# liangfu/dspnet

Hardware: AMD Instinct MI355X
Metric: training images/sec at 512x512 multitask (higher is better)
Workload: dtype f32; 1 GPU; resnet-50 multitask (det+depth+seg) 512x512, 8 det classes, 19 seg classes, N=6132 anchors, forward+backward+SGD; batch_per_gpu=32, global_batch=32, parallelism=dp1, f16x2_fallback_calls=0

## Files before the change

### dspnet_amd/csrc/bn_final_job.h

```cpp
#pragma once
#include <hip/hip_runtime.h>

namespace dspn {

constexpr int kBnJobChannels = 16;

struct BnFinalJob {
  const float *tile_sums;
  int tiles, C, blocks;
  double inv_rows;
  const float *mean, *rstd, *gamma;
  float *coef, *dgamma, *dbeta;
  const float *dy_absmax, *x_minmax;
  unsigned *dx_bound, *dx_bound_min;
};

void bn_job_defer(hipStream_t s, const BnFinalJob &job);
bool bn_job_take(hipStream_t s, BnFinalJob *job);

__device__ __forceinline__ void bn_final_channel(const int c, const int C, const double S, const double SS, const double inv_rows,
                                                 const float *__restrict__ mean, const float *__restrict__ rstd, const float *__restrict__ gamma,
                                                 float *__restrict__ coef, float *__restrict__ dgamma, float *__restrict__ dbeta,
                                                 const float *__restrict__ x_minmax, unsigned *__restrict__ dx_bound,
                                                 unsigned *__restrict__ dx_bound_min, const float D) {
  if (dbeta) dbeta[c] = (float)S;
  if (dgamma) dgamma[c] = (float)SS;
  const double rs = rstd[c], mu = mean[c];
  const double a = (gamma ? (double)gamma[c] : 1.0) * rs;
  const double c1 = -a * rs * (SS * inv_rows);
  coef[c] = (float)a;
  coef[C + c] = (float)c1;
  const double c0 = -a * (S * inv_rows) - c1 * mu;
  coef[2 * C + c] = (float)c0;
  if (dx_bound) {
    const double lo = x_minmax[c], hi = x_minmax[C + c];
    double b = fabs(a) * (double)D + fmax(fabs(c1 * lo + c0), fabs(c1 * hi + c0));
    b *= 1.0 + 1e-6;
    float bf = (float)b;
    if (!(bf == bf)) bf = INFINITY;
    if (bf > 0.f) atomicMax(dx_bound + (c & 63), __float_as_uint(bf));
    if (dx_bound_min && bf > 0.f && bf < INFINITY) atomicMin(dx_bound_min, __float_as_uint(bf));
  }
}

__device__ __forceinline__ void bn_final_job_run(const BnFinalJob &j, const int b, void *smem) {
  double *s_S = static_cast<double *>(smem), *s_SS = s_S + 16 * kBnJobChannels;
  float *s_D = reinterpret_cast<float *>(s_SS + 16 * kBnJobChannels);
  const int tid = threadIdx.x;
  if (j.dx_bound && tid < 64) {
    float m = j.dy_absmax[tid];
#pragma unroll
    for (int o = 32; o >= 1; o >>= 1) m = fmaxf(m, __shfl_xor(m, o, 64));
    if (tid == 0) *s_D = m;
  }
  const int cl = tid & (kBnJobChannels - 1), v = tid >> 4;
  const int c = b * kBnJobChannels + cl;
  const int C = j.C;
  if (tid < 256) {
    double S = 0, SS = 0;
    if (c < C) {
      const float *__restrict__ ts = j.tile_sums;
#pragma unroll 8
      for (int k = v; k < j.tiles; k += 16) {
        S += ts[(long long)k * 2 * C + c];
        SS += ts[(long long)k * 2 * C + C + c];
      }
    }
    s_S[v * kBnJobChannels + cl] = S; s_SS[v * kBnJobChannels + cl] = SS;
  }
  __syncthreads();
  if (tid < kBnJobChannels && c < C) {
    double S = s_S[cl], SS = s_SS[cl];
    for (int k = 1; k < 16; ++k) { S += s_S[k * kBnJobChannels + cl]; SS += s_SS[k * kBnJobChannels + cl]; }
    bn_final_channel(c, C, S, SS, j.inv_rows, j.mean, j.rstd, j.gamma, j.coef, j.dgamma, j.dbeta, j.x_minmax, j.dx_bound,
                     j.dx_bound_min, j.dx_bound ? *s_D : 0.f);
// ... 5 lines not shown
```

### dspnet_amd/csrc/conv.hip

```cpp
#include "dspn_common.h"
#include "bn_final_job.h"
#include "dspn_store.h"
#include "dspn_pieces.h"
#include "conv_geom.h"
#include <cstdlib>
#include "../../include/dspn_nn.h"

using dspn::st_t;
using dspn::kHalf;
using dspn::u32x4_t;

namespace {

using dspn::conv::f32x16;
using dspn::conv::bf16x8;
using dspn::pieces::bf16x4;
typedef __attribute__((address_space(3))) bf16x4 lds_bf16x4;

constexpr int kLdsRowH = kHalf ? 72 : 40;
__device__ __forceinline__ bf16x4 to_bf16x4(const float4 v) {
  bf16x4 r = {(__bf16)v.x, (__bf16)v.y, (__bf16)v.z, (__bf16)v.w};
  return r;
}

// ... 1630 lines not shown
    splits = (int)std::min<long long>((384 + nblk - 1) / nblk, nk / 8);
    splits = std::max(1, std::min(splits, 32));
    while (splits > 1 && sizeof(float) * (size_t)splits * M * g.Cout > ws.bytes) --splits;
    per = (nk + splits - 1) / splits;
    splits = (nk + per - 1) / per;
  }
  static const int eight_mode = (int)dspn::env_int("DSPN_NT_8WAVE", -1);
  const bool one_tap = g.TR * g.TS == 1;
  const bool eight = eight_mode == 0 ? false : eight_mode == 1 ? true : (kHalf || g.bf16 >= 2) ? true
                     : ((!g.stats && !g.bn_sums) || (eight_mode == 2 && one_tap && g.bn_sums) || (eight_mode == 3 && one_tap));
  bool wide_ok = splits == 1 && (cfg == 0 || (cfg == 2 && g.Cout > 32 && g.Cout <= 64)) && (g.flags & 16) && g.Cout % 4 == 0 &&
                 g.TR * g.TS > 0;
  if (kHalf) wide_ok = wide_ok && !g.in_scale && g.Cin % 64 == 0 && dspn::wide_tiles_mode() >= 2;
  else wide_ok = wide_ok && pre && g.bf16 == 3;
  const dspn::conv::WideRoute route = wide_ok ? dspn::conv::wide_route(g, M, nk) : dspn::conv::WideRoute{};
  if (g.sadd) {
    constexpr const char *who = DSPN_FN_NAME(dspn_conv2d_dgrad_bn_sadd);
    if (kHalf) return dspn::fail(DSPN_ERR_ARG_, "%s: the strided addend takes float tensors only", who);
    if (g.bf16 != 3) return dspn::fail(DSPN_ERR_ARG_, "%s: the strided addend needs DSPN_MATH_F32_F16X2", who);
    if (splits > 1) return dspn::fail(DSPN_ERR_ARG_, "%s: the strided addend cannot be combined with split-K (%d splits)", who, splits);
    if (!g.bn_sums) return dspn::fail(DSPN_ERR_ARG_, "%s: the strided addend needs the BatchNorm-backward sums (bn_sums)", who);
    if (!g.dense || g.ldc != g.Cout || (g.flags & (1 | 2 | 4 | 8)) || residual)
      return dspn::fail(DSPN_ERR_ARG_, "%s: the strided addend needs a dense dx written by this call alone (no accumulate)", who);
    if (g.sadd_h != (g.Hg + 1) / 2 || g.sadd_w != (g.Wg + 1) / 2 || g.Wg < 8 || g.Wg % 4 != 0)
      return dspn::fail(DSPN_ERR_ARG_, "%s: the strided addend is (N, ceil(H / 2), ceil(W / 2), Cin) with W >= 8 and W %% 4 == 0, got %d x %d for %d x %d", who,
                        g.sadd_h, g.sadd_w, g.Hg, g.Wg);
    if (!((route.tile == dspn::conv::WideTile::P128x128 || route.tile == dspn::conv::WideTile::P128x256) &&
          route.loop == dspn::conv::WideLoop::Spanning))
      return dspn::fail(DSPN_ERR_ARG_, "%s: no kernel takes the strided addend on this route (it needs dy as piece planes, N H W %% 128 == 0 "
                        "and the plane-fed 128-row tiles on the tile-spanning loop)", who);
    g.sadd_bytes = (unsigned)((long long)sizeof(st_t) * g.N * g.sadd_h * g.sadd_w * g.Cout);
    if (g.probe) return 0;
  }
  if (route) return dspn::conv::launch_wide(route, in, w, bias, out, g, s, residual);
  const int rc = cfg == 0 && eight ? launch_nt<4, 2, 1, 2>(in, w, bias, out, g, s, splits, per, ws.ptr, residual)
                 : cfg == 0        ? launch_nt<2, 2, 2, 2>(in, w, bias, out, g, s, splits, per, ws.ptr, residual)
                 : cfg == 1        ? launch_nt<2, 2, 2, 1>(in, w, bias, out, g, s, splits, per, ws.ptr, residual)
                 : cfg == 2        ? launch_nt<2, 2, 1, 1>(in, w, bias, out, g, s, splits, per, ws.ptr, residual)
                                   : launch_nt<4, 1, 2, 1>(in, w, bias, out, g, s, splits, per, ws.ptr, residual);
  return rc ? rc : output_absmax_pass(out, g, s);
}

struct WgradPlan { int bm; int bn; int splits; int pps; };
constexpr int kPlanPK = 64;
static_assert(kPlanPK % kPK == 0, "split sizes must be whole k-steps");
long long wgrad_x_footprint(long long P, int Cin, int taps, int stride) { return taps > 1 ? 4ll * P * Cin * std::min(stride, 2) * std::min(stride, 2) : 0; }
WgradPlan wgrad_plan(long long P, int Cout, int J, long long x_bytes = 0, long long max_splits = 1 << 30) {
  WgradPlan p;
  p.bm = Cout <= 32 ? 32 : (Cout <= 64 ? 64 : 128);
  if (p.bm == 128 && (Cout + 63) / 64 * 64 < (Cout + 127) / 128 * 128) p.bm = 64;
  p.bn = (J <= 64 && p.bm == 128) ? 64 : 128;
  if (const char *e = getenv("DSPN_WG_TILE")) {
    const int t = atoi(e);
    p.bm = t == 0 ? 32 : (t == 1 ? 64 : 128);
    p.bn = t == 2 ? 64 : 128;
  }
  const long long tiles = (long long)((Cout + p.bm - 1) / p.bm) * ((J + p.bn - 1) / p.bn);
  const long long lds = 4ll * std::max(2 * kPK * (p.bm + p.bn), p.bm * (p.bn + 4));
  const long long slots = 256 * std::min<long long>(8, (160ll << 10) / lds);
  long long s_min = 1;
  if (x_bytes > 0) s_min = (x_bytes + (32ll << 20) - 1) / (32ll << 20);
  const long long s_max = std::max<long long>(1, std::min<long long>(std::min<long long>(P / 128, 1024), max_splits));
  s_min = std::min(s_min, s_max);
  const double flop_per_pix = 2.0 * p.bm * p.bn, slot_rate = 120e12 / (double)slots, ovh_pix = 160;
  double best = 1e30;
  long long splits = s_min;
// ... 268 lines not shown
  return dspn::check_launch("absmax_batch");
}

int dspn_conv2d_weight_planes_batch_f32(const void *table, int n, long long total_tiles, void *stream) {
  DSPN_REQUIRE(table && n > 0 && total_tiles > 0 && total_tiles < (1ll << 31), "weight_planes_batch: bad argument");
  static_assert(sizeof(WpDesc) == 64, "table row layout: 3 pointers, 4 ints, 1 int64, 1 pointer, 2 ints");
  hipLaunchKernelGGL(weight_planes_batch_kernel, dim3((unsigned)total_tiles), dim3(256), 0, (hipStream_t)stream,
                     static_cast<const WpDesc *>(table), n);
  return dspn::check_launch("weight_planes_batch");
}
#else
int dspn_conv2d_weight_prepare_bf16(const float *w, st_t *wh, st_t *wt, int Cout, int taps, int Cin,
                                    int Cout_pad, void *stream) {
  DSPN_REQUIRE(w && wt && Cout > 0 && taps > 0 && Cin > 0 && Cout_pad >= Cout && Cout_pad % kEPC == 0,
               "weight_prepare: bad argument");
  const long long total = (long long)Cin * taps * Cout_pad;
  const int blocks = (int)std::min<long long>((total + 255) / 256, 4096);
  hipLaunchKernelGGL(weight_transpose_kernel, dim3(blocks), dim3(256), 0, (hipStream_t)stream, w,
                     wt, wh, Cout, taps, Cin, Cout_pad);
  return dspn::check_launch("weight_prepare");
}

int dspn_conv2d_weight_prepare_batch_bf16(const void *table, int n, long long total_tiles, void *stream) {
  DSPN_REQUIRE(table && n > 0 && total_tiles > 0 && total_tiles < (1ll << 31), "weight_prepare_batch: bad argument");
  static_assert(sizeof(WtDesc) == 48, "table row layout: 2 pointers, 4 ints, 1 int64, 1 pointer");
  hipLaunchKernelGGL(weight_transpose_batch_kernel, dim3((unsigned)total_tiles), dim3(256), 0, (hipStream_t)stream,
                     static_cast<const WtDesc *>(table), n);
  return dspn::check_launch("weight_prepare_batch");
}
#endif

struct BnBwd { const st_t *x; const float *scale, *shift, *mean, *rstd; int relu; float *sums; float *dy_absmax; };
struct StridedAddend { const st_t *p; int h, w, probe; };

static int dgrad_tiles(int N, int H, int W, int Cin, int stride, int *per_class ) {
  int total = 0;
  for (int ph = 0; ph < (stride == 1 ? 1 : 2); ++ph)
    for (int pw = 0; pw < (stride == 1 ? 1 : 2); ++pw) {
      const long long hg = stride == 1 ? H : (H - ph + 1) / 2, wg = stride == 1 ? W : (W - pw + 1) / 2;
      const long long M = (long long)N * hg * wg;
      const int t = M > 0 ? (int)((M + kNtBm[nt_config(M, Cin)] - 1) / kNtBm[nt_config(M, Cin)]) : 0;
      if (per_class) per_class[ph * 2 + pw] = t;
      total += t;
    }
  return total;
}

static int conv2d_dgrad_one(int math, OpScales scales, const st_t *dy, const st_t *wt, const void *wt_planes, st_t *dx, int N, int H, int W,
                          int Cin, int ldy, int R, int S, int stride, int pad_h, int pad_w, int dil, int Ho,
                          int Wo, int dx_ldc, int accumulate, BnBwd bn, void *workspace, size_t workspace_bytes,
                          void *stream, StridedAddend sa = StridedAddend{nullptr, 0, 0, 0}) {
  DSPN_REQUIRE(dy && (wt || wt_planes) && dx, "conv2d_dgrad: null pointer");
  DSPN_REQUIRE(ldy % kEPC == 0, "conv2d_dgrad: dy channel stride must be a multiple of %d", kEPC);
  DSPN_REQUIRE(stride == 1 || (stride == 2 && dil == 1), "conv2d_dgrad: stride 1, or stride 2 with dilation 1");
  DSPN_REQUIRE(N > 0 && H > 0 && W > 0 && Cin > 0 && R > 0 && S > 0, "conv2d_dgrad: bad geometry");
  ConvGeom g;
  memset(&g, 0, sizeof(g));
  g.N = N; g.Hin = Ho; g.Win = Wo; g.Cin = ldy; g.Cout = Cin;
  g.WTAPS = R * S; g.WS = S;
  g.ldc = dx_ldc > 0 ? dx_ldc : Cin;
  g.obs = (long long)H * W * g.ldc;
  g.OW = W;
  g.flags = accumulate ? 4 : 0;
  g.bf16 = kHalf ? 1 : math;
  g.w_planes = wt_planes;
  g.a_absmax = scales.a; g.b_absmax = scales.b;
  g.bn_x = bn.x; g.bn_scale = bn.scale; g.bn_shift = bn.shift; g.bn_mean = bn.mean; g.bn_rstd = bn.rstd;
  g.bn_relu = bn.relu; g.bn_sums = bn.sums; g.bn_tile_base = 0;
  g.bn_dy_absmax = (bn.sums && !kHalf && math == DSPN_MATH_F32_F16X2) ? reinterpret_cast<unsigned *>(bn.dy_absmax) : nullptr;
  g.a_planes = scales.a_planes;
  g.sadd = sa.p; g.sadd_h = sa.h; g.sadd_w = sa.w; g.probe = sa.probe;
  int class_tiles[4] = {0, 0, 0, 0};
  if (bn.sums) dgrad_tiles(N, H, W, Cin, stride, class_tiles);
  hipStream_t s = (hipStream_t)stream;
  const SplitWs sws{static_cast<float *>(workspace), workspace ? workspace_bytes : 0};
  if (stride == 1) {
    g.Hg = H; g.Wg = W; g.ish = 1; g.isw = 1; g.ioh = pad_h; g.iow = pad_w; g.idh = -dil; g.idw = -dil;
    g.TR = R; g.TS = S; g.wr0 = 0; g.wrs = 1; g.ws0 = 0; g.wss = 1;
    g.osh = 1; g.osw = 1; g.dense = 1;
    return dispatch_nt(dy, wt, nullptr, dx, g, s, sws);
  }
  for (int ph = 0; ph < 2; ++ph)
    for (int pw = 0; pw < 2; ++pw) {
      ConvGeom c = g;
      c.Hg = (H - ph + 1) / 2; c.Wg = (W - pw + 1) / 2;
      for (int q = 0; q < ph * 2 + pw; ++q) c.bn_tile_base += class_tiles[q];
      if (c.Hg <= 0 || c.Wg <= 0) continue;
      const int r0 = (ph + pad_h) & 1, s0 = (pw + pad_w) & 1;
      c.TR = r0 < R ? (R - r0 + 1) / 2 : 0;
      c.TS = s0 < S ? (S - s0 + 1) / 2 : 0;
      if (c.TR == 0 || c.TS == 0) {
        c.TR = 0; c.TS = 1;
        if (accumulate && !bn.sums) continue;
      }
      c.ish = 1; c.isw = 1; c.ioh = (ph + pad_h - r0) / 2; c.iow = (pw + pad_w - s0) / 2;
      c.idh = -1; c.idw = -1;
      c.wr0 = r0; c.wrs = 2; c.ws0 = s0; c.wss = 2;
      c.osh = 2; c.osw = 2; c.ooh = ph; c.oow = pw; c.dense = 0;
      const int rc = dispatch_nt(dy, wt, nullptr, dx, c, s, sws);
      if (rc) return rc;
    }
  return 0;
}

static int dgrad_bn_tiles(int N, int H, int W, int Cin, int stride) {
  if (N <= 0 || H <= 0 || W <= 0 || Cin <= 0 || Cin % 4 != 0 || (stride != 1 && stride != 2)) return 0;
  return dgrad_tiles(N, H, W, Cin, stride, nullptr);
}
#ifndef DSPN_HALF
int dspn_conv2d_dgrad_bn_tiles(int N, int H, int W, int Cin, int stride) { return dgrad_bn_tiles(N, H, W, Cin, stride); }
#endif

}
static int conv2d_dgrad_bn_impl(const st_t *dy, const st_t *wt, const void *wt_planes, st_t *dx, int N, int H, int W,
                             int Cin, int ldy, int R, int S, int stride, int pad_h, int pad_w, int dil, int Ho,
                             int Wo, int dx_ldc, int accumulate,
                             const st_t *bn_x, const float *bn_scale, const float *bn_shift, const float *bn_mean,
                             const float *bn_rstd, int bn_relu, float *bn_sums, size_t bn_sums_bytes, float *bn_dy_absmax,
                             int math, const float *dy_absmax, const float *w_absmax, void *workspace, size_t workspace_bytes,
                             void *stream, StridedAddend sa) {
  DSPN_REQUIRE(N > 0 && Ho > 0 && Wo > 0 && ldy > 0, "conv2d_dgrad: bad geometry");
  if (sa.p) {
    constexpr const char *who = DSPN_FN_NAME(dspn_conv2d_dgrad_bn_sadd);
    DSPN_REQUIRE(stride == 1 && !accumulate, "%s: the strided addend goes with a stride-1 data gradient that is the only writer of dx (no accumulate)", who);
    DSPN_REQUIRE((dx_ldc <= 0 || dx_ldc == Cin), "%s: the strided addend needs a dense dx (dx_ldc %d, Cin %d)", who, dx_ldc, Cin);
    DSPN_REQUIRE(batch_chunk(N, (long long)sizeof(st_t) * Ho * Wo * ldy) == N, "%s: dy of 2 GiB or more", who);
  }
  const int flags = split_math(&math, DSPN_MATH_DY_PLANES), dy_planes = (flags & DSPN_MATH_DY_PLANES) ? 1 : 0;
  DSPN_REQUIRE(!dy_planes || (!dspn::kHalf && math == DSPN_MATH_F32_F16X2 && ldy % 32 == 0 && dy_absmax),
               "conv2d_dgrad: DSPN_MATH_DY_PLANES needs DSPN_MATH_F32_F16X2, ldy %% 32 == 0 and the block the planes were cut by (dy_absmax)");
  if (const int rc = check_math_mode("conv2d_dgrad", math)) return rc;
  if (const int rc = check_math_blocks("conv2d_dgrad", math, flags, dy_absmax, w_absmax)) return rc;
  const int ldc = dx_ldc > 0 ? dx_ldc : Cin;
  const int nb = batch_chunk(N, (long long)sizeof(st_t) * Ho * Wo * ldy);
  if (bn_sums) {
    DSPN_REQUIRE(bn_x && bn_mean && bn_rstd && (!bn_relu || (bn_scale && bn_shift)), "conv2d_dgrad: BatchNorm operands missing");
    DSPN_REQUIRE(ldc == Cin && nb == N, "conv2d_dgrad: BatchNorm sums need a dense dx and dy below 2 GiB");
    const int tiles = dgrad_bn_tiles(N, H, W, Cin, stride);
    DSPN_REQUIRE(tiles > 0 && bn_sums_bytes >= sizeof(float) * 2 * (size_t)tiles * Cin,
                 "conv2d_dgrad: bn_sums needs dspn_conv2d_dgrad_bn_tiles() x 2 x Cin floats");
  }
  for (int n0 = 0; n0 < N; n0 += nb) {
    const int n = std::min(nb, N - n0);
    const int rc = conv2d_dgrad_one(math, OpScales{dy_absmax, w_absmax, dy_planes}, dy + (long long)n0 * Ho * Wo * ldy, wt, wt_planes, dx + (long long)n0 * H * W * ldc, n, H,
                                    W, Cin, ldy, R, S, stride, pad_h, pad_w, dil, Ho, Wo, dx_ldc, accumulate,
                                    BnBwd{bn_x, bn_scale, bn_shift, bn_mean, bn_rstd, bn_relu, bn_sums, bn_dy_absmax}, workspace,
                                    workspace_bytes, stream, sa);
    if (rc) return rc;
  }
  return 0;
}
extern "C" {
int DSPN_FN(dspn_conv2d_dgrad_bn)(const st_t *dy, const st_t *wt, const void *wt_planes, st_t *dx, int N, int H, int W,
                             int Cin, int ldy, int R, int S, int stride, int pad_h, int pad_w, int dil, int Ho,
                             int Wo, int dx_ldc, int accumulate,
                             const st_t *bn_x, const float *bn_scale, const float *bn_shift, const float *bn_mean,
                             const float *bn_rstd, int bn_relu, float *bn_sums, size_t bn_sums_bytes, float *bn_dy_absmax,
                             int math, const float *dy_absmax, const float *w_absmax, void *workspace, size_t workspace_bytes,
                             void *stream) {
  return conv2d_dgrad_bn_impl(dy, wt, wt_planes, dx, N, H, W, Cin, ldy, R, S, stride, pad_h, pad_w, dil, Ho, Wo, dx_ldc, accumulate, bn_x,
                              bn_scale, bn_shift, bn_mean, bn_rstd, bn_relu, bn_sums, bn_sums_bytes, bn_dy_absmax, math, dy_absmax,
                              w_absmax, workspace, workspace_bytes, stream, StridedAddend{nullptr, 0, 0, 0});
}
int DSPN_FN(dspn_conv2d_dgrad_bn_sadd)(const st_t *dy, const st_t *wt, const void *wt_planes, st_t *dx, int N, int H, int W,
                             int Cin, int ldy, int R, int S, int stride, int pad_h, int pad_w, int dil, int Ho,
                             int Wo, int dx_ldc, int accumulate,
                             const st_t *bn_x, const float *bn_scale, const float *bn_shift, const float *bn_mean,
                             const float *bn_rstd, int bn_relu, float *bn_sums, size_t bn_sums_bytes, float *bn_dy_absmax,
                             int math, const float *dy_absmax, const float *w_absmax, void *workspace, size_t workspace_bytes,
                             const st_t *strided_addend, int addend_h, int addend_w, void *stream) {
  DSPN_REQUIRE(strided_addend && addend_h > 0 && addend_w > 0, "%s: no strided addend (dspn_conv2d_dgrad_bn is the call without one)",
               DSPN_FN_NAME(dspn_conv2d_dgrad_bn_sadd));
  return conv2d_dgrad_bn_impl(dy, wt, wt_planes, dx, N, H, W, Cin, ldy, R, S, stride, pad_h, pad_w, dil, Ho, Wo, dx_ldc, accumulate, bn_x,
                              bn_scale, bn_shift, bn_mean, bn_rstd, bn_relu, bn_sums, bn_sums_bytes, bn_dy_absmax, math, dy_absmax,
                              w_absmax, workspace, workspace_bytes, stream, StridedAddend{strided_addend, addend_h, addend_w, 0});
}
#ifndef DSPN_HALF
int dspn_conv2d_dgrad_bn_sadd_route_f32(int N, int H, int W, int Cin, int ldy, int dy_planes) {
  float *const q = reinterpret_cast<float *>(uintptr_t(256));
  const int tiles = dgrad_bn_tiles(N, H, W, Cin, 1);
  if (tiles <= 0 || N <= 0 || ldy <= 0) return 0;
  return conv2d_dgrad_bn_impl(q, nullptr, q, q, N, H, W, Cin, ldy, 1, 1, 1, 0, 0, 1, H, W, Cin, 0, q, q, q, q, q, 1, q,
                              sizeof(float) * 2 * (size_t)tiles * Cin, q, DSPN_MATH_F32_F16X2 | (dy_planes ? DSPN_MATH_DY_PLANES : 0), q, q,
                              nullptr, 0, nullptr, StridedAddend{q, (H + 1) / 2, (W + 1) / 2, 1}) == 0 ? 1 : 0;
}
#endif

#ifndef DSPN_HALF
int dspn_conv2d_dgrad_f32(const float *dy, const float *wt, float *dx, int N, int H, int W,
                          int Cin, int ldy, int R, int S, int stride, int pad_h, int pad_w, int dil, int Ho,
                          int Wo, int dx_ldc, int accumulate, void *workspace, size_t workspace_bytes,
                          void *stream) {
  return dspn_conv2d_dgrad_bn_f32(dy, wt, nullptr, dx, N, H, W, Cin, ldy, R, S, stride, pad_h, pad_w, dil, Ho, Wo, dx_ldc,
                                  accumulate, nullptr, nullptr, nullptr, nullptr, nullptr, 0, nullptr, 0, nullptr, DSPN_MATH_FP32,
                                  nullptr, nullptr, workspace, workspace_bytes, stream);
}

size_t dspn_conv2d_input_sum_grad_workspace_bytes(int Ho, int Wo, int ldy, int R, int S) {
  return sizeof(float) * ((size_t)Ho * Wo * ldy + (size_t)R * S * 32 * ldy);
}
#endif

int DSPN_FN(dspn_conv2d_input_sum_grad)(const st_t *dy, const float *w, float *out, int N, int H, int W,
                                   int Cin, int Cout, int ldy, int R, int S, int stride, int pad_h, int pad_w, int dil,
                                   int Ho, int Wo, void *workspace, size_t workspace_bytes, void *stream) {
  DSPN_REQUIRE(dy && w && out && workspace, "conv2d_input_sum_grad: null pointer");
  DSPN_REQUIRE(ldy % 4 == 0 && Cin >= 1 && Cin <= 8, "conv2d_input_sum_grad: Cin <= 8, ldy % 4 == 0");
  if (workspace_bytes < sizeof(float) * ((size_t)Ho * Wo * ldy + (size_t)R * S * 32 * ldy))
    return dspn::fail(DSPN_ERR_WORKSPACE_, "conv2d_input_sum_grad: workspace too small");
  hipStream_t s = (hipStream_t)stream;
  float *p2 = static_cast<float *>(workspace);
  float *partial = p2 + (size_t)Ho * Wo * ldy;
  const long long per4 = (long long)Ho * Wo * ldy / 4;
  hipLaunchKernelGGL(batch_sum_kernel, dim3((int)std::min<long long>((per4 + 255) / 256, 8192)), dim3(256), 0, s,
                     dspn::CA4Ptr(dy), reinterpret_cast<float4 *>(p2), N, per4);
  SumGradGeom g{H, W, Ho, Wo, ldy, R, S, stride, stride, pad_h, pad_w, dil, dil, 32};
  hipLaunchKernelGGL(tap_sum_kernel, dim3(R * S, 32), dim3(256), 0, s, p2, partial, g);
// ... 146 lines not shown
```

### dspnet_amd/csrc/conv_geom.h

```cpp
#pragma once
#include <hip/hip_runtime.h>

namespace dspn {
namespace conv {

typedef float f32x16 __attribute__((ext_vector_type(16)));
typedef __bf16 bf16x8 __attribute__((ext_vector_type(8)));

template <typename st_t>
struct ConvGeomT {
  int N, Hin, Win, Cin;
  int Hg, Wg;
  int ish, isw, ioh, iow, idh, idw;
  int TR, TS;
  int WTAPS, WS, wr0, wrs, ws0, wss;
  int Cout;
  long long obs;
  int OW, osh, osw, ooh, oow, ldc;
  int flags;
  int dense;
  int dbg;
  int bf16;
  unsigned in_bytes, w_bytes;
  const float *in_scale, *in_shift;
  float *stats;
  float *minmax;
  const st_t *bn_x;
  const float *bn_scale, *bn_shift, *bn_mean, *bn_rstd;
  float *bn_sums;
  int bn_relu, bn_tile_base;
  unsigned *bn_dy_absmax;
  const float *a_absmax, *b_absmax;
  int a_planes;
  const void *w_planes;
  const st_t *sadd;
  int sadd_h, sadd_w;
  unsigned sadd_bytes;
  int probe;
};

__device__ __forceinline__ int xcd_remap(int bid, int nblk) {
  const int q = nblk >> 3, r = nblk & 7, x = bid & 7;
  const int start = x < r ? x * (q + 1) : r * (q + 1) + (x - r) * q;
  return start + (bid >> 3);
}


enum class WideTile { None, P256x128, P128x256, P128x128, P256x64, F128x256, F128x128, F256x64 };
enum class WideLoop { Plain, Spanning, Direct };
struct WideRoute {
  WideTile tile = WideTile::None; WideLoop loop = WideLoop::Plain;
  explicit operator bool() const { return tile != WideTile::None; }
};
WideRoute wide_route(const ConvGeomT<float> &g, long long M, int nk);
WideRoute wide_route(const ConvGeomT<__bf16> &g, long long M, int nk);
int launch_wide(WideRoute r, const float *in, const float *w_planes, const float *bias, float *out, const ConvGeomT<float> &g,
                hipStream_t s, const float *residual);
int launch_wide(WideRoute r, const __bf16 *in, const __bf16 *w, const float *bias, __bf16 *out, const ConvGeomT<__bf16> &g,
                hipStream_t s, const __bf16 *residual);

int launch_stem(const float *x, const float *w, float *y, int N, int H, int W, int Cin, int Cout, int Ho, int Wo,
                const float *x_absmax, const float *w_absmax, float *stats, float *minmax, hipStream_t s);

}
}
```

### dspnet_amd/csrc/conv_wide.h

```cpp

#ifdef DSPN_STAMPS
__device__ unsigned long long g_wide_stamps[1024 * 16];
struct WideStamps {
  unsigned long long last, sum[16];
  __device__ __forceinline__ void begin() { for (int i = 0; i < 16; ++i) sum[i] = 0; last = __builtin_readcyclecounter(); }
  __device__ __forceinline__ void mark(int i) { const unsigned long long t = __builtin_readcyclecounter(); sum[i] += t - last; last = t; }
  __device__ __forceinline__ void flush() {
    if (threadIdx.x == 0 && blockIdx.x < 1024) for (int i = 0; i < 16; ++i) g_wide_stamps[blockIdx.x * 16 + i] = sum[i];
  }
};
#define DSPN_STAMP_DECL WideStamps stamps_; stamps_.begin()
#define DSPN_STAMP(i) stamps_.mark(i)
#define DSPN_STAMP_FLUSH stamps_.flush()
#define DSPN_STAMP_ARG , stamps_
#define DSPN_STAMP_PARAM , WideStamps &stamps_
#else
#define DSPN_STAMP_DECL
#define DSPN_STAMP(i)
#define DSPN_STAMP_FLUSH
#define DSPN_STAMP_ARG
#define DSPN_STAMP_PARAM
#endif

struct NoStage {};
// ... 170 lines not shown
  if constexpr (EPI == 2) {
    __builtin_amdgcn_s_barrier();
    float *red = reinterpret_cast<float *>(wsm);
    if (cvalid) {
#pragma unroll
      for (int h = 0; h < HALVES; ++h)
#pragma unroll
        for (int e = 0; e < 4; ++e) {
          red[((h * RPP + er0) * BN + c4 * 4 + e) * 2] = gs[h][e];
          red[((h * RPP + er0) * BN + c4 * 4 + e) * 2 + 1] = gss[h][e];
        }
    }
    asm volatile("s_waitcnt lgkmcnt(0)" ::: "memory");
    __builtin_amdgcn_s_barrier();
    for (int hc = tid; hc < HALVES * BN; hc += NTHR) {
      const int h = hc / BN, col = hc - h * BN;
      if (n0 + col >= g.Cout || m0 + h * SR >= M) continue;
      const float *rh = red + (size_t)h * RPP * BN * 2;
      float a = 0.f, b = 0.f;
      for (int er = 0; er < RPP; ++er) { a += rh[(er * BN + col) * 2]; b += rh[(er * BN + col) * 2 + 1]; }
      const long long mt_ = g.bn_tile_base + m0 / SR + h;
      g.bn_sums[(mt_ * 2 + 0) * g.Cout + n0 + col] = a;
      g.bn_sums[(mt_ * 2 + 1) * g.Cout + n0 + col] = b;
    }
    gmx_all = fmaxf(gmx_all, gmx);
  }
  if constexpr (EPI == 0) gmx_all = fmaxf(gmx_all, gmx);
  asm volatile("s_waitcnt lgkmcnt(0)" ::: "memory");
  __builtin_amdgcn_s_barrier();
  DSPN_STAMP(6);
}

#ifndef DSPN_HALF
template <int WAVES_M, int WAVES_N, int EPI, int RB = 16, int SR = 128, bool CLOSE = false, bool SADD = false>
__device__ __forceinline__ void direct_epilogue(const ConvGeom &g, char *exch, f32x16 (&acc)[2][2], const float inv_a, const float inv_b, const int m0,
                                                const int n0, const int M, const int tid, const int wave,
                                                const float *__restrict__ bias, float *__restrict__ out,
                                                const float *__restrict__ residual, float &gmx_all) {
  constexpr int TM = 2, TN = 2, BN = WAVES_N * 64, NTHR = WAVES_M * WAVES_N * 64, PARTS = WAVES_M * 2;
  constexpr int WRT = SR / 64, TILES = WAVES_M / WRT, PPT = WRT * 2;
  static_assert(SR == 64 || SR == 128, "statistics tiles of 64 or 128 rows");
  static_assert(WAVES_M % WRT == 0, "whole statistics tiles per output tile");
  const int lane = tid & 63, half = lane >> 5, lc = lane & 31;
  const int wr = wave / WAVES_N, wm = wr * 64, wn = (wave % WAVES_N) * 64;
  const bool has_bias = g.flags & 1, relu = g.flags & 2, accum = g.flags & 4, has_res = g.flags & 8;
  const float *addsrc = has_res ? residual : (accum ? out : nullptr);
  const unsigned obytes = (unsigned)M * (unsigned)g.ldc * 4u;
  const __amdgpu_buffer_rsrc_t rs_o = __builtin_amdgcn_make_buffer_rsrc(out, 0, obytes, 0x00020000);
  const __amdgpu_buffer_rsrc_t rs_a = __builtin_amdgcn_make_buffer_rsrc(const_cast<float *>(addsrc ? addsrc : out), 0, addsrc ? obytes : 0u, 0x00020000);
  const __amdgpu_buffer_rsrc_t rs_x = __builtin_amdgcn_make_buffer_rsrc(const_cast<float *>(EPI == 2 ? g.bn_x : out), 0, EPI == 2 ? obytes : 0u, 0x00020000);
  constexpr unsigned kOOB = 0x80000000u;
  constexpr float kInf = __builtin_huge_valf();
  int col[TN];
  unsigned cbyte[TN];
  bool cv[TN];
  float bv[TN], bsc[TN], bsh[TN], bmu[TN], brs[TN];
#pragma unroll
  for (int j = 0; j < TN; ++j) {
    col[j] = n0 + wn + j * 32 + lc;
    cv[j] = col[j] < g.Cout;
    cbyte[j] = cv[j] ? (unsigned)col[j] * 4u : kOOB;
    bv[j] = (has_bias && cv[j]) ? bias[col[j]] : 0.f;
    bsc[j] = bsh[j] = bmu[j] = brs[j] = 0.f;
    if (EPI == 2 && cv[j]) {
      bmu[j] = g.bn_mean[col[j]]; brs[j] = g.bn_rstd[col[j]];
      if (g.bn_relu) { bsc[j] = g.bn_scale[col[j]]; bsh[j] = g.bn_shift[col[j]]; }
    }
  }
  const int row0 = m0 + wm + 4 * half;
  const unsigned pitch = (unsigned)g.ldc * 4u;
  float sK[TN], s1[TN], s2[TN], vmn[TN], vmx[TN], gs[TN], gss[TN];
  int scnt = 0;
  float gmx = 0.f;
#pragma unroll
  for (int j = 0; j < TN; ++j) { sK[j] = 0.f; s1[j] = 0.f; s2[j] = 0.f; vmn[j] = kInf; vmx[j] = -kInf; gs[j] = 0.f; gss[j] = 0.f; }
  const bool both = has_res && accum;
  constexpr int NB = TM * 16 / RB;
  const bool need_rows = addsrc != nullptr || EPI == 2;
  if constexpr (EPI == 2) {
    float rq[2][RB][TN], xq[2][RB][TN], oq[2][RB][TN];
    int sa_n = 0, sa_h = 0, sa_w = 0;
    __amdgpu_buffer_rsrc_t rs_s = rs_a;
    if constexpr (SADD) {
      static_assert(!SADD || RB == 4, "one group of four rows per batch");
      rs_s = __builtin_amdgcn_make_buffer_rsrc(const_cast<float *>(g.sadd), 0, g.sadd_bytes, 0x00020000);
      const int hw = g.Hg * g.Wg;
      sa_n = row0 / hw;
      const int rem = row0 - sa_n * hw;
      sa_h = rem / g.Wg; sa_w = rem - sa_h * g.Wg;
    }
    auto request = [&](const int bb, const int s_) __attribute__((always_inline)) {
      const int i = bb / (16 / RB), r0 = (bb % (16 / RB)) * RB;
      unsigned sa_off[TN];
#pragma unroll
      for (int j = 0; j < TN; ++j) sa_off[j] = kOOB;
      if constexpr (SADD) {
        const unsigned sa_rb = (unsigned)((sa_n * g.sadd_h + (sa_h >> 1)) * g.sadd_w + (sa_w >> 1)) * pitch;
#pragma unroll
        for (int j = 0; j < TN; ++j) sa_off[j] = ((sa_h & 1) || !cv[j]) ? kOOB : sa_rb + cbyte[j];
        sa_w += 8;
        const bool wrap = sa_w >= g.Wg;
        sa_w -= wrap ? g.Wg : 0;
        sa_h += wrap ? 1 : 0;
        const bool wrap2 = sa_h >= g.Hg;
        sa_h = wrap2 ? 0 : sa_h;
        sa_n += wrap2 ? 1 : 0;
      }
#pragma unroll
      for (int rr = 0; rr < RB; ++rr) {
        const int r = r0 + rr;
        const unsigned rb = (unsigned)(row0 + 32 * i + (r & 3) + 8 * (r >> 2)) * pitch;
#pragma unroll
        for (int j = 0; j < TN; ++j) {
          const unsigned off = rb + cbyte[j];
          if constexpr (SADD)
            rq[s_][rr][j] = (rr & 1) ? 0.f : __builtin_bit_cast(float, __builtin_amdgcn_raw_buffer_load_b32(rs_s, (int)(sa_off[j] + (unsigned)(rr >> 1) * pitch), 0, 0));
          else
          rq[s_][rr][j] = addsrc ? __builtin_bit_cast(float, __builtin_amdgcn_raw_buffer_load_b32(rs_a, (int)off, 0, 0)) : 0.f;
          xq[s_][rr][j] = __builtin_bit_cast(float, __builtin_amdgcn_raw_buffer_load_b32(rs_x, (int)off, 0, 0));
          oq[s_][rr][j] = both ? __builtin_bit_cast(float, __builtin_amdgcn_raw_buffer_load_b32(rs_o, (int)off, 0, 0)) : 0.f;
        }
      }
    };
    request(0, 0);
#pragma unroll
    for (int bb = 0; bb < NB; ++bb) {
      const int i = bb / (16 / RB), r0 = (bb % (16 / RB)) * RB, s_ = bb & 1;
      if (bb + 1 < NB) request(bb + 1, s_ ^ 1);
#pragma unroll
      for (int rr = 0; rr < RB; ++rr) {
        const int r = r0 + rr;
        const unsigned rb = (unsigned)(row0 + 32 * i + (r & 3) + 8 * (r >> 2)) * pitch;
#pragma unroll
        for (int j = 0; j < TN; ++j) {
          float v = acc[i][j][r] * inv_a * inv_b + bv[j];
          v += rq[s_][rr][j];
          if (both) v += oq[s_][rr][j];
          if (relu) v = v > 0.f ? v : 0.f;
          __builtin_amdgcn_raw_buffer_store_b32(__builtin_bit_cast(unsigned, v), rs_o, (int)(rb + cbyte[j]), 0, 0);
          const float xv = xq[s_][rr][j];
          const float gd = (!g.bn_relu || fmaf(xv, bsc[j], bsh[j]) > 0.f) ? v : 0.f;
          gs[j] += gd;
          gss[j] += gd * ((xv - bmu[j]) * brs[j]);
          gmx = fmaxf(gmx, fabsf(v));
        }
      }
    }
#pragma unroll
    for (int j = 0; j < TN; ++j) { gs[j] = cv[j] ? gs[j] : 0.f; gss[j] = cv[j] ? gss[j] : 0.f; }
  } else {
    typedef float f32x2 __attribute__((ext_vector_type(2)));
    f32x2 s1p[TN], s2p[TN];
#pragma unroll
    for (int j = 0; j < TN; ++j) { s1p[j] = f32x2{0.f, 0.f}; s2p[j] = f32x2{0.f, 0.f}; }
    f32x2 rq[2][RB / 2][TN], oq[2][RB / 2][TN];
    auto request = [&](const int bb, const int s_) __attribute__((always_inline)) {
      const int i = bb / (16 / RB), r0 = (bb % (16 / RB)) * RB;
#pragma unroll
      for (int rr = 0; rr < RB; rr += 2) {
        const int r = r0 + rr;
        const unsigned rb = (unsigned)(row0 + 32 * i + (r & 3) + 8 * (r >> 2)) * pitch;
#pragma unroll
        for (int j = 0; j < TN; ++j) {
          const unsigned off = rb + cbyte[j];
          rq[s_][rr / 2][j] = f32x2{0.f, 0.f}; oq[s_][rr / 2][j] = f32x2{0.f, 0.f};
          if (addsrc) rq[s_][rr / 2][j] = f32x2{__builtin_bit_cast(float, __builtin_amdgcn_raw_buffer_load_b32(rs_a, (int)off, 0, 0)),
                                               __builtin_bit_cast(float, __builtin_amdgcn_raw_buffer_load_b32(rs_a, (int)(off + pitch), 0, 0))};
          if (both) oq[s_][rr / 2][j] = f32x2{__builtin_bit_cast(float, __builtin_amdgcn_raw_buffer_load_b32(rs_o, (int)off, 0, 0)),
                                             __builtin_bit_cast(float, __builtin_amdgcn_raw_buffer_load_b32(rs_o, (int)(off + pitch), 0, 0))};
        }
      }
    };
    if (need_rows) request(0, 0);
#pragma unroll
    for (int bb = 0; bb < NB; ++bb) {
      const int i = bb / (16 / RB), r0 = (bb % (16 / RB)) * RB, s_ = bb & 1;
      if (need_rows && bb + 1 < NB) request(bb + 1, s_ ^ 1);
#pragma unroll
      for (int rr = 0; rr < RB; rr += 2) {
        const int r = r0 + rr;
        const unsigned rb = (unsigned)(row0 + 32 * i + (r & 3) + 8 * (r >> 2)) * pitch;
#pragma unroll
        for (int j = 0; j < TN; ++j) {
          f32x2 t = f32x2{acc[i][j][r], acc[i][j][r + 1]} * inv_a * inv_b + bv[j];
          if (need_rows) t += rq[s_][rr / 2][j];
          else t += f32x2{0.f, 0.f};
          float v0 = t[0], v1 = t[1];
          if (both) { v0 += oq[s_][rr / 2][j][0]; v1 += oq[s_][rr / 2][j][1]; }
          if (relu) { v0 = v0 > 0.f ? v0 : 0.f; v1 = v1 > 0.f ? v1 : 0.f; }
          __builtin_amdgcn_raw_buffer_store_b32(__builtin_bit_cast(unsigned, v0), rs_o, (int)(rb + cbyte[j]), 0, 0);
          __builtin_amdgcn_raw_buffer_store_b32(__builtin_bit_cast(unsigned, v1), rs_o, (int)(rb + pitch + cbyte[j]), 0, 0);
          const f32x2 v = f32x2{v0, v1};
          if constexpr (EPI == 0) {
            if (g.bn_dy_absmax) gmx = fmaxf(fmaxf(gmx, fabsf(v0)), fabsf(v1));
          }
          if constexpr (EPI == 1) {
            if (bb == 0 && rr == 0) sK[j] = v0;
            const f32x2 d = v - sK[j];
            s1p[j] += d; s2p[j] += d * d;
            vmn[j] = fminf(fminf(vmn[j], v0), v1); vmx[j] = fmaxf(fmaxf(vmx[j], v0), v1);
          }
        }
      }
    }
    scnt = 32;
#pragma unroll
    for (int j = 0; j < TN; ++j) { s1[j] = s1p[j].x + s1p[j].y; s2[j] = s2p[j].x + s2p[j].y; }
  }
  if constexpr (EPI == 0) gmx_all = fmaxf(gmx_all, gmx);
  if constexpr (EPI == 2) gmx_all = fmaxf(gmx_all, gmx);
  if constexpr (EPI != 0) {
    float *red = reinterpret_cast<float *>(exch);
    float *red2 = red + PARTS * BN * 4;
    const bool mmx = EPI == 1 && g.minmax != nullptr;
    const int p = wr * 2 + half;
#pragma unroll
    for (int j = 0; j < TN; ++j) {
      float *q = red + (p * BN + wn + j * 32 + lc) * 4;
      if constexpr (EPI == 1) {
        const float inv_n = scnt > 0 ? 1.f / (float)scnt : 0.f;
        q[0] = (float)scnt; q[1] = sK[j] + s1[j] * inv_n; q[2] = s2[j] - s1[j] * s1[j] * inv_n;
        if (mmx) { float *q2 = red2 + (p * BN + wn + j * 32 + lc) * 2; q2[0] = vmn[j]; q2[1] = vmx[j]; }
      } else {
        q[0] = gs[j]; q[1] = gss[j];
      }
    }
    asm volatile("s_waitcnt lgkmcnt(0)" ::: "memory");
    __builtin_amdgcn_s_barrier();
    for (int hc = tid; hc < TILES * BN; hc += NTHR) {
      const int h = hc / BN, c = hc - h * BN;
      if (n0 + c >= g.Cout || m0 + h * SR >= M) continue;
      const long long mt_ = m0 / SR + h;
      if constexpr (EPI == 1) {
        float n = 0.f, mean = 0.f, m2 = 0.f, mn = kInf, mx = -kInf;
#pragma unroll
        for (int pq = 0; pq < PPT; ++pq) {
          const int pp = h * PPT + pq;
          const float *q = red + (pp * BN + c) * 4;
          const float nb = q[0];
          if (nb > 0.f) {
            const float d = q[1] - mean, nn = n + nb;
            mean += d * (nb / nn);
            m2 += q[2] + d * d * (n * nb / nn);
            n = nn;
// ... 11 lines not shown
#pragma unroll
        for (int pq = 0; pq < PPT; ++pq) { a += red[((h * PPT + pq) * BN + c) * 4]; b += red[((h * PPT + pq) * BN + c) * 4 + 1]; }
        const long long t_ = g.bn_tile_base + mt_;
        g.bn_sums[(t_ * 2 + 0) * g.Cout + n0 + c] = a;
        g.bn_sums[(t_ * 2 + 1) * g.Cout + n0 + c] = b;
      }
    }
    if constexpr (CLOSE) {
      asm volatile("s_waitcnt lgkmcnt(0)" ::: "memory");
      __builtin_amdgcn_s_barrier();
    }
  }
}
#endif

template <int NWV>
__device__ __forceinline__ void wide_publish_absmax(const ConvGeom &g, char *wsm, float gmx_all, const int tid) {
  const int lane = tid & 63, wave = tid >> 6;
    if (g.bn_dy_absmax) {
#pragma unroll
      for (int o = 32; o >= 1; o >>= 1) gmx_all = fmaxf(gmx_all, __shfl_xor(gmx_all, o, 64));
      float *sm = reinterpret_cast<float *>(wsm);
      if (lane == 0) sm[wave] = gmx_all;
      asm volatile("s_waitcnt lgkmcnt(0)" ::: "memory");
      __builtin_amdgcn_s_barrier();
      if (tid == 0) {
        float m = sm[0];
        for (int q = 1; q < NWV; ++q) m = fmaxf(m, sm[q]);
        if (m > 0.f) atomicMax(g.bn_dy_absmax + (blockIdx.x & 63u), __float_as_uint(m));
      }
    }
}

template <int WAVES_M, int WAVES_N, int STAGES, int EPI, int SR = 128, bool XT = false, bool SADD = false>
__global__ __launch_bounds__(WAVES_M * WAVES_N * 64, 2) void conv_ntw_kernel(
    const st_t *__restrict__ in, const st_t *__restrict__ wgt, const float *__restrict__ bias,
    st_t *__restrict__ out, const ConvGeom g, const int m_tiles, const int n_tiles,
    const st_t *__restrict__ residual) {
  constexpr int TM = 2, TN = 2;
  constexpr int KB = 128 / (int)sizeof(st_t);
  constexpr int NKK = kHalf ? 4 : 2, NPROD = kHalf ? 1 : 3;
  constexpr int BM = WAVES_M * TM * 32, BN = WAVES_N * TN * 32;
  constexpr int NWV = WAVES_M * WAVES_N, NTHR = NWV * 64;
  constexpr int A_NI = BM / (8 * NWV), B_NI = BN / (8 * NWV), NI = A_NI + B_NI;
  static_assert(BM % (8 * NWV) == 0 && BN % (8 * NWV) == 0, "whole pieces per wave");
  constexpr int STG = (BM + BN) * 128;
  constexpr int D = STAGES - 1;
  static_assert(STAGES >= 2 && STAGES <= 4, "ring depth");
  static_assert(BM % SR == 0, "BatchNorm tables are per SR rows");
  static_assert(!XT || !kHalf, "the tile-spanning loop: float build");
  static_assert(!SADD || (XT && EPI == 2 && SR == 128), "the strided addend: tile-spanning loop, BatchNorm-backward sums, 128-row tables");
  extern __shared__ __attribute__((aligned(1024))) char wsm[];

#ifdef DSPN_ABLATE
  const int dbg = g.dbg;
#else
  constexpr int dbg = 0;
#endif
  const int tid = threadIdx.x, lane = tid & 63;
  const int wave = __builtin_amdgcn_readfirstlane(tid >> 6);
  const int ntiles = m_tiles * n_tiles;
  const int M = g.N * g.Hg * g.Wg;
  const int CB = g.Cin / KB;
  const int ntaps = g.TR * g.TS;
  const int nk = ntaps * CB;
  const float sc_a = kHalf ? 1.f : operand_scale(g.a_absmax), sc_b = kHalf ? 1.f : operand_scale(g.b_absmax);
  const float inv_a = 1.f / sc_a, inv_b = 1.f / sc_b;
  const __amdgpu_buffer_rsrc_t rsrc_a = __builtin_amdgcn_make_buffer_rsrc(const_cast<st_t *>(in), 0, g.in_bytes, 0x00020000);
  const __amdgpu_buffer_rsrc_t rsrc_b = __builtin_amdgcn_make_buffer_rsrc(const_cast<st_t *>(wgt), 0, g.w_bytes, 0x00020000);
  constexpr unsigned kOOB = 0x80000000u;

  int a_row[A_NI], b_row[B_NI], a_cb[A_NI], b_cb[B_NI];
#pragma unroll
  for (int i = 0; i < A_NI; ++i) {
    const int line = 4 * (wave * A_NI + i) + (lane >> 4), sl = (lane & 15) ^ (line & 7);
    a_row[i] = 2 * line + (sl >> 3); a_cb[i] = (sl & 7) * 16;
  }
#pragma unroll
  for (int i = 0; i < B_NI; ++i) {
    const int line = 4 * (wave * B_NI + i) + (lane >> 4), sl = (lane & 15) ^ (line & 7);
    b_row[i] = 2 * line + (sl >> 3); b_cb[i] = (sl & 7) * 16;
  }
  int a_ih0[A_NI], a_iw0[A_NI], a_boff[A_NI], b_boff[B_NI];
  int ld_m0 = 0, ld_n0 = 0;
// ... 109 lines not shown
        acc[i][j] = __builtin_amdgcn_mfma_f32_32x32x16_bf16(fa[ia][i], fb[ib][j], acc[i][j], 0, 0, 0);
      else
        acc[i][j] = __builtin_amdgcn_mfma_f32_32x32x16_f16(__builtin_bit_cast(f16x8, fa[ia][i]),
                                                           __builtin_bit_cast(f16x8, fb[ib][j]), acc[i][j], 0, 0, 0);
#pragma unroll
      for (int q = 0; q < NI; ++q)
        if (((q + 1) * NMMA) / NI - 1 == m) {
          issue_piece(q);
          __builtin_amdgcn_sched_barrier(0);
        }
    }
  };

  float gmx_all = 0.f;

  if constexpr (XT) {
    constexpr bool EXCH_IN_RING = NWV == 8 || BM == 256;
    int t = blockIdx.x;
    if (t < ntiles) {
      setup_tile(t);
#pragma unroll
      for (int j = 0; j < D; ++j) issue(j, true);
    }
    int slot = 0, islot = D % STAGES;
    bool more = false;
    DSPN_STAMP_DECL;
    for (; t < ntiles; t += gridDim.x) {
      const int m0 = ld_m0, n0 = ld_n0;
      const int tn = t + (int)gridDim.x;
      const bool first = t == (int)blockIdx.x;
      zero_acc();
      int last_slot = 0;
      for (int kt = 0; kt < nk; ++kt) {
        if (!first && kt < D) asm volatile("s_waitcnt vmcnt(63)" ::: "memory");
        else asm volatile("s_waitcnt vmcnt(%0)" ::"n"((D - 1) * NI) : "memory");
        __builtin_amdgcn_s_barrier();
        if (kt + D < nk) {
          issue_begin(islot, true);
        } else {
          if (kt + D == nk) { more = tn < ntiles; if (more) setup_tile(tn); }
          issue_begin(islot, more);
        }
        mma_step(slot);
        last_slot = slot;
        slot = slot + 1 == STAGES ? 0 : slot + 1;
        islot = islot + 1 == STAGES ? 0 : islot + 1;
      }
      DSPN_STAMP(2);
      char *exch = wsm + STAGES * STG;
      if constexpr (EXCH_IN_RING) {
        exch = wsm + last_slot * STG;
        if constexpr (EPI != 0) { asm volatile("s_waitcnt lgkmcnt(0)" ::: "memory"); __builtin_amdgcn_s_barrier(); }
      }
      if constexpr (!kHalf) direct_epilogue<WAVES_M, WAVES_N, EPI, (EPI == 2 ? 4 : 8), SR, false, SADD>(g, exch, acc, inv_a, inv_b, m0, n0, M, tid, wave, bias, out, residual, gmx_all);
      DSPN_STAMP(5);
    }
    DSPN_STAMP_FLUSH;
    asm volatile("s_waitcnt vmcnt(0)" ::: "memory");
    if constexpr (EPI != 1) {
      asm volatile("s_waitcnt lgkmcnt(0)" ::: "memory");
      __builtin_amdgcn_s_barrier();
      wide_publish_absmax<NWV>(g, wsm, gmx_all, tid);
    }
    return;
  }

  DSPN_STAMP_DECL;
  for (int t = blockIdx.x; t < ntiles; t += gridDim.x) {
    setup_tile(t);
    const int m0 = ld_m0, n0 = ld_n0;
#pragma unroll
    for (int j = 0; j < D; ++j) issue(j, j < nk);
    zero_acc();
    DSPN_STAMP(1);
    int slot = 0, islot = D % STAGES;
    for (int kt = 0; kt < nk; ++kt) {
      asm volatile("s_waitcnt vmcnt(%0)" ::"n"((D - 1) * NI) : "memory");
      if (!(dbg & 8)) __builtin_amdgcn_s_barrier();
      issue_begin(islot, kt + D < nk);
      mma_step(slot);
      slot = slot + 1 == STAGES ? 0 : slot + 1;
      islot = islot + 1 == STAGES ? 0 : islot + 1;
    }
    asm volatile("s_waitcnt vmcnt(0)" ::: "memory");
    asm volatile("s_waitcnt lgkmcnt(0)" ::: "memory");
    __builtin_amdgcn_s_barrier();
    DSPN_STAMP(2);
    if (dbg & 16) { if (acc[0][0][0] == 1.2345e33f) out[0] = (st_t)acc[TM - 1][TN - 1][5]; continue; }

    {
      constexpr int SLD = BN + 4;
      float *st = reinterpret_cast<float *>(wsm);
// ... 362 lines not shown
  const int mt = (int)((M + BM - 1) / BM), nt = (g.Cout + BN - 1) / BN;
  const size_t lds = XT == 1 ? (size_t)2 * (BM + BN) * 128 + sizeof(float) * 4 * BN * 6
                     : XT == 2 ? (size_t)2 * (BM + BN) * 128
                               : std::max<size_t>((size_t)2 * (BM + BN) * 128, sizeof(float) * BM * (BN + 4));
  static_assert(XT != 2 || (size_t)(BM + BN) * 128 >= sizeof(float) * 2 * WAVES_M * BN * 6, "the exchange fits a ring slot");
  constexpr auto kern = conv_ntv_kernel<WAVES_M, WAVES_N, INTF, EPI, SR, XT>;
  const int grid_x = dspn::persistent_grid<kern>(WAVES_M * WAVES_N * 64, lds, (long long)mt * nt, "conv_ntv",
                                                 "conv_ntv<%d,%d,intf=%d,epi=%d,xt=%d>", WAVES_M, WAVES_N, (int)INTF, EPI, (int)XT);
  if (grid_x < 0) return grid_x;
  {
    dspn::ProfScope prof(0, s);
    hipLaunchKernelGGL(kern, dim3(grid_x), dim3(WAVES_M * WAVES_N * 64), lds, s, in, w, bias, out, g, mt, nt, residual);
  }
  return dspn::check_launch("conv_ntv");
}
template <int WAVES_M, int WAVES_N, int SR, int XT>
int launch_ntv_on(const float *in, const float *w, const float *bias, float *out, const ConvGeom &g, hipStream_t s, const float *residual) {
#define DSPN_NTV_(T) \
  (g.bn_sums ? launch_ntv_impl<WAVES_M, WAVES_N, T, 2, SR, XT>(in, w, bias, out, g, s, residual) \
   : g.stats ? launch_ntv_impl<WAVES_M, WAVES_N, T, 1, SR, XT>(in, w, bias, out, g, s, residual) \
             : launch_ntv_impl<WAVES_M, WAVES_N, T, 0, SR, XT>(in, w, bias, out, g, s, residual))
  return g.in_scale ? DSPN_NTV_(true) : DSPN_NTV_(false);
#undef DSPN_NTV_
}
template <int WAVES_M, int WAVES_N, int SR = 128, bool SPANS = false>
int launch_ntv(WideLoop loop, const float *in, const float *w, const float *bias, float *out, const ConvGeom &g, hipStream_t s,
               const float *residual) {
  if constexpr (SPANS) if (loop == WideLoop::Spanning) return launch_ntv_on<WAVES_M, WAVES_N, SR, 1>(in, w, bias, out, g, s, residual);
  return loop == WideLoop::Direct ? launch_ntv_on<WAVES_M, WAVES_N, SR, 2>(in, w, bias, out, g, s, residual)
                                  : launch_ntv_on<WAVES_M, WAVES_N, SR, 0>(in, w, bias, out, g, s, residual);
}
#endif

template <int WAVES_M, int WAVES_N, int STAGES, int EPI, int SR, bool XT, bool SADD = false>
int launch_ntw_impl(const st_t *in, const st_t *w, const float *bias, st_t *out, const ConvGeom &g, hipStream_t s,
                    const st_t *residual) {
  constexpr int BM = WAVES_M * 64, BN = WAVES_N * 64;
  const long long M = (long long)g.N * g.Hg * g.Wg;
  const int mt = (int)((M + BM - 1) / BM), nt = (g.Cout + BN - 1) / BN;
  const size_t lds = XT ? (size_t)STAGES * (BM + BN) * 128 + ((WAVES_M * WAVES_N == 8 || BM == 256) ? 0 : sizeof(float) * 4 * BN * 6)
                        : std::max<size_t>((size_t)STAGES * (BM + BN) * 128, sizeof(float) * BM * (BN + 4));
  constexpr auto kern = conv_ntw_kernel<WAVES_M, WAVES_N, STAGES, EPI, SR, XT, SADD>;
  const int grid_x = dspn::persistent_grid<kern>(WAVES_M * WAVES_N * 64, lds, (long long)mt * nt, "conv_ntw",
                                                 SADD ? "conv_ntw<%d,%d,stages=%d,epi=%d,xt=%d,sadd>" : "conv_ntw<%d,%d,stages=%d,epi=%d,xt=%d>",
                                                 WAVES_M, WAVES_N, STAGES, EPI, (int)XT);
  if (grid_x < 0) return grid_x;
  {
    dspn::ProfScope prof(0, s);
    hipLaunchKernelGGL(kern, dim3(grid_x), dim3(WAVES_M * WAVES_N * 64), lds, s, in, w, bias, out, g, mt, nt, residual);
  }
  return dspn::check_launch("conv_ntw");
}
template <int WAVES_M, int WAVES_N, int STAGES, int SR, bool XT>
int launch_ntw_on(const st_t *in, const st_t *w, const float *bias, st_t *out, const ConvGeom &g, hipStream_t s, const st_t *residual) {
  if constexpr (XT && SR == 128 && WAVES_M == 2 && !kHalf) {
    if (g.bn_sums && g.sadd) return launch_ntw_impl<WAVES_M, WAVES_N, STAGES, 2, SR, XT, true>(in, w, bias, out, g, s, residual);
  }
  if (g.sadd) return dspn::fail(DSPN_ERR_ARG_, "conv: this kernel does not take a strided addend");
  if (g.bn_sums) return launch_ntw_impl<WAVES_M, WAVES_N, STAGES, 2, SR, XT>(in, w, bias, out, g, s, residual);
  if (g.stats) return launch_ntw_impl<WAVES_M, WAVES_N, STAGES, 1, SR, XT>(in, w, bias, out, g, s, residual);
  return launch_ntw_impl<WAVES_M, WAVES_N, STAGES, 0, SR, XT>(in, w, bias, out, g, s, residual);
}
template <int WAVES_M, int WAVES_N, int STAGES, int SR = 128, bool SPANS = false>
int launch_ntw(WideLoop loop, const st_t *in, const st_t *w, const float *bias, st_t *out, const ConvGeom &g, hipStream_t s,
               const st_t *residual) {
  if constexpr (SPANS) if (loop == WideLoop::Spanning) return launch_ntw_on<WAVES_M, WAVES_N, STAGES, SR, true>(in, w, bias, out, g, s, residual);
  return launch_ntw_on<WAVES_M, WAVES_N, STAGES, SR, false>(in, w, bias, out, g, s, residual);
}
```

### dspnet_amd/csrc/conv_wide.hip

```cpp
#include "dspn_common.h"
#include "dspn_store.h"
#include "dspn_pieces.h"
#include "conv_geom.h"
#include "../../include/dspn_nn.h"
#include <algorithm>
#include <type_traits>

namespace {
using namespace dspn::pieces;
using dspn::st_t;
using dspn::kHalf;
using dspn::u32x4_t;
using dspn::conv::f32x16;
using dspn::conv::bf16x8;
using dspn::conv::xcd_remap;
using dspn::conv::WideLoop;
using ConvGeom = dspn::conv::ConvGeomT<st_t>;
#include "conv_wide.h"
#ifndef DSPN_HALF
#include "conv_stem.h"
#endif
}

#ifndef DSPN_HALF
namespace {
struct AbsminRowsDesc { const float *w; unsigned *out; int rows, row_len; long long begin; };
__global__ __launch_bounds__(256) void absmin_rows_batch_kernel(const AbsminRowsDesc *__restrict__ d, int n) {
  __shared__ float sm[4];
  const long long row = blockIdx.x;
  int lo = 0, hi = n - 1;
  while (lo < hi) {
    const int mid = (lo + hi + 1) >> 1;
    if (d[mid].begin <= row) lo = mid; else hi = mid - 1;
  }
  const AbsminRowsDesc e = d[lo];
  const float *p = e.w + (row - e.begin) * (long long)e.row_len;
// ... 35 lines not shown
  return dspn::check_launch("absmin_rows_batch");
}
int dspn_tile_minmax_f32(const float *x, long long rows, int C, int tile_rows, float *minmax, void *stream) {
  DSPN_REQUIRE(x && minmax && rows > 0 && C > 0 && C % 4 == 0 && tile_rows > 0, "tile_minmax: bad argument (C must be a multiple of 4)");
  const long long tiles = (rows + tile_rows - 1) / tile_rows;
  DSPN_REQUIRE(tiles < (1ll << 31), "tile_minmax: too many tiles");
  hipLaunchKernelGGL(tile_minmax_kernel, dim3((unsigned)tiles, (C / 4 + 255) / 256), dim3(256), 0, (hipStream_t)stream,
                     reinterpret_cast<const float4 *>(x), rows, C / 4, tile_rows, reinterpret_cast<float4 *>(minmax));
  return dspn::check_launch("tile_minmax");
}
}

#endif

namespace dspn {
namespace conv {
#ifndef DSPN_HALF
int launch_stem(const float *x, const float *w, float *y, int N, int H, int W, int Cin, int Cout, int Ho, int Wo,
                const float *x_absmax, const float *w_absmax, float *stats, float *minmax, hipStream_t s) {
  return launch_conv_stem(x, w, y, N, H, W, Cin, Cout, Ho, Wo, x_absmax, w_absmax, stats, minmax, s);
}
#endif
static WideTile wide_tile_choice(long long M, int Cout, int nk, int fused_epilogue) {
  constexpr WideTile forced[5] = {WideTile::None, WideTile::None, WideTile::P256x128, WideTile::P128x256, WideTile::P128x128};
  const int mode = dspn::wide_tiles_mode();
  if (mode == 1) return WideTile::None;
  if (mode >= 2) return Cout <= 64 ? WideTile::P256x64 : forced[mode];
  if (Cout <= 64) return nk >= 4 ? WideTile::P256x64 : WideTile::None;
  if (nk < 4 && !(fused_epilogue && nk >= 2)) return WideTile::None;
  if (Cout % 256 == 0 && nk >= 8 && ((M + 127) / 128) * (Cout / 256) >= 256) return WideTile::P128x256;
  return WideTile::P128x128;
}
WideRoute wide_route(const ConvGeomT<st_t> &g, long long M, int nk) {
  WideRoute r{wide_tile_choice(M, g.Cout, nk, (g.stats || g.bn_sums) ? 1 : 0)};
#ifndef DSPN_HALF
  if (!r) return r;
  if (!g.a_planes)
    r.tile = r.tile == WideTile::P128x256 ? WideTile::F128x256 : r.tile == WideTile::P256x64 ? WideTile::F256x64 : WideTile::F128x128;
  const int xt = dspn::tile_spanning();
  const int bm = (r.tile == WideTile::P256x64 || r.tile == WideTile::F256x64) ? 256 : 128;
  const bool output_ok = g.dense && (g.flags & 16) && M % bm == 0 && M * g.ldc * (long long)sizeof(st_t) < (1ll << 31);
  if (xt == 0 || !output_ok) return r;
  if (r.tile == WideTile::P128x128) {
    if (nk >= 2) r.loop = WideLoop::Spanning;
  } else if (r.tile == WideTile::P128x256) {
    static const bool wide8 = dspn::env_int("DSPN_XT8", 1) != 0;
    if (nk >= 3 && wide8) r.loop = WideLoop::Spanning;
  } else if (bm == 256) {
    static const bool c64 = dspn::env_int("DSPN_XT64", 1) != 0;
    if (nk >= 2 && c64) r.loop = r.tile == WideTile::P256x64 ? WideLoop::Spanning : WideLoop::Direct;
  } else if (r.tile == WideTile::F128x128 && xt >= 2 && nk >= 2 && nk <= 8 && nk % 2 == 0 &&
             ((M + 127) / 128) * ((g.Cout + 127) / 128) >= 2048) {
    r.loop = WideLoop::Spanning;
  } else if (r.tile == WideTile::F128x128) {
    static const bool direct = dspn::env_int("DSPN_NTV_DIRECT", 1) != 0;
    if (nk >= 2 && direct) r.loop = WideLoop::Direct;
  } else if (r.tile == WideTile::F128x256) {
    static const bool direct8 = dspn::env_int("DSPN_NTV_DIRECT8", 1) != 0;
    if (nk >= 2 && direct8) r.loop = WideLoop::Direct;
  }
#endif
  return r;
}
int launch_wide(WideRoute r, const st_t *in, const st_t *w_planes, const float *bias, st_t *out, const ConvGeomT<st_t> &g,
                hipStream_t s, const st_t *residual) {
  switch (r.tile) {
    case WideTile::P256x128: return launch_ntw<4, 2, 3>(r.loop, in, w_planes, bias, out, g, s, residual);
// ... 14 lines not shown
```

### dspnet_amd/csrc/nn.hip

```cpp
#include "dspn_common.h"
#include "bn_final_job.h"
#include "dspn_store.h"
#include "dspn_pieces.h"
#include "../../include/dspn_nn.h"

using dspn::st_t;
using dspn::A1Ptr;
using dspn::A4Ptr;
using dspn::CA1Ptr;
using dspn::CA4Ptr;

#pragma clang fp contract(fast)

namespace {

constexpr int kT = 256;
inline int slab_rows_for(long long rows) {
  const long long want = (rows + 1023) / 1024;
  return (int)std::min<long long>(512, std::max<long long>(32, (want + 7) / 8 * 8));
}

inline int grid_for(long long n, int per_block = kT, int cap = 8192) {
  long long b = (n + per_block - 1) / per_block;
  return (int)std::max<long long>(1, std::min<long long>(b, cap));
// ... 1774 lines not shown
  j.dx_bound = reinterpret_cast<unsigned *>(dx_bound); j.dx_bound_min = reinterpret_cast<unsigned *>(dx_bound_min);
  return j;
}
static void bn_final_launch(hipStream_t s, const dspn::BnFinalJob &j) {
  hipLaunchKernelGGL(bn_bwd_final_kernel, dim3((j.C + 63) / 64), dim3(1024), 0, s, j.tile_sums, j.tiles, j.C, j.inv_rows, j.mean,
                     j.rstd, j.gamma, j.coef, j.dgamma, j.dbeta, j.dy_absmax, j.x_minmax, j.dx_bound, j.dx_bound_min);
}

static int bn_bwd_apply_launch(hipStream_t s, const st_t *x, const float *scale, const float *shift, const st_t *dy,
                               const float *coef, st_t *dx, long long rows, int C, int relu, int accumulate, float *dx_absmax,
                               const char *what) {
  const int C4 = C / 4;
  const long long n4 = rows * C4;
  int fixed = 0, u4 = 0;
#ifdef DSPN_HALF
  if (C % 8 == 0 && ((reinterpret_cast<uintptr_t>(x) | reinterpret_cast<uintptr_t>(dy) | reinterpret_cast<uintptr_t>(dx)) & 15) == 0) {
    const int grid8 = grid_fixed_channel(n4 / 2, C / 8, &fixed, &u4);
    hipLaunchKernelGGL(u4 ? bn_bwd_apply8_kernel<4> : bn_bwd_apply8_kernel<1>, dim3(grid8), dim3(kT), 0, s,
                       reinterpret_cast<const dspn::u32x4_t *>(x), reinterpret_cast<const float4 *>(scale),
                       reinterpret_cast<const float4 *>(shift), reinterpret_cast<const dspn::u32x4_t *>(dy),
                       reinterpret_cast<const float4 *>(coef), reinterpret_cast<dspn::u32x4_t *>(dx), n4 / 2, C / 8, relu,
                       accumulate, fixed);
    return dspn::check_launch(what);
  }
#endif
  const int grid4 = grid_fixed_channel(n4, C4, &fixed, &u4);
  hipLaunchKernelGGL(u4 ? bn_bwd_apply_kernel<4> : bn_bwd_apply_kernel<1>, dim3(grid4), dim3(kT), 0, s, CA4Ptr(x),
                     reinterpret_cast<const float4 *>(scale), reinterpret_cast<const float4 *>(shift), CA4Ptr(dy),
                     reinterpret_cast<const float4 *>(coef), A4Ptr(dx), n4, C4, relu, accumulate,
                     dspn::kHalf ? nullptr : reinterpret_cast<unsigned *>(dx_absmax), fixed);
  return dspn::check_launch(what);
}

extern "C" {

#ifndef DSPN_HALF
size_t dspn_bn_workspace_bytes(long long rows, int C) { return bn_workspace_bytes(rows, C); }
#endif

static int bn_moving_arg(const dspn_bn_moving *mv, long long rows, int C, const char *what, BnMovingK *out) {
  *out = kNoMoving;
  if (!mv) return 0;
  DSPN_REQUIRE(mv->moving_mean && mv->moving_var, "%s: moving_mean and moving_var must not be NULL", what);
  DSPN_REQUIRE(mv->momentum >= 0.f && mv->momentum <= 1.f, "%s: momentum must be in [0, 1]", what);
  DSPN_REQUIRE(mv->mode == DSPN_BN_TRACK || mv->mode == DSPN_BN_GLOBAL, "%s: mode must be DSPN_BN_TRACK or DSPN_BN_GLOBAL", what);
  DSPN_REQUIRE(mv->channels >= 0 && mv->channels <= C, "%s: channels must be in [0, C]", what);
  const double n = (double)rows;
  *out = BnMovingK{mv->moving_mean, mv->moving_var, (double)mv->momentum, 1.0 - (double)mv->momentum,
                   rows > 1 ? n / (n - 1.0) : 1.0, mv->mode, mv->channels ? mv->channels : C};
  return 0;
}

static int bn_stats_run(const st_t *x, long long rows, int C, float eps, const float *gamma, const float *beta, float *mean,
                        float *rstd, float *scale, float *shift, void *workspace, size_t workspace_bytes, const BnMovingK &mv,
                        void *stream) {
  DSPN_REQUIRE(x && beta && mean && rstd && scale && shift && workspace, "bn_stats: null pointer");
  DSPN_REQUIRE(rows > 0 && C > 0 && C % 4 == 0, "bn_stats: C must be a positive multiple of 4");
  if (workspace_bytes < bn_workspace_bytes(rows, C))
    return dspn::fail(DSPN_ERR_WORKSPACE_, "bn_stats: workspace too small");
  const int C4 = C / 4, CL = std::min(C4, 64);
  int ns = 0;
  float *partial = static_cast<float *>(workspace);
  if (mv.mode != DSPN_BN_GLOBAL) {
    ns = bn_slabs(rows);
    hipLaunchKernelGGL(bn_stats_partial_kernel, dim3(ns, (C4 + CL - 1) / CL), dim3(kT),
                       sizeof(float4) * 2 * kT, S_(stream), CA4Ptr(x), rows,
// ... 137 lines not shown
                     reinterpret_cast<const float4 *>(scale), reinterpret_cast<const float4 *>(shift),
                     reinterpret_cast<const float4 *>(coef), reinterpret_cast<float4 *>(dx), n4, C4, relu,
                     reinterpret_cast<unsigned *>(dx_absmax), pool);
  return dspn::check_launch("bn_backward_maxpool");
}
#endif

#ifndef DSPN_HALF
int dspn_bn_apply_planes_f32(const float *x, const float *scale, const float *shift, void *y_planes, long long rows, int C,
                             int relu, const float *y_absmax, void *stream) {
  DSPN_REQUIRE(x && scale && shift && y_planes && y_absmax, "bn_apply_planes: null pointer (y_absmax is the block the planes are cut by)");
  DSPN_REQUIRE(rows > 0 && C > 0 && C % 32 == 0, "bn_apply_planes: C must be a positive multiple of 32");
  DSPN_REQUIRE(static_cast<const void *>(x) != y_planes, "bn_apply_planes: in place is not supported");
  const long long n4 = rows * (C / 4);
  int fixed4 = 0, u4 = 0;
  const int grid4 = grid_fixed_channel(n4, C / 4, &fixed4, &u4);
  hipLaunchKernelGGL(u4 ? bn_apply_planes_kernel<4> : bn_apply_planes_kernel<1>, dim3(grid4), dim3(kT), 0, S_(stream),
                     reinterpret_cast<const float4 *>(x), reinterpret_cast<const float4 *>(scale),
                     reinterpret_cast<const float4 *>(shift), static_cast<uint4 *>(y_planes), n4, C / 4, relu, y_absmax, fixed4);
  return dspn::check_launch("bn_apply_planes");
}
#endif

int DSPN_FN(dspn_bn_backward_from_sums)(const st_t *x, const float *scale, const float *shift, const st_t *dy,
                                   const float *mean, const float *rstd, const float *gamma, const float *tile_sums,
                                   int tiles, st_t *dx, float *dgamma, float *dbeta, long long rows, int C, int relu,
                                   int accumulate, float *dx_absmax, float *dx_absmin, const float *dy_absmax, const float *x_chan_minmax,
                                   int flags, void *workspace, size_t workspace_bytes, void *stream) {
  const int planes = flags & DSPN_BN_SUMS_PLANES, half = flags & (DSPN_BN_SUMS_FINALIZE_ONLY | DSPN_BN_SUMS_APPLY_ONLY),
            parked = flags & DSPN_BN_SUMS_PARKED;
  DSPN_REQUIRE((flags & ~(DSPN_BN_SUMS_PLANES | DSPN_BN_SUMS_FINALIZE_ONLY | DSPN_BN_SUMS_APPLY_ONLY | DSPN_BN_SUMS_PARKED)) == 0 &&
                   half != (DSPN_BN_SUMS_FINALIZE_ONLY | DSPN_BN_SUMS_APPLY_ONLY) && (!parked || half == DSPN_BN_SUMS_FINALIZE_ONLY),
               "bn_backward_from_sums: flag word = dx_planes | 2 (finalize only, | 8: parked for the next weight gradient) | 4 (apply only)");
  DSPN_REQUIRE(x && dy && mean && rstd && workspace && tile_sums && tiles > 0, "bn_backward_from_sums: null pointer");
  DSPN_REQUIRE(dx || flags == DSPN_BN_SUMS_FINALIZE_ONLY, "bn_backward_from_sums: dx == NULL needs the finalize-only flag word 2");
  DSPN_REQUIRE(!planes || (!dspn::kHalf && !accumulate && C % 32 == 0 && dx_absmax && dy_absmax && x_chan_minmax &&
                           static_cast<const void *>(dx) != static_cast<const void *>(dy) && static_cast<const void *>(dx) != static_cast<const void *>(x)),
               "bn_backward_from_sums: dx as piece planes needs float tensors, C %% 32 == 0, no accumulation, dx apart from x and dy, "
               "and dx_absmax / dy_absmax / x_chan_minmax (the bound of dx is formed from the last two)");
  DSPN_REQUIRE(!relu || (scale && shift), "bn_backward_from_sums: relu needs the forward scale/shift");
  DSPN_REQUIRE(rows > 0 && C > 0 && C % 4 == 0, "bn_backward_from_sums: C must be a positive multiple of 4");
  const size_t coef_bytes = sizeof(float) * 3 * (size_t)C;
  if (workspace_bytes < coef_bytes)
    return dspn::fail(DSPN_ERR_WORKSPACE_, "bn_backward_from_sums: workspace too small (3*C floats)");
  float *coef = static_cast<float *>(workspace);
  if (half == DSPN_BN_SUMS_APPLY_ONLY) {
    for (dspn::BnFinalJob job; dspn::bn_job_take(S_(stream), &job);)
      hipLaunchKernelGGL(bn_final_job_kernel, dim3(job.blocks), dim3(256), 0, S_(stream), job);
  } else {
    BnTiles t{tile_sums, tiles, 1, tiles, nullptr};
    bn_group_tiles<1>(S_(stream), t, C, coef + 3 * (size_t)C, workspace_bytes - coef_bytes);
    const dspn::BnFinalJob job = bn_final_job(t.table, t.tiles, C, rows, mean, rstd, gamma, coef, dgamma, dbeta,
                                              planes ? dy_absmax : nullptr, planes ? x_chan_minmax : nullptr,
                                              planes ? dx_absmax : nullptr, planes ? dx_absmin : nullptr);
    if (parked) {
      dspn::bn_job_defer(S_(stream), job);
      return dspn::check_launch("bn_backward_from_sums (parked)");
    }
    bn_final_launch(S_(stream), job);
  }
  if (half == DSPN_BN_SUMS_FINALIZE_ONLY) return dspn::check_launch("bn_backward_from_sums (finalize)");
#ifndef DSPN_HALF
  if (planes) {
    const int C4 = C / 4;
    const long long n4 = rows * C4;
    int fixed4 = 0, u4 = 0;
    const int grid4 = grid_fixed_channel(n4, C4, &fixed4, &u4);
    hipLaunchKernelGGL(u4 ? bn_bwd_apply_planes_kernel<4> : bn_bwd_apply_planes_kernel<1>, dim3(grid4), dim3(kT), 0, S_(stream),
                       CA4Ptr(x), reinterpret_cast<const float4 *>(scale), reinterpret_cast<const float4 *>(shift), CA4Ptr(dy),
                       reinterpret_cast<const float4 *>(coef), reinterpret_cast<uint4 *>(dx), n4, C4, relu, dx_absmax, fixed4);
    return dspn::check_launch("bn_backward_from_sums");
  }
#endif
  return bn_bwd_apply_launch(S_(stream), x, scale, shift, dy, coef, dx, rows, C, relu, accumulate, dx_absmax, "bn_backward_from_sums");
}

int DSPN_FN(dspn_add)(const st_t *a, const st_t *b, st_t *out, long long n, void *stream) {
  DSPN_REQUIRE(a && b && out && n >= 0, "add: bad argument");
  const long long n4 = n / 4;
  if (n4 > 0)
    hipLaunchKernelGGL(add_kernel, dim3(grid_for(n4)), dim3(kT), 0, S_(stream),
// ... 446 lines not shown
```

### dspnet_amd/engine.py

```python
import math
import os
import re

import numpy as np
import torch

from . import functional as fn, graph_plan


FUSE_BATCHNORM = True
COMMUTE_RESIZE_CONV = True
MATERIALISE_MULTITAP_INPUT_BF16 = os.environ.get("DSPN_MAT3X3", "1") != "0"


_SHARED_STREAMS = {}


def shared_stream(device, kind, priority=0):
    key = (str(device), kind)
    ent = _SHARED_STREAMS.get(key)
    if ent is None:
        ent = _SHARED_STREAMS[key] = (torch.cuda.Stream(device=device, priority=priority), priority)
    assert ent[1] == priority, "shared stream %r of %s was created with priority %d, asked for %d" % (kind, device, ent[1], priority)
    return ent[0]
# ... 130 lines not shown
        wrapped.__wrapped__ = init
        cls.__init__ = wrapped

    def forward(self):
        raise NotImplementedError

    def backward(self):
        pass


class Graph:
    def __init__(self, device):
        self.device = device
        self.nodes = []
        self.params = {}
        self.param_order = []
        self.bn_names = []
        self.bn_nodes = {}
        self.bn_momentum, self.bn_global = 0.9, False
        self.bn_track = False
        self.tensors = {}
        self.all_tensors = []
        self.pre_forward = []
        self.wgrad_side_allowed = True
        self.wg = WgradSide(device)
        self._bn_chain = None
        self.side_segment = None
        self.side_pending = False
        self.side_bwd = None
        self.side_fwd_events, self.side_fwd_waits = {}, {}
        self.side_plan = None
        self.slab_tables = {}
        self.sc_compact_buf = None
        self.wt_table = None
        self.wt_batched = False
        self.arena = self.grad_arena = self.mom_arena = None
        self.half_operands = False
        self.math = fn.get_conv_math()
        self.wp_table = None
        self._nscal = 0
        self.scalars = None
        self.am_table = None
        self._am_x = {}
        self._am_wanted = set()
        self._am_done = set()
        self._am_bwd_slots, self._am_bwd_ran = set(), False
        self._am_table_slots = set()
        self.scalars_min = None
        self.guard = dict(enabled=os.environ.get("DSPN_RANGE_GUARD", "1") != "0", have_stats=False, risk=frozenset(),
                          calls=0, calls_total=0, at_risk_slots=0)
        self.wmin_table = None
        self.fixed_names, self.freeze_re, self.freezing = frozenset(), None, False
        self.wt_frozen = self.wp_frozen = self.am_frozen = self.wmin_frozen = None
        self.frozen_stale = False
        self._nscal_step = 0

    def set_freeze(self, fixed_param_names=None, freeze_pattern=None):
        assert not self.nodes, "set_freeze() before the graph is built"
        self.fixed_names = frozenset(fixed_param_names or ())
        self.freeze_re = re.compile(freeze_pattern) if freeze_pattern else None
        self.freezing = bool(self.fixed_names) or self.freeze_re is not None

    def is_fixed(self, name):
        return name in self.fixed_names or (self.freeze_re is not None and self.freeze_re.match(name) is not None)

    @property
# ... 406 lines not shown

    def begin_backward(self):
        for t in self.all_tensors:
            t._gw = False
            t.grad = None
            t.grad_planes = False
            t.sc_compact = None
        if self.side_bwd is not None:
            assert not self.side_bwd["dirty"], "the previous backward pass left side-stream work unjoined"
            self.side_bwd["forked"] = False
        self.guard["have_stats"] = True
        if self.scalars is not None:
            if self._am_bwd_ran:
                for slot in self._am_bwd_slots & self._am_done:
                    self.scalar(slot).zero_()
                self._am_done -= self._am_bwd_slots
            self._am_bwd_ran = True
        if self.half_operands:
            return
        self.wt_batched = self.wt_table is not None
        if self.wt_batched:
            fn.weight_transpose_batch(*self.wt_table)

    def abandon_backward(self):
        self.wg.reset()
        self.side_pending = False
        if self.side_bwd is not None:
            self.side_bwd["dirty"] = self.side_bwd["forked"] = False
        streams = set()
        for n in self.nodes:
            if isinstance(n, BatchNorm):
                if n._pending is not None:
                    streams.add(n._pending[2])
                n._pending, n.bwd_sums_ready = None, False
        for s in streams:
            fn.bn_discard_parked(s)

    def backward(self):
        self.begin_backward()
        for idx in range(len(self.nodes) - 1, -1, -1):
            self.backward_node(idx)
        self.join_side_backward()
        self.flush_slabs()

    def num_params(self):
        return sum(p.size for p in self.param_order)

    def set_params(self, arg_params, allow_missing=False, allow_extra=True):
        missing = [p.name for p in self.param_order if p.name not in arg_params]
        if missing and not allow_missing:
            raise KeyError("set_params: no value for " + ", ".join(missing[:8]) + (" ..." if len(missing) > 8 else ""))
        extra = [k for k in arg_params if k not in self.params]
        if extra and not allow_extra:
            raise KeyError("set_params: graph has no parameter " + ", ".join(extra[:8]))
        for p in self.param_order:
            if p.name not in arg_params:
                continue
            v = np.asarray(arg_params[p.name], np.float32)
            logical = tuple(p.logical or p.shape)
            if tuple(v.shape) != logical:
                raise ValueError("set_params: %s has shape %s, the graph expects %s" % (p.name, tuple(v.shape), logical))
            dev = np.zeros(p.shape, np.float32)
            if p.kind == "raw":
                dev[:] = v.reshape(p.shape)
            elif p.kind in ("conv", "deconv"):
                t = v.transpose(0, 2, 3, 1)
                dev[:t.shape[0], :, :, :t.shape[3]] = t
# ... 118 lines not shown
            if p is not None:
                p.logical = (x.channels or C,)
        g.bn_names.append((name, x.channels or C, bool(fix_gamma)))
        g.bn_nodes[name] = self
        self.channels = x.channels or C
        self.momentum, self.use_global_stats = float(g.bn_momentum), bool(g.bn_global)
        self.moving_mean = torch.zeros(C, dtype=torch.float32, device=g.device)
        self.moving_var = torch.ones(C, dtype=torch.float32, device=g.device)
        self.mean = fn.zeros(C, device=g.device)
        self.rstd = fn.zeros(C, device=g.device)
        self.scale = fn.zeros(C, device=g.device)
        self.shift = fn.zeros(C, device=g.device)
        self.defer_apply = defer_apply
        self.tile_stats = (x.producer.enable_out_stats()
                           if FUSE_BATCHNORM and x.producer is not None else None)
        self.out = g.tensor(x.shape, name + ("_relu" if relu else "_out"), requires_grad=not beta_grad_from_consumer,
                            virtual=bool(defer_apply))
        if defer_apply:
            self.out.affine_src = (x, self.scale, self.shift, relu)
        self.out.bn_node = self
        self.am_out = g.new_scalar() if (g.math == "f16x2" and self.out.dtype == torch.float32) else None
        self.out.am_slot = self.am_out
        self.conv_consumers = []
        self.mat_consumers = []
        self.bwd_sums = None
        self.bwd_sums_ready = False
        self.bwd_ws = None
        self.dx_planes, self.x_ext, self.am_dyin = False, None, None
        self.planes, self.planes_ready = None, False
        self.pool_grad = None
        self._g = g
        self.completes_x_grad = False
        self._pending = None

    def _moving(self):
        if self.use_global_stats:
            mode = fn.BN_GLOBAL
        elif self._g.bn_track:
            mode = fn.BN_TRACK
        else:
            return None
        return fn.bn_moving(self.moving_mean, self.moving_var, self.momentum, mode, self.channels)

    def forward(self):
        moving = self._moving()
        if self.tile_stats is not None:
            buf, tiles, tile_rows = self.tile_stats
            rows = int(np.prod(self.x.shape[:-1]))
            g, mm, am = self._g, getattr(self.x.producer, "out_minmax", None), None
            slot = g._am_x.get((id(self.x), id(self.scale))) if (mm is not None and g.scalars is not None) else None
            if slot is not None:
                am = g.scalar(slot)
                g._am_done.add(slot)
            fn.bn_stats_from_tiles(buf, tiles, tile_rows, rows, self.x.shape[-1], self.eps,
                                   None if self.gamma is None else self.gamma.data, self.beta.data,
                                   self.mean, self.rstd, self.scale, self.shift,
                                   tile_minmax=mm if am is not None else None, relu=self.relu, out_absmax=am,
                                   out_absmin=None if am is None else g.scalars_min[slot:slot + 1],
                                   out_chan_minmax=self.x_ext if am is not None else None, moving=moving)
            self.planes_ready = self.planes is not None and am is not None
            if self.planes_ready:
                fn.bn_apply_planes(self.x.data, self.scale, self.shift, am, relu=self.relu, out=self.planes)
        else:
            fn.bn_stats(self.x.data, self.eps, None if self.gamma is None else self.gamma.data, self.beta.data,
                        self.mean, self.rstd, self.scale, self.shift, moving=moving)
        if not self.defer_apply:
            am = self._g.scalar(self.am_out)
            fn.bn_apply(self.x.data, self.scale, self.shift, relu=self.relu, out=self.out.data, out_absmax=am)
            if am is not None:
                self._g._am_done.add(self.am_out)

    def _x_ext_valid(self):
        g = self._g
        slot = g._am_x.get((id(self.x), id(self.scale)))
        return slot is not None and slot in g._am_done

    def finalize_beside(self):
        g = self._g
        if (not FINALIZE_BESIDE or g.device.type != "cuda" or not self.bwd_sums_ready or self.pool_grad is not None
                or not self.out._gw or self._pending is not None or not self.x.requires_grad):
            return False
        self.backward(beside=True)
        return self._pending is not None

    def _from_sums(self, beside, args, kw):
        kw["workspace"] = self.bwd_ws
        if not beside:
            fn.bn_backward_from_sums(*args, **kw)
            return
        fn.bn_backward_from_sums(*args, phase=1, park=True, **kw)
        self._pending = (args, kw, fn.stream())

    def backward(self, beside=False):
        if self._pending is not None:
            args, kw, _ = self._pending
            self._pending = None
            fn.bn_backward_from_sums(*args, phase=2, **kw)
            return
        if not self.out._gw:
            return
        am = None
        dgam = None if self.gamma is None else (fn.NO_OUTPUT if self.gamma.fixed else self.gamma.grad)
        dbet = fn.NO_OUTPUT if self.beta.fixed else self.beta.grad
        if self.x.requires_grad:
            dx, acc = self.x.grad_target()
            prod, g = self.x.producer, self._g
            if (isinstance(prod, Conv) and prod.am_dy is not None and g.scalars is not None and dx.dtype == torch.float32
                    and self.completes_x_grad):
                am = g.scalar(prod.am_dy)
                g._am_done.add(prod.am_dy)
        else:
            dx, acc = fn.NO_OUTPUT, False
        if self.pool_grad is not None:
            argmax, dyp, k, s, p = self.pool_grad
            self.pool_grad = None
            if not acc:
                fn.bn_backward_maxpool(self.x.data, self.scale, self.shift, dyp, argmax, k, s, p, self.mean, self.rstd,
                                       None if self.gamma is None else self.gamma.data, relu=self.relu, dx=dx,
                                       dgamma=dgam, dbeta=dbet, dx_absmax=am)
                return
            fn.maxpool_backward_argmax(argmax, dyp, self.out.shape, k, s, p, dx=self.out.own_grad())
            self.out.grad = self.out.own_grad()
        if (self.bwd_sums_ready and self.dx_planes and am is not None and not acc and self._x_ext_valid()
                and not getattr(prod, "guard_fb", False)):
            self.bwd_sums_ready = False
            self._from_sums(beside, (self.x.data, self.scale, self.shift, self.out.grad, self.mean, self.rstd,
                                     None if self.gamma is None else self.gamma.data, self.bwd_sums[0], self.bwd_sums[1]),
                            dict(relu=self.relu, dx=dx, dgamma=dgam, dbeta=dbet, accumulate=False, dx_absmax=am,
                                 dy_absmax=self._g.scalar(self.am_dyin), x_chan_minmax=self.x_ext, dx_planes=True,
                                 dx_absmin=g.scalars_min[prod.am_dy:prod.am_dy + 1] if g.guard["enabled"] else None))
            self.x.grad_planes = True
            return
        if self.bwd_sums_ready:
            self.bwd_sums_ready = False
            self._from_sums(beside, (self.x.data, self.scale, self.shift, self.out.grad, self.mean, self.rstd,
                                     None if self.gamma is None else self.gamma.data, self.bwd_sums[0], self.bwd_sums[1]),
                            dict(relu=self.relu, dx=dx, dgamma=dgam, dbeta=dbet, accumulate=acc, dx_absmax=am))
            return
        assert not beside, "finalize_beside() without the data gradient's sums"
        fn.bn_backward(self.x.data, self.scale, self.shift, self.out.grad, self.mean, self.rstd,
                       None if self.gamma is None else self.gamma.data, relu=self.relu, dx=dx, dgamma=dgam, dbeta=dbet,
                       accumulate=acc, dx_absmax=am)


WGRAD_SIDE = int(os.environ.get("DSPN_WGRAD_SIDE", "1"))
WGRAD_SIDE_MIN_US = float(os.environ.get("DSPN_WGRAD_SIDE_MIN_US", "30"))

FINALIZE_BESIDE = os.environ.get("DSPN_FINALIZE_BESIDE", "1") != "0"

FUSE_CONV_MAGNITUDES = os.environ.get("DSPN_CONV_MAGNITUDES", "1") != "0"

SC_COMPACT = os.environ.get("DSPN_SC_COMPACT", "1") != "0"


def xa_unavailable(conv):
    return conv.out.data is None or conv.out.data.shape[-1] % 4 != 0


class Conv(Node):

    def __init__(self, g, x, name, num_filter, kernel, stride=1, pad=0, dilate=1, no_bias=True, relu=False,
                 init="xavier", cin_logical=None, cout_phys=None, input_sum_grad=None, residual=None, out_name=None,
                 tap_expand=False):
        N, H, W, Cin = x.shape
        kh, kw = fn._hw(kernel)
        ph, pw = fn._hw(pad)
        self.x, self.stride, self.pad, self.dil, self.relu = x, stride, (ph, pw), dilate, relu
        self.x_raw, self.in_affine = x, None
        if x.affine_src is not None:
            raw, sc, sh, arelu = x.affine_src
            self.x_raw, self.in_affine = raw, (sc, sh, arelu)
            assert not tap_expand
            x.bn_node.conv_consumers.append(self)
        elif x.bn_node is not None and not tap_expand:
            x.bn_node.mat_consumers.append(self)
        self.cout = num_filter
        self.input_sum_grad = input_sum_grad
        cin_meta = cin_logical if cin_logical is not None else (x.channels or Cin)
        cin_logical = Cin if cin_logical is None else cin_logical
        self.w = g.param(name + "_weight", (num_filter, kh, kw, Cin), conv_weight_init(init, cin_logical))
        self.b = None if no_bias else g.param(name + "_bias", (num_filter,), init_zeros)
        self.w.logical, self.w.kind = (num_filter, cin_meta, kh, kw), "conv"
        if self.b is not None:
            self.b.logical = (num_filter,)
        Ho, Wo = fn.conv_out_size(H, kh, stride, ph, dilate), fn.conv_out_size(W, kw, stride, pw, dilate)
        ldc = fn.padc(num_filter) if cout_phys is None else cout_phys
        self.out = g.tensor((N, Ho, Wo, ldc), out_name or (name + "_out"))
        self.out.channels = num_filter
        self.out.producer = self
        self.slabs, self.slabs_fresh = None, False
        self.out_stats = None
        self.out_minmax = None
        self._g = g
        self.residual = residual
        assert residual is None or residual.shape == self.out.shape
        half = self.out.dtype == torch.bfloat16
        self.wt_shape = (Cin, kh, kw, ldc)
        planes_t = g.device.type == "cuda" and x.requires_grad and fn.needs_planes(self.out.dtype, ldc, g.math)
        self.wt = None if (not x.requires_grad or planes_t) else fn.zeros(Cin, kh, kw, ldc, device=g.device, dtype=self.out.dtype)
        self.wh = fn.zeros(num_filter, kh, kw, Cin, device=g.device, dtype=torch.bfloat16) if half else None
        self.math = g.math
        self.am_x = self.am_dy = self.am_w = None
        if g.math == "f16x2" and self.out.dtype == torch.float32:
            key = (id(self.x_raw), None if self.in_affine is None else id(self.in_affine[0]))
            if key not in g._am_x:
                g._am_x[key] = g.new_scalar()
            self.am_x, self.am_dy, self.am_w = g._am_x[key], g.new_scalar(backward=True), g.new_scalar()
        self.am_out = g.new_scalar() if (self.am_x is not None and not tap_expand) else None
        if self.am_out is not None:
            self.out.am_slot = self.am_out
        if self.am_x is not None and self.in_affine is None:
            g.want_magnitude(self.x_raw)
        self.x_planes_bn = None
        self.bn_bwd_node = None
        self._wg_worth = None
        self.guard_fb = False
        self.sc_pair = None
        self.wp = self.wtp = None
        if g.device.type == "cuda":
            npc = fn.plane_pieces(g.math)
            if fn.needs_planes(self.out.dtype, Cin, g.math):
                self.wp = fn.zeros(num_filter, kh * kw, Cin // 32, npc, 32, device=g.device, dtype=torch.bfloat16)
            if x.requires_grad and fn.needs_planes(self.out.dtype, ldc, g.math):
                self.wtp = fn.zeros(Cin, kh * kw, ldc // 32, npc, 32, device=g.device, dtype=torch.bfloat16)
        self.tap_expand = bool(tap_expand) and kh * kw > 1
        if self.tap_expand:
            assert stride == 1 and dilate == 1 and not relu and residual is None
            assert (Ho, Wo) == (H, W), "tap expansion needs a 'same' convolution"
            self.z = fn.act_zeros(N, H, W, fn.padc(num_filter * kh * kw), device=g.device)
        self.flops_fwd = 2.0 * cin_logical * num_filter * kh * kw * Ho * Wo * N
        self.flops_bwd = self.flops_fwd * (2 if x.requires_grad else 1)

    def alloc_slabs(self):
        if self.w.fixed:
            return
        cout, kh, kw, cin = self.w.shape
        wshape = (cout * kh * kw, 1, 1, cin) if self.tap_expand else self.w.shape
        xs = self.x.shape
        splits = fn.conv2d_wgrad_splits(xs, self.z.shape if self.tap_expand else self.out.shape, wshape,
                                        1 if self.tap_expand else self.stride)
        if splits > 0 and self.w.data.numel() % 4 == 0:
            self.slabs = fn.zeros(splits, self.w.data.numel(), device=self._g.device)

    def wop(self):
        return self.w.data if self.wh is None else self.wh

    def enable_out_stats(self):
        if self.tap_expand or self.out.shape[3] != self.cout or self.cout % 4 != 0:
            return None
# ... 165 lines not shown
            self._g.guard["calls"] += 1
            self._g.guard["calls_total"] += 1
        elif self.slabs is not None:
            xp = self._x_planes()
            fn.conv2d_wgrad_slabs(self.x_raw.data if xp is None else xp, dy, self.w.shape, self.slabs, self.stride, self.pad,
                                  self.dil, in_affine=self.in_affine if xp is None else None, math=self.math, x_absmax=xa,
                                  dy_absmax=dya, dy_planes=planes, x_planes=xp is not None)
        else:
            xp = self._x_planes()
            fn.conv2d_wgrad(self.x_raw.data if xp is None else xp, dy, self.w.shape, self.stride, self.pad, self.dil,
                            out=self.w.grad, in_affine=self.in_affine if xp is None else None, math=self.math, x_absmax=xa,
                            dy_absmax=dya, dy_planes=planes, x_planes=xp is not None)
        self.slabs_fresh = self.slabs is not None

    def _data_gradient(self, dy, planes, dya, wa):
        g = self._g
        if self.wtp is not None and (g.wp_frozen if self.w.fixed else g.wp_table) is None:
            fn.weight_planes(self.w.data, transposed=True, cols=self.wtp.shape[2] * 32, out=self.wtp, math=self.math,
                             w_absmax=wa)
        elif self.wtp is None and not (g.wt_frozen is not None if self.w.fixed else g.wt_batched):
            fn.weight_transpose(self.w.data, out=self.wt, copy=self.wh)
        if self.sc_pair is not None and self.stride == 2 and self._compact_shortcut(dy, planes, dya, wa):
            return
        dx, acc = self.x.grad_target()
        sa = self.x.sc_compact
        assert sa is None or (not acc and not self.guard_fb and self.bn_bwd_node is not None)
        bn = self.bn_bwd_node
        bn_bwd, bn_dya = None, None
        if bn is not None:
            bn_bwd = (bn.x.data, bn.scale, bn.shift, bn.mean, bn.rstd, bn.relu, bn.bwd_sums[0])
            bn.bwd_sums_ready = True
            if bn.dx_planes:
                bn_dya = self._g.scalar(bn.am_dyin)
        if self.guard_fb:
            w3 = self._w3(True)
            fn.conv2d_dgrad(dy, self.wt if w3 is None else None, self.x.shape, self.stride, self.pad, self.dil, out=dx,
                            accumulate=acc, bn_bwd=bn_bwd, wt_planes=w3, math="bf16x3", wt_shape=self.wt_shape)
            if bn_dya is not None:
                fn.absmax(dx, out=bn_dya)
            self._g.guard["calls"] += 1
            self._g.guard["calls_total"] += 1
            return
        fn.conv2d_dgrad(dy, self.wt, self.x.shape, self.stride, self.pad, self.dil, out=dx, accumulate=acc,
                        bn_bwd=bn_bwd, wt_planes=self.wtp, math=self.math, dy_absmax=dya, w_absmax=wa,
                        bn_dy_absmax=bn_dya, dy_planes=planes, wt_shape=self.wt_shape, strided_addend=sa)

    def _compact_shortcut(self, dy, planes, dya, wa):
        conv1, x, g = self.sc_pair, self.x, self._g
        if (not SC_COMPACT or self.guard_fb or conv1.guard_fb or planes or x._gw or not conv1.out._gw or g.sc_compact_buf is None
                or not fn.conv2d_dgrad_addend_route(x.shape, conv1.out.shape[3], conv1.out.grad_planes)):
            return False
        N, H, W, C = x.shape
        Ho, Wo = dy.shape[1], dy.shape[2]
        dxc = g.sc_compact_buf[:N * Ho * Wo * C].view(N, Ho, Wo, C)
        fn.conv2d_dgrad(dy, self.wt, dxc.shape, 1, 0, 1, out=dxc, wt_planes=self.wtp, math=self.math, dy_absmax=dya, w_absmax=wa,
                        wt_shape=self.wt_shape)
        x.sc_compact = dxc
        return True


class BilinearConcatConv(Node):

    def __init__(self, g, inputs, name, num_filter, kernel, pad, target_hw, theta, init="maxdim"):
        N = inputs[0].shape[0]
        kh, kw = fn._hw(kernel)
        self.pad = fn._hw(pad)
        assert (kh - 1) // 2 == self.pad[0] and (kw - 1) // 2 == self.pad[1], "needs a 'same' convolution"
        Ht, Wt = target_hw
        self.inputs = inputs
        self.theta = theta
        self.offsets = np.cumsum([0] + [t.shape[3] for t in inputs]).tolist()
        Cin = self.offsets[-1]
        self.cout, self.kh, self.kw = num_filter, kh, kw
        self.w = g.param(name + "_weight", (num_filter, kh, kw, Cin), conv_weight_init(init, Cin))
        self.w.logical, self.w.kind = (num_filter, Cin, kh, kw), "conv"
        T = num_filter * kh * kw
        Tp = fn.padc(T)
        self.T = T
# ... 289 lines not shown
```

### dspnet_amd/functional.py

```python
import ctypes
import os

import numpy as np
import torch

from . import _lib
from ._lib import check

_c = ctypes
_vp = _c.c_void_p
_i = _c.c_int
_ll = _c.c_longlong
_f = _c.c_float
_sz = _c.c_size_t

_lib.register({
    "dspn_conv2d_split_workspace_bytes": (_sz, [_ll, _i]),
    "dspn_conv2d_forward_f32": (_i, [_vp, _vp, _vp, _vp, _vp, _i, _i, _i, _i, _i, _i, _i, _i, _i, _i, _i, _i, _i,
                                     _ll, _i, _i, _i, _vp, _sz, _vp]),
    "dspn_conv2d_forward_bn_f32": (_i, [_vp, _vp, _vp, _i, _vp, _vp, _vp, _vp, _vp, _i, _i, _i, _i, _i, _i, _i, _i, _i, _i, _i, _i,
                                        _i, _ll, _i, _i, _i, _vp, _sz, _vp, _i, _vp, _vp, _vp, _sz, _vp]),
    "dspn_absmax_f32": (_i, [_vp, _ll, _i, _vp, _vp, _i, _vp, _vp]),
    "dspn_absmax_batch_f32": (_i, [_vp, _i, _ll, _vp]),
    "dspn_conv2d_weight_planes_f32": (_i, [_vp, _vp, _vp, _i, _i, _i, _i, _i, _vp, _vp]),
    "dspn_conv2d_weight_planes_tiles": (_ll, [_i, _i, _i, _i, _i]),
    "dspn_conv2d_weight_planes_batch_f32": (_i, [_vp, _i, _ll, _vp]),
    "dspn_conv2d_stats_layout": (_i, [_ll, _i, _c.POINTER(_c.c_int)]),
    "dspn_bn_stats_from_tiles_f32": (_i, [_vp, _i, _i, _ll, _i, _f, _vp, _vp, _vp, _vp, _vp, _vp, _vp, _i, _vp, _vp, _vp, _vp, _sz, _vp]),
    "dspn_bn_tiles_workspace_bytes": (_sz, [_i, _i]),
    "dspn_conv2d_wgrad_bn_f32": (_i, [_vp, _vp, _vp, _i, _vp, _vp, _i, _i, _i, _i, _i, _i, _i, _i, _i, _i, _i, _i, _i, _i,
                                      _i, _i, _vp, _vp, _vp, _sz, _vp]),
    "dspn_conv2d_wgrad_splits": (_i, [_i, _i, _i, _i, _i, _i, _i, _i]),
    "dspn_conv2d_wgrad_slabs_f32": (_i, [_vp, _vp, _vp, _i, _vp, _vp, _sz, _i, _i, _i, _i, _i, _i, _i, _i, _i, _i, _i, _i,
                                         _i, _i, _i, _vp, _vp, _vp]),
    "dspn_conv2d_slab_reduce_batch_f32": (_i, [_vp, _i, _ll, _vp]),
    "dspn_conv2d_weight_transpose_batch_f32": (_i, [_vp, _i, _ll, _vp]),
    "dspn_conv2d_weight_transpose_tiles": (_ll, [_i, _i, _i, _i]),
    "dspn_conv2d_weight_transpose_f32": (_i, [_vp, _vp, _i, _i, _i, _i, _vp]),
    "dspn_conv2d_dgrad_f32": (_i, [_vp, _vp, _vp, _i, _i, _i, _i, _i, _i, _i, _i, _i, _i, _i, _i, _i, _i, _i, _vp,
                                   _sz, _vp]),
    "dspn_conv2d_dgrad_bn_tiles": (_i, [_i, _i, _i, _i, _i]),
    "dspn_conv2d_dgrad_bn_f32": (_i, [_vp, _vp, _vp, _vp, _i, _i, _i, _i, _i, _i, _i, _i, _i, _i, _i, _i, _i, _i, _i,
                                      _vp, _vp, _vp, _vp, _vp, _i, _vp, _sz, _vp, _i, _vp, _vp, _vp, _sz, _vp]),
    "dspn_conv2d_dgrad_bn_sadd_f32": (_i, [_vp, _vp, _vp, _vp, _i, _i, _i, _i, _i, _i, _i, _i, _i, _i, _i, _i, _i, _i, _i,
                                           _vp, _vp, _vp, _vp, _vp, _i, _vp, _sz, _vp, _i, _vp, _vp, _vp, _sz, _vp, _i, _i, _vp]),
    "dspn_conv2d_dgrad_bn_sadd_route_f32": (_i, [_i, _i, _i, _i, _i, _i]),
    "dspn_bn_backward_from_sums_f32": (_i, [_vp, _vp, _vp, _vp, _vp, _vp, _vp, _vp, _i, _vp, _vp, _vp, _ll, _i, _i, _i,
                                            _vp, _vp, _vp, _vp, _i, _vp, _sz, _vp]),
    "dspn_bn_discard_parked": (_i, [_vp]),
    "dspn_absmin_rows_batch_f32": (_i, [_vp, _i, _ll, _vp]),
    "dspn_tile_minmax_f32": (_i, [_vp, _ll, _i, _i, _vp, _vp]),
    "dspn_conv2d_input_sum_grad_workspace_bytes": (_sz, [_i, _i, _i, _i, _i]),
    "dspn_conv2d_input_sum_grad_f32": (_i, [_vp, _vp, _vp, _i, _i, _i, _i, _i, _i, _i, _i, _i, _i, _i, _i, _i, _i,
                                            _vp, _sz, _vp]),
    "dspn_conv2d_wgrad_workspace_bytes": (_sz, [_i, _i, _i, _i, _i, _i, _i]),
    "dspn_conv2d_wgrad_f32": (_i, [_vp, _vp, _vp, _i, _i, _i, _i, _i, _i, _i, _i, _i, _i, _i, _i, _i, _i, _i,
                                   _vp, _sz, _vp]),
    "dspn_bn_workspace_bytes": (_sz, [_ll, _i]),
    "dspn_bn_stats_f32": (_i, [_vp, _ll, _i, _f, _vp, _vp, _vp, _vp, _vp, _vp, _vp, _sz, _vp]),
    "dspn_bn_apply_f32": (_i, [_vp, _vp, _vp, _vp, _ll, _i, _i, _vp, _vp]),
    "dspn_bn_apply_planes_f32": (_i, [_vp, _vp, _vp, _vp, _ll, _i, _i, _vp, _vp]),
    "dspn_absmax_affine_bound_f32": (_i, [_vp, _vp, _i, _vp, _vp, _vp]),
    "dspn_bn_backward_f32": (_i, [_vp, _vp, _vp, _vp, _vp, _vp, _vp, _vp, _vp, _vp, _ll, _i, _i, _i, _vp, _vp, _sz,
                                  _vp]),
    "dspn_add_f32": (_i, [_vp, _vp, _vp, _ll, _vp]),
    "dspn_relu_backward_f32": (_i, [_vp, _vp, _vp, _ll, _i, _vp]),
    "dspn_fill_f32": (_i, [_vp, _f, _ll, _vp]),
    "dspn_relu_backward_colsum_f32": (_i, [_vp, _vp, _vp, _ll, _i, _i, _vp, _vp, _vp, _sz, _vp]),
    "dspn_colsum_workspace_bytes": (_sz, [_ll, _i]),
    "dspn_colsum_f32": (_i, [_vp, _ll, _i, _i, _vp, _vp, _sz, _vp]),
    "dspn_nchw_to_nhwc_f32": (_i, [_vp, _vp, _i, _i, _i, _i, _i, _vp]),
    "dspn_nhwc_to_nchw_f32": (_i, [_vp, _vp, _i, _i, _i, _i, _i, _vp]),
    "dspn_copy_block_f32": (_i, [_vp, _vp, _i, _ll, _i, _ll, _i, _i, _ll, _i, _i, _i, _vp]),
    "dspn_copy_block_batch_f32": (_i, [_vp, _i, _ll, _vp]),
    "dspn_transpose_bnc_f32": (_i, [_vp, _vp, _i, _i, _i, _vp]),
    "dspn_avgpool2d_forward_f32": (_i, [_vp, _vp, _i, _i, _i, _i, _i, _i, _i, _i, _i, _vp]),
    "dspn_avgpool2d_backward_f32": (_i, [_vp, _vp, _i, _i, _i, _i, _i, _i, _i, _i, _i, _i, _vp]),
    "dspn_bilinear_backward_workspace_bytes": (_sz, [_i, _i, _i, _i]),
    "dspn_bilinear_backward_ws_f32": (_i, [_vp, _vp, _i, _i, _i, _i, _i, _i, _i, _i, _vp, _sz, _vp]),
# ... 6 lines not shown
    "dspn_maxpool_forward_f32": (_i, [_vp, _vp, _vp, _i, _i, _i, _i, _i, _i, _i, _i, _i, _vp]),
    "dspn_maxpool_forward_bn_f32": (_i, [_vp, _vp, _vp, _i, _vp, _vp, _i, _i, _i, _i, _i, _i, _i, _i, _i, _vp, _vp]),
    "dspn_maxpool_backward_argmax_f32": (_i, [_vp, _vp, _vp, _i, _i, _i, _i, _i, _i, _i, _i, _i, _vp]),
    "dspn_bn_backward_maxpool_f32": (_i, [_vp, _vp, _vp, _vp, _vp, _i, _i, _i, _i, _i, _i, _i, _i, _i, _vp, _vp, _vp, _vp, _vp,
                                          _vp, _i, _vp, _vp, _sz, _vp]),
    "dspn_maxpool_backward_f32": (_i, [_vp, _vp, _vp, _vp, _i, _i, _i, _i, _i, _i, _i, _i, _i, _vp]),
    "dspn_avgpool_forward_f32": (_i, [_vp, _vp, _i, _i, _i, _i, _i, _i, _i, _vp]),
    "dspn_avgpool_backward_f32": (_i, [_vp, _vp, _i, _i, _i, _i, _i, _i, _i, _i, _vp]),
    "dspn_bilinear_forward_f32": (_i, [_vp, _vp, _i, _i, _i, _i, _i, _i, _i, _i, _vp]),
    "dspn_bilinear_forward_acc_f32": (_i, [_vp, _vp, _i, _i, _i, _i, _i, _i, _i, _i, _vp]),
    "dspn_bilinear_backward_f32": (_i, [_vp, _vp, _i, _i, _i, _i, _i, _i, _i, _i, _vp]),
    "dspn_affine_sampler_forward_f32": (_i, [_vp, _vp, _vp, _vp, _vp, _i, _vp, _vp, _i, _i, _i, _i, _vp]),
    "dspn_affine_sampler_backward_data_f32": (_i, [_vp, _vp, _vp, _i, _i, _i, _i, _i, _i, _i, _i, _i, _vp]),
    "dspn_affine_sampler_theta_workspace_bytes": (_sz, [_i, _i, _i]),
    "dspn_affine_sampler_backward_theta_f32": (_i, [_vp, _vp, _vp, _vp, _vp, _i, _vp, _vp, _i, _i, _i, _i, _vp, _i,
                                                    _vp, _sz, _vp]),
    "dspn_affine_sampler_backward_data_theta_f32": (_i, [_vp, _vp, _vp, _vp, _i, _i, _i, _i, _i, _i, _i, _i, _i, _vp, _sz, _vp,
                                                         _vp, _sz, _vp]),
    "dspn_affine_sampler_theta_rows": (_ll, [_i, _i, _i, _i]),
    "dspn_affine_sampler_backward_workspace_bytes": (_sz, [_i, _i, _i, _i, _i]),
    "dspn_affine_sampler_theta_reduce_workspace_bytes": (_sz, [_ll]),
    "dspn_affine_sampler_theta_reduce": (_i, [_vp, _ll, _vp, _i, _vp, _sz, _vp]),
    "dspn_softmax_output_f32": (_i, [_vp, _vp, _vp, _vp, _ll, _i, _i, _f, _f, _vp, _vp]),
    "dspn_count_f32": (_i, [_vp, _ll, _i, _f, _vp, _vp]),
    "dspn_smooth_l1_forward_f32": (_i, [_vp, _vp, _vp, _vp, _ll, _vp]),
    "dspn_smooth_l1_backward_f32": (_i, [_vp, _vp, _vp, _vp, _ll, _f, _vp, _vp]),
    "dspn_cross_entropy_sum_f32": (_i, [_vp, _vp, _ll, _i, _i, _f, _f, _vp, _vp]),
    "dspn_sum_f32": (_i, [_vp, _ll, _vp, _vp]),
    "dspn_sgd_momentum_f32": (_i, [_vp, _vp, _vp, _ll, _f, _f, _f, _f, _vp]),
    "dspn_sgd_momentum_segments_f32": (_i, [_vp, _vp, _vp, _vp, _i, _ll, _f, _f, _f, _f, _vp]),
})


for _name in ("dspn_conv2d_forward_bn", "dspn_conv2d_dgrad_bn", "dspn_conv2d_dgrad_bn_sadd", "dspn_conv2d_wgrad_bn", "dspn_conv2d_wgrad_slabs",
              "dspn_conv2d_input_sum_grad", "dspn_bn_stats", "dspn_bn_apply", "dspn_bn_backward",
              "dspn_bn_backward_from_sums", "dspn_add", "dspn_relu_backward", "dspn_relu_backward_colsum", "dspn_colsum",
              "dspn_nchw_to_nhwc", "dspn_copy_block", "dspn_tap_sum", "dspn_tap_spread", "dspn_maxpool_forward", "dspn_maxpool_forward_bn",
              "dspn_maxpool_backward_argmax", "dspn_maxpool_backward", "dspn_avgpool_forward", "dspn_avgpool_backward",
              "dspn_avgpool2d_forward", "dspn_avgpool2d_backward", "dspn_softmax_output", "dspn_affine_sampler_forward",
              "dspn_affine_sampler_backward_data", "dspn_affine_sampler_backward_theta",
              "dspn_affine_sampler_backward_data_theta"):
    _lib.register({_name + "_bf16": _lib.SIGNATURES[_name + "_f32"]})
_lib.register({
    "dspn_conv2d_weight_prepare_bf16": (_i, [_vp, _vp, _vp, _i, _i, _i, _i, _vp]),
    "dspn_conv2d_weight_prepare_batch_bf16": (_i, [_vp, _i, _ll, _vp]),
    "dspn_copy_block_bf16_f32": _lib.SIGNATURES["dspn_copy_block_f32"],
    "dspn_copy_block_f32_bf16": _lib.SIGNATURES["dspn_copy_block_f32"],
})
_lib.register({
    "dspn_box_rank_select_f32": (_i, [_vp, _i, _i, _i, _vp, _i, _vp, _vp, _vp, _vp]),
    "dspn_box_rank_select_u16": (_i, [_vp, _i, _i, _i, _vp, _i, _vp, _vp, _vp, _vp]),
    "dspn_distance_boxes_workspace_bytes": (_sz, [_i]),
    "dspn_distance_boxes_f32": (_i, [_vp, _i, _i, _i, _i, _f, _i, _i, _vp, _vp, _vp, _vp, _sz, _vp]),
})
_lib.register({
    "dspn_tensor_stats_chunk_elems": (_i, []),
    "dspn_tensor_stats_workspace_bytes": (_sz, [_i, _ll]),
    "dspn_tensor_stats": (_i, [_vp, _i, _ll, _vp, _vp, _sz, _vp]),
})
_lib.register({
    "dspn_render_chunk_rows": (_i, []),
    "dspn_render_classmap_f32": (_i, [_vp, _i, _i, _i, _i, _i, _vp, _vp, _vp, _i, _i, _vp, _i, _i, _i, _i, _vp]),
    "dspn_render_labels_f32": (_i, [_vp, _i, _i, _i, _vp, _vp, _vp, _i, _i, _vp, _i, _i, _i, _i, _vp]),
    "dspn_render_data_f32": (_i, [_vp, _i, _i, _i, _c.POINTER(_c.c_int), _c.POINTER(_c.c_double), _vp, _i, _i, _i, _i, _vp]),
    "dspn_render_check_draw_rows": (_i, [_vp, _i, _vp, _i]),
    "dspn_render_draw_list_u8": (_i, [_vp, _i, _i, _i, _i, _i, _i, _i, _vp, _i, _vp, _vp, _vp]),
})
# ... 315 lines not shown
    Cout, R, S, Cin = w.shape
    dtype = out.dtype if out is not None else (dtype or torch.float32)
    Kp = padc(Cout, dtype) if out is None else out.shape[3]
    if out is None:
        out = empty(Cin, R, S, Kp, device=w.device, dtype=dtype)
    if dtype == torch.bfloat16:
        check(L().dspn_conv2d_weight_prepare_bf16(ptr(w), ptr(copy), ptr(out), Cout, R * S, Cin, Kp, stream()),
              "weight_prepare")
    else:
        check(L().dspn_conv2d_weight_transpose_f32(ptr(w), ptr(out), Cout, R * S, Cin, Kp, stream()),
              "weight_transpose")
    return out


def weight_cast(w):
    return w.to(torch.bfloat16)


def conv_dgrad_bn_tiles(x_shape, stride):
    N, H, W, C = x_shape
    return L().dspn_conv2d_dgrad_bn_tiles(N, H, W, C, stride)


MATH_DY_PLANES = 0x200
MATH_X_PLANES = 0x400
BN_SUMS_PLANES, BN_SUMS_FINALIZE_ONLY, BN_SUMS_APPLY_ONLY, BN_SUMS_PARKED = 1, 2, 4, 8


def conv2d_dgrad_addend_route(x_shape, ldy, dy_planes):
    N, H, W, C = x_shape
    return bool(L().dspn_conv2d_dgrad_bn_sadd_route_f32(N, H, W, C, ldy, int(bool(dy_planes))))


def conv2d_dgrad(dy, wt, x_shape, stride=1, pad=0, dil=1, out=None, accumulate=False, bn_bwd=None, wt_planes=None,
                 math=None, dy_absmax=None, w_absmax=None, bn_dy_absmax=None, dy_planes=False, wt_shape=None,
                 strided_addend=None):
    N, H, W, Cx = x_shape
    Cin, R, S, ldy = wt.shape if wt is not None else wt_shape
    assert dy.shape[3] == ldy, (dy.shape, (Cin, R, S, ldy))
    assert wt is not None or wt_planes is not None
    math = _math_code(math)
    if math == 3 and dy.dtype == torch.float32:
        assert wt_planes is None or w_absmax is not None, "f16x2 planes come with the magnitude block they were cut by"
        assert not dy_planes or dy_absmax is not None, "piece-plane gradients come with the magnitude block they were cut by"
        dy_absmax = absmax(dy) if dy_absmax is None else dy_absmax
        w_absmax = absmax(wt) if w_absmax is None else w_absmax
    else:
        dy_absmax = w_absmax = None
    if needs_planes(dy.dtype, ldy, math):
        if wt_planes is None:
            wt_planes = weight_planes(wt, math=math, w_absmax=w_absmax)
    else:
        wt_planes = None
    Ho, Wo = dy.shape[1], dy.shape[2]
    if out is None:
        out = (zeros if Cx != Cin else empty)(N, H, W, Cx, device=dy.device, dtype=dy.dtype)
    assert (wt is None or wt.dtype == dy.dtype) and dy.dtype == out.dtype, (dy.dtype, out.dtype)
    ws = workspace(L().dspn_conv2d_split_workspace_bytes(N * H * W, Cin), dy.device, "split")
    ph, pw = _hw(pad)
    bx, bsc, bsh, bmu, brs, brelu, bsums = bn_bwd if bn_bwd is not None else (None, None, None, None, None, False, None)
    args = (ptr(dy), ptr(wt), ptr(wt_planes), ptr(out), N, H, W, Cin, ldy, R, S, stride, ph, pw,
            dil, Ho, Wo, out.shape[3], int(accumulate), ptr(bx), ptr(bsc), ptr(bsh), ptr(bmu),
            ptr(brs), int(brelu), ptr(bsums), 0 if bsums is None else bsums.numel() * 4,
            ptr(bn_dy_absmax), math | (MATH_DY_PLANES if dy_planes else 0), ptr(dy_absmax),
            ptr(w_absmax), ptr(ws), ws.numel())
    if strided_addend is not None:
        sa = strided_addend
        assert sa.dtype == out.dtype and sa.is_contiguous() and sa.shape == (N, (H + 1) // 2, (W + 1) // 2, Cin), (sa.shape, x_shape)
        check(_f("dspn_conv2d_dgrad_bn_sadd", dy)(*args, ptr(sa), sa.shape[1], sa.shape[2], stream()), "conv2d_dgrad")
    else:
        check(_f("dspn_conv2d_dgrad_bn", dy)(*args, stream()), "conv2d_dgrad")
    return out


def _wgrad_absmax(x, dy, in_affine, math, x_absmax, dy_absmax):
    if math == 3 and x.dtype == torch.float32:
        return (absmax(x, in_affine) if x_absmax is None else x_absmax, absmax(dy) if dy_absmax is None else dy_absmax)
    return None, None


def conv2d_wgrad(x, dy, w_shape, stride=1, pad=0, dil=1, out=None, accumulate=False, in_affine=None, math=None,
                 x_absmax=None, dy_absmax=None, dy_planes=False, x_planes=False):
    N, H, W, Cin = x.shape
    Cout, R, S, Cw = w_shape
    assert Cw == Cin
    Ho, Wo, ldy = dy.shape[1], dy.shape[2], dy.shape[3]
    if out is None:
        out = empty(Cout, R, S, Cin, device=x.device)
    nbytes = L().dspn_conv2d_wgrad_workspace_bytes(N, Ho, Wo, Cin, Cout, R, S)
    ws = workspace(nbytes, x.device, "wgrad")
    ph, pw = _hw(pad)
    sc, sh, arelu = in_affine if in_affine is not None else (None, None, False)
    assert x.dtype == dy.dtype and out.dtype == torch.float32
    math = _math_code(math)
    assert not x_planes or (x_absmax is not None and in_affine is None)
    x_absmax, dy_absmax = _wgrad_absmax(x, dy, in_affine, math, x_absmax, dy_absmax)
    check(_f("dspn_conv2d_wgrad_bn", x)(ptr(x), ptr(sc), ptr(sh), int(arelu), ptr(dy), ptr(out), N, H, W, Cin, Cout, ldy,
                                       R, S, stride, ph, pw, dil, Ho, Wo, int(accumulate),
                                       math | (MATH_DY_PLANES if dy_planes else 0) | (MATH_X_PLANES if x_planes else 0),
                                       ptr(x_absmax), ptr(dy_absmax), ptr(ws), ws.numel(), stream()), "conv2d_wgrad")
    return out

# ... 137 lines not shown
    check(_f("dspn_bn_backward", x)(ptr(x), ptr(scale), ptr(shift), ptr(dy), ptr(mean), ptr(rstd), ptr(gamma), ptr(dx),
                                   ptr(dgamma), ptr(dbeta), rows, C, int(relu), int(accumulate), ptr(dx_absmax), ptr(ws),
                                   ws.numel(), stream()), "bn_backward")
    return dx, dgamma, dbeta


def bn_backward_maxpool(x, scale, shift, dy_pool, argmax, k, stride, pad, mean, rstd, gamma, relu=False, dx=None, dgamma=None,
                        dbeta=None, dx_absmax=None):
    N, H, W, C = x.shape
    assert x.dtype == dy_pool.dtype == torch.float32 and argmax.dtype == torch.uint8 and argmax.shape == dy_pool.shape
    dx, dgamma, dbeta = _bn_outputs(x, gamma, dx, dgamma, dbeta)
    ws = workspace(L().dspn_bn_workspace_bytes(N * H * W, C), x.device, "bn")
    check(L().dspn_bn_backward_maxpool_f32(ptr(x), ptr(scale), ptr(shift), ptr(dy_pool), ptr(argmax), N, H, W, C, k, stride, pad,
                                           dy_pool.shape[1], dy_pool.shape[2], ptr(mean), ptr(rstd), ptr(gamma), ptr(dx),
                                           ptr(dgamma), ptr(dbeta), int(relu), ptr(dx_absmax), ptr(ws), ws.numel(), stream()),
          "bn_backward_maxpool")
    return dx, dgamma, dbeta


def bn_backward_from_sums(x, scale, shift, dy, mean, rstd, gamma, sums, tiles, relu=False, dx=None, dgamma=None,
                          dbeta=None, accumulate=False, dx_absmax=None, dy_absmax=None, x_chan_minmax=None, dx_planes=False,
                          dx_absmin=None, phase=0, park=False, workspace=None):
    assert phase in (0, 1, 2) and (not park or phase == 1)
    C = x.shape[-1]
    rows = _rows(x)
    dx, dgamma, dbeta = _bn_outputs(x, gamma, dx, dgamma, dbeta)
    if dx is None:
        assert phase == 0 and not park and not dx_planes, "dx=NO_OUTPUT is a whole call"
        phase = 1
    flags = ((BN_SUMS_PLANES if dx_planes else 0) | {0: 0, 1: BN_SUMS_FINALIZE_ONLY, 2: BN_SUMS_APPLY_ONLY}[phase] |
             (BN_SUMS_PARKED if park else 0))
    if workspace is None:
        workspace = _scratch(12 * C + L().dspn_bn_tiles_workspace_bytes(tiles, C), x.device, "bn_from_sums")
    assert dy.dtype == x.dtype
    check(_f("dspn_bn_backward_from_sums", x)(ptr(x), ptr(scale), ptr(shift), ptr(dy), ptr(mean), ptr(rstd), ptr(gamma),
                                             ptr(sums), tiles, ptr(dx), ptr(dgamma), ptr(dbeta), rows, C, int(relu),
                                             int(accumulate), ptr(dx_absmax), ptr(dx_absmin), ptr(dy_absmax), ptr(x_chan_minmax),
                                             flags, ptr(workspace), workspace.numel(), stream()),
          "bn_backward_from_sums")
    return dx, dgamma, dbeta


def bn_from_sums_workspace(tiles, C, device):
    return torch.empty(12 * C + L().dspn_bn_tiles_workspace_bytes(tiles, C), dtype=torch.uint8, device=device)


def bn_discard_parked(stream_handle):
    return L().dspn_bn_discard_parked(stream_handle)


def add(a, b, out=None):
    out = torch.empty_like(a) if out is None else out
    assert a.dtype == b.dtype == out.dtype
    check(_f("dspn_add", a)(ptr(a), ptr(b), ptr(out), a.numel(), stream()), "add")
    return out


def relu_backward(y, dy, dx=None, accumulate=False):
    dx = torch.empty_like(y) if dx is None else dx
    assert y.dtype == dy.dtype == dx.dtype
    check(_f("dspn_relu_backward", y)(ptr(y), ptr(dy), ptr(dx), y.numel(), int(accumulate), stream()),
          "relu_backward")
    return dx


def relu_backward_colsum(y, dy, C, dx=None, out=None, dx_absmax=None):
    dx = dy if dx is None else dx
# ... 557 lines not shown
```

### dspnet_amd/graph_plan.py

```python
import os

import torch

from . import engine as E, functional as fn


class WiringIndex:

    def __init__(self, nodes):
        self.readers, self.writer = {}, {}
        for i, n in enumerate(nodes):
            for t in n.wiring.outputs:
                self.writer[id(t)] = i
            for k, t in n.wiring.reads:
                self.readers.setdefault(id(t), []).append((i, k))

    def reader_nodes(self, t, skip=()):
        return {i for i, k in self.readers.get(id(t), ()) if k not in skip}

    def first_reader(self, t):
        return min(self.reader_nodes(t), default=None)

    def repoint(self, i, node, attr, old, new):
        node.wiring.reads[node.wiring.reads.index((attr, old))] = (attr, new)
        self.readers[id(old)].remove((i, attr))
        self.readers[id(new)] = sorted(self.readers[id(new)] + [(i, attr)])


def plan(g):
    index = WiringIndex(g.nodes)
    resolve_auto_deferred(g, index)
    side_sync(g, index)
    if os.environ.get("DSPN_X_PLANES", "1") != "0":
        input_planes(g)
    bn_backward_fusion(g, index)
    gradient_magnitudes(g, index)
    if os.environ.get("DSPN_DY_PLANES", "1") != "0":
        gradient_planes(g, index)
    shortcut_compaction(g, index)


def resolve_auto_deferred(g, index):
    def applies_in_loader(m, k, t):
        return (isinstance(m, E.Conv) and k == "x" and not m.tap_expand and not
                (E.MATERIALISE_MULTITAP_INPUT_BF16 and t.dtype == torch.bfloat16 and m.w.shape[1] * m.w.shape[2] > 1))

    for n in g.nodes:
        if not isinstance(n, E.BatchNorm) or n.defer_apply != "auto":
            continue
        rs = [(g.nodes[i], k) for i, k in index.readers.get(id(n.out), ()) if k != "x_raw"]
        if rs and all(applies_in_loader(m, k, n.out) for m, k in rs):
            n.defer_apply = True
            continue
        n.defer_apply = False
        n.out.affine_src = None
        n.out.data = fn.zeros(*n.out.shape, device=g.device, dtype=n.out.dtype)
        for c in n.conv_consumers:
            index.repoint(g.nodes.index(c), c, "x_raw", c.x_raw, c.x)
            c.x_raw, c.in_affine = c.x, None
        n.mat_consumers = list(n.conv_consumers)
        n.conv_consumers = []


def bn_backward_fusion(g, index):
    for n in g.nodes:
        if not isinstance(n, E.BatchNorm) or not n.out.requires_grad:
            continue
        cons = n.conv_consumers if n.defer_apply else n.mat_consumers
        if not cons or (not n.defer_apply and index.reader_nodes(n.out) != {g.nodes.index(c) for c in cons}):
            continue
        last = min(cons, key=g.nodes.index)
        if last.stride not in (1, 2) or (last.stride == 2 and last.dil != 1) or last.x.shape[3] % 4 != 0:
# ... 28 lines not shown
        if not (prod is not None and prod.out is x and index.reader_nodes(x, skip=("x_raw",)) == {idx} and x.requires_grad
                and x.dtype == torch.float32 and n.completes_x_grad and n.tile_stats is not None):
            continue
        if (prod.tap_expand or prod.relu or prod.b is not None or prod.residual is not None or prod.input_sum_grad is not None
                or prod.am_dy is None or x.shape[3] != prod.cout or prod.cout % 32 != 0 or prod.out_minmax is None
                or gatherer[id(n)].math != "f16x2"):
            continue
        n.dx_planes = True
        n.x_ext = fn.zeros(2, x.shape[3], device=g.device)
        n.am_dyin = g.new_scalar(backward=True)


def shortcut_compaction(g, index):
    if g.math != "f16x2" or g.device.type != "cuda":
        return
    largest = 0
    for n in g.nodes:
        if not isinstance(n, E.BatchNorm) or not n.out.requires_grad or n.out.dtype != torch.float32:
            continue
        readers = sorted(index.reader_nodes(n.out))
        if len(readers) != 2 or not all(isinstance(g.nodes[i], E.Conv) and g.nodes[i].x is n.out for i in readers):
            continue
        conv1, sc = g.nodes[readers[0]], g.nodes[readers[1]]
        one_by_one = lambda c: c.w.shape[1:3] == (1, 1) and c.pad == (0, 0) and c.dil == 1 and not c.tap_expand
        if not (one_by_one(conv1) and conv1.stride == 1 and conv1.bn_bwd_node is n and conv1.math == "f16x2"
                and one_by_one(sc) and sc.stride == 2 and sc.math == "f16x2" and sc.input_sum_grad is None
                and conv1.input_sum_grad is None and n.out.shape[3] == conv1.w.shape[3]):
            continue
        conv1.sc_pair, sc.sc_pair = sc, conv1
        N, H, W, C = n.out.shape
        largest = max(largest, N * ((H + 1) // 2) * ((W + 1) // 2) * C)
    if largest:
        g.sc_compact_buf = fn.zeros(largest, device=g.device)


def input_planes(g):
    if g.math != "f16x2" or g.device.type != "cuda":
        return
    for n in g.nodes:
        if not isinstance(n, E.BatchNorm) or n.defer_apply is not True or n.tile_stats is None:
            continue
        x = n.x
        if (x.dtype != torch.float32 or x.shape[3] % 32 != 0 or x.data is None
                or x.producer is None or x.producer.out_minmax is None):
            continue
        cons = [c for c in n.conv_consumers if c.math == "f16x2" and c.wp is not None and c.x_raw is x]
        reads = sum(c.w.shape[1] * c.w.shape[2] * ((c.cout + 127) // 128) for c in cons)
        if reads < E.X_PLANES_MIN_READS:
            continue
        n.planes = fn.zeros(*x.shape, device=g.device)
        for c in cons:
            c.x_planes_bn = n


def side_sync(g, index):
    plan = g.side_plan
    g.side_fwd_events, g.side_fwd_waits = {}, {}
    if plan is None:
        return
    first, last = plan["first"], plan["last"]
    cuda = g.side_segment is not None
    refs = [g._node_tensors(n) for n in g.nodes]
    holders = {}
    for i, ts in enumerate(refs):
        for t in ts:
            holders.setdefault(id(t), []).append(i)
# ... 40 lines not shown
```

### include/dspn_nn.h

```cpp
#ifndef DSPN_NN_H_
#define DSPN_NN_H_

#include <stddef.h>

#ifdef __cplusplus
extern "C" {
#endif


size_t dspn_conv2d_split_workspace_bytes(long long out_pixels, int Cout);
#define DSPN_MATH_FP32 0
#define DSPN_MATH_BF16 1
#define DSPN_MATH_F32_BF16X3 2
#define DSPN_MATH_F32_F16X2 3
#define DSPN_MATH_UNSCALED_OK 0x100
#define DSPN_MATH_DY_PLANES 0x200
#define DSPN_MATH_X_PLANES 0x400

int dspn_conv2d_forward_f32(const float *x, const float *w, const float *bias, const float *residual, float *y,
                            int N, int H, int W, int Cin, int Cout, int R, int S,
                            int stride, int pad_h, int pad_w, int dil, int Ho, int Wo,
                            long long y_batch_stride, int y_ldc, int relu, int accumulate,
                            void *workspace, size_t workspace_bytes, void *stream);

// ... 6 lines not shown
                               const float *x_absmax, const float *w_absmax,
                               void *workspace, size_t workspace_bytes, void *stream);
int dspn_conv2d_stats_layout(long long out_pixels, int Cout, int *tile_rows);

int dspn_conv2d_weight_planes_f32(const float *w, void *planes, void *planes_t, int Cout, int taps, int Cin, int cols_t,
                                  int pieces, const float *w_absmax, void *stream);
long long dspn_conv2d_weight_planes_tiles(int Cout, int taps, int Cin, int cols_t, int with_transposed);
int dspn_conv2d_weight_planes_batch_f32(const void *table, int n, long long total_tiles, void *stream);

int dspn_conv2d_weight_transpose_f32(const float *w, float *wt, int Cout, int taps, int Cin,
                                     int Cout_pad, void *stream);
long long dspn_conv2d_weight_transpose_tiles(int Cout, int taps, int Cin, int Cout_pad);
int dspn_conv2d_weight_transpose_batch_f32(const void *table, int n, long long total_tiles, void *stream);

int dspn_conv2d_dgrad_f32(const float *dy, const float *wt, float *dx,
                          int N, int H, int W, int Cin, int ldy, int R, int S,
                          int stride, int pad_h, int pad_w, int dil, int Ho, int Wo, int dx_ldc,
                          int accumulate, void *workspace, size_t workspace_bytes, void *stream);
int dspn_conv2d_dgrad_bn_tiles(int N, int H, int W, int Cin, int stride);
int dspn_conv2d_dgrad_bn_f32(const float *dy, const float *wt, const void *wt_planes, float *dx, int N, int H, int W, int Cin, int ldy,
                             int R, int S, int stride, int pad_h, int pad_w, int dil, int Ho, int Wo, int dx_ldc,
                             int accumulate, const float *bn_x, const float *bn_scale, const float *bn_shift,
                             const float *bn_mean, const float *bn_rstd, int bn_relu, float *bn_sums,
                             size_t bn_sums_bytes, float *bn_dy_absmax, int math, const float *dy_absmax, const float *w_absmax,
                             void *workspace, size_t workspace_bytes, void *stream);
int dspn_conv2d_dgrad_bn_sadd_f32(const float *dy, const float *wt, const void *wt_planes, float *dx, int N, int H, int W, int Cin, int ldy,
                                  int R, int S, int stride, int pad_h, int pad_w, int dil, int Ho, int Wo, int dx_ldc,
                                  int accumulate, const float *bn_x, const float *bn_scale, const float *bn_shift,
                                  const float *bn_mean, const float *bn_rstd, int bn_relu, float *bn_sums,
                                  size_t bn_sums_bytes, float *bn_dy_absmax, int math, const float *dy_absmax, const float *w_absmax,
                                  void *workspace, size_t workspace_bytes, const float *strided_addend, int addend_h, int addend_w,
                                  void *stream);
int dspn_conv2d_dgrad_bn_sadd_route_f32(int N, int H, int W, int Cin, int ldy, int dy_planes);

size_t dspn_conv2d_input_sum_grad_workspace_bytes(int Ho, int Wo, int ldy, int R, int S);
int dspn_conv2d_input_sum_grad_f32(const float *dy, const float *w, float *out, int N, int H, int W,
                                   int Cin, int Cout, int ldy, int R, int S, int stride, int pad_h, int pad_w, int dil,
                                   int Ho, int Wo, void *workspace, size_t workspace_bytes, void *stream);

size_t dspn_conv2d_wgrad_workspace_bytes(int N, int Ho, int Wo, int Cin, int Cout, int R, int S);

int dspn_conv2d_wgrad_f32(const float *x, const float *dy, float *dw,
                          int N, int H, int W, int Cin, int Cout, int ldy, int R, int S,
                          int stride, int pad_h, int pad_w, int dil, int Ho, int Wo, int accumulate,
                          void *workspace, size_t workspace_bytes, void *stream);
int dspn_conv2d_wgrad_bn_f32(const float *x, const float *in_scale, const float *in_shift, int in_relu,
                             const float *dy, float *dw, int N, int H, int W, int Cin, int Cout, int ldy,
                             int R, int S, int stride, int pad_h, int pad_w, int dil, int Ho, int Wo,
                             int accumulate, int math, const float *x_absmax, const float *dy_absmax,
                             void *workspace, size_t workspace_bytes, void *stream);

int dspn_conv2d_wgrad_splits(int N, int Ho, int Wo, int Cin, int Cout, int R, int S, int stride);
int dspn_conv2d_wgrad_slabs_f32(const float *x, const float *in_scale, const float *in_shift, int in_relu,
                                const float *dy, float *slabs, size_t slabs_bytes, int N, int H, int W, int Cin,
                                int Cout, int ldy, int R, int S, int stride, int pad_h, int pad_w, int dil, int Ho,
                                int Wo, int math, const float *x_absmax, const float *dy_absmax, void *stream);
int dspn_conv2d_slab_reduce_batch_f32(const void *table, int n, long long total4, void *stream);

#define DSPN_ABSMAX_SLOTS 64
int dspn_absmax_f32(const float *x, long long rows, int C, const float *scale, const float *shift, int relu,
                    float *out_dev, void *stream);
int dspn_absmin_rows_batch_f32(const void *table, int n, long long total_rows, void *stream);
int dspn_tile_minmax_f32(const float *x, long long rows, int C, int tile_rows, float *minmax, void *stream);
int dspn_absmax_batch_f32(const void *table, int n, long long total_chunks, void *stream);
int dspn_absmax_affine_bound_f32(const float *scale, const float *shift, int C, const float *x_absmax_dev, float *out_dev,
                                 void *stream);

#ifdef DSPN_BF16_ELEMENT
typedef DSPN_BF16_ELEMENT dspn_bf16;
#else
typedef unsigned short dspn_bf16;
#endif
int dspn_conv2d_forward_bn_bf16(const dspn_bf16 *x, const float *in_scale, const float *in_shift, int in_relu,
                                const dspn_bf16 *w, const void *w_planes_unused, const float *bias, const dspn_bf16 *residual, dspn_bf16 *y,
                                int N, int H, int W, int Cin, int Cout, int R, int S,
                                int stride, int pad_h, int pad_w, int dil, int Ho, int Wo,
                                long long y_batch_stride, int y_ldc, int relu, int accumulate,
                                float *out_stats, size_t out_stats_bytes, float *out_minmax_unused, int math,
                                const float *absmax_unused_a, const float *absmax_unused_b,
                                void *workspace, size_t workspace_bytes, void *stream);
int dspn_conv2d_dgrad_bn_bf16(const dspn_bf16 *dy, const dspn_bf16 *wt, const void *wt_planes_unused, dspn_bf16 *dx, int N, int H, int W, int Cin,
                              int ldy, int R, int S, int stride, int pad_h, int pad_w, int dil, int Ho, int Wo,
                              int dx_ldc, int accumulate, const dspn_bf16 *bn_x, const float *bn_scale,
                              const float *bn_shift, const float *bn_mean, const float *bn_rstd, int bn_relu,
                              float *bn_sums, size_t bn_sums_bytes, float *bn_dy_absmax_unused, int math,
                              const float *absmax_unused_a, const float *absmax_unused_b, void *workspace,
                              size_t workspace_bytes, void *stream);
int dspn_conv2d_dgrad_bn_sadd_bf16(const dspn_bf16 *dy, const dspn_bf16 *wt, const void *wt_planes_unused, dspn_bf16 *dx, int N, int H, int W,
                                   int Cin, int ldy, int R, int S, int stride, int pad_h, int pad_w, int dil, int Ho, int Wo,
                                   int dx_ldc, int accumulate, const dspn_bf16 *bn_x, const float *bn_scale,
                                   const float *bn_shift, const float *bn_mean, const float *bn_rstd, int bn_relu,
                                   float *bn_sums, size_t bn_sums_bytes, float *bn_dy_absmax_unused, int math,
                                   const float *absmax_unused_a, const float *absmax_unused_b, void *workspace,
                                   size_t workspace_bytes, const dspn_bf16 *strided_addend, int addend_h, int addend_w,
                                   void *stream);
int dspn_conv2d_wgrad_bn_bf16(const dspn_bf16 *x, const float *in_scale, const float *in_shift, int in_relu,
                              const dspn_bf16 *dy, float *dw, int N, int H, int W, int Cin, int Cout, int ldy,
                              int R, int S, int stride, int pad_h, int pad_w, int dil, int Ho, int Wo,
                              int accumulate, int math, const float *absmax_unused_a, const float *absmax_unused_b,
                              void *workspace, size_t workspace_bytes, void *stream);
int dspn_conv2d_wgrad_slabs_bf16(const dspn_bf16 *x, const float *in_scale, const float *in_shift, int in_relu,
                                 const dspn_bf16 *dy, float *slabs, size_t slabs_bytes, int N, int H, int W, int Cin,
                                 int Cout, int ldy, int R, int S, int stride, int pad_h, int pad_w, int dil, int Ho,
                                 int Wo, int math, const float *absmax_unused_a, const float *absmax_unused_b, void *stream);
int dspn_conv2d_input_sum_grad_bf16(const dspn_bf16 *dy, const float *w, float *out, int N, int H, int W,
                                    int Cin, int Cout, int ldy, int R, int S, int stride, int pad_h, int pad_w, int dil,
                                    int Ho, int Wo, void *workspace, size_t workspace_bytes, void *stream);
int dspn_conv2d_weight_prepare_bf16(const float *w, dspn_bf16 *wh, dspn_bf16 *wt, int Cout, int taps, int Cin,
                                    int Cout_pad, void *stream);
int dspn_conv2d_weight_prepare_batch_bf16(const void *table, int n, long long total_tiles, void *stream);


size_t dspn_bn_workspace_bytes(long long rows, int C);

int dspn_bn_stats_f32(const float *x, long long rows, int C, float eps, const float *gamma,
                      const float *beta, float *mean, float *rstd, float *scale, float *shift,
                      void *workspace, size_t workspace_bytes, void *stream);

int dspn_bn_stats_from_tiles_f32(const float *tile_stats, int tiles, int tile_rows, long long rows, int C, float eps,
                                 const float *gamma, const float *beta, float *mean, float *rstd, float *scale,
                                 float *shift, const float *tile_minmax, int relu, float *out_absmax, float *out_absmin,
                                 float *out_chan_minmax, void *workspace, size_t workspace_bytes, void *stream);
size_t dspn_bn_tiles_workspace_bytes(int tiles, int C);

#define DSPN_BN_TRACK 1
#define DSPN_BN_GLOBAL 2
typedef struct dspn_bn_moving {
  float *moving_mean;
// ... 227 lines not shown
```

Baseline: 974.6 images/s.

## Recompute 1x1 dgrad to fuse BatchNorm-backward apply into its epilogue

```diff
diff --git a/dspnet_amd/csrc/bn_final_job.h b/dspnet_amd/csrc/bn_final_job.h
--- a/dspnet_amd/csrc/bn_final_job.h
+++ b/dspnet_amd/csrc/bn_final_job.h
@@ -17,6 +17,7 @@
 
 void bn_job_defer(hipStream_t s, const BnFinalJob &job);
 bool bn_job_take(hipStream_t s, BnFinalJob *job);
+void bn_jobs_run(hipStream_t s);
 
 __device__ __forceinline__ void bn_final_channel(const int c, const int C, const double S, const double SS, const double inv_rows,
                                                  const float *__restrict__ mean, const float *__restrict__ rstd, const float *__restrict__ gamma,
@@ -41,6 +42,11 @@
     if (bf > 0.f) atomicMax(dx_bound + (c & 63), __float_as_uint(bf));
     if (dx_bound_min && bf > 0.f && bf < INFINITY) atomicMin(dx_bound_min, __float_as_uint(bf));
   }
+}
+
+__device__ __forceinline__ float bn_apply_element(const float a, const float g, const float c1, const float x, const float c0) {
+  const float ag = a * g;
+  return fmaf(c1, x, ag) + c0;
 }
 
 __device__ __forceinline__ void bn_final_job_run(const BnFinalJob &j, const int b, void *smem) {
diff --git a/dspnet_amd/csrc/conv.hip b/dspnet_amd/csrc/conv.hip
--- a/dspnet_amd/csrc/conv.hip
+++ b/dspnet_amd/csrc/conv.hip
@@ -1686,6 +1686,26 @@
     g.sadd_bytes = (unsigned)((long long)sizeof(st_t) * g.N * g.sadd_h * g.sadd_w * g.Cout);
     if (g.probe) return 0;
   }
+  if (g.bn_recompute) {
+    const char *who = g.bn_recompute == 1 ? DSPN_FN_NAME(dspn_conv2d_dgrad_bn_sums) : DSPN_FN_NAME(dspn_conv2d_dgrad_bn_apply);
+    if (kHalf) return dspn::fail(DSPN_ERR_ARG_, "%s: float tensors only", who);
+    if (g.bf16 != 3) return dspn::fail(DSPN_ERR_ARG_, "%s: needs DSPN_MATH_F32_F16X2", who);
+    if (splits > 1 || (g.dense && nblk < 192 && nk >= 16))
+      return dspn::fail(DSPN_ERR_ARG_, "%s: cannot be combined with split-K (%lld workgroups, %d k-steps: a shape that is split)", who, nblk, nk);
+    if (!g.a_planes) return dspn::fail(DSPN_ERR_ARG_, "%s: needs dy as piece planes (DSPN_MATH_DY_PLANES)", who);
+    if (g.sadd || g.stats || g.in_scale || residual || (g.flags & (1 | 2 | 8)))
+      return dspn::fail(DSPN_ERR_ARG_, "%s: a plain data gradient only (no strided addend, statistics, input affine, bias, ReLU or residual)", who);
+    if (!g.dense || g.ldc != g.Cout) return dspn::fail(DSPN_ERR_ARG_, "%s: needs a dense dx (dx_ldc %d, Cin %d)", who, g.ldc, g.Cout);
+    if (g.TR * g.TS != 1 || g.ish != 1 || g.isw != 1 || g.ioh != 0 || g.iow != 0)
+      return dspn::fail(DSPN_ERR_ARG_, "%s: a 1 x 1 / stride-1 / pad-0 convolution only", who);
+    if ((g.bn_recompute == 1) != (g.bn_sums != nullptr) || (g.bn_recompute == 1 && (g.flags & 4)))
+      return dspn::fail(DSPN_ERR_ARG_, "%s: the sums pass writes the tables and adds to nothing; the apply pass reads the coefficients", who);
+    if (!((route.tile == dspn::conv::WideTile::P128x128 || route.tile == dspn::conv::WideTile::P128x256) &&
+          route.loop == dspn::conv::WideLoop::Spanning))
+      return dspn::fail(DSPN_ERR_ARG_, "%s: no kernel on this route (it needs N H W %% 128 == 0 and the plane-fed 128-row tiles on the "
+                        "tile-spanning loop)", who);
+    if (g.probe) return 0;
+  }
   if (route) return dspn::conv::launch_wide(route, in, w, bias, out, g, s, residual);
   const int rc = cfg == 0 && eight ? launch_nt<4, 2, 1, 2>(in, w, bias, out, g, s, splits, per, ws.ptr, residual)
                  : cfg == 0        ? launch_nt<2, 2, 2, 2>(in, w, bias, out, g, s, splits, per, ws.ptr, residual)
@@ -2020,6 +2040,7 @@
 
 struct BnBwd { const st_t *x; const float *scale, *shift, *mean, *rstd; int relu; float *sums; float *dy_absmax; };
 struct StridedAddend { const st_t *p; int h, w, probe; };
+struct BnRecompute { int mode; const float *coef; float *dx_absmax; int probe; };
 
 static int dgrad_tiles(int N, int H, int W, int Cin, int stride, int *per_class ) {
   int total = 0;
@@ -2037,8 +2058,8 @@
 static int conv2d_dgrad_one(int math, OpScales scales, const st_t *dy, const st_t *wt, const void *wt_planes, st_t *dx, int N, int H, int W,
                           int Cin, int ldy, int R, int S, int stride, int pad_h, int pad_w, int dil, int Ho,
                           int Wo, int dx_ldc, int accumulate, BnBwd bn, void *workspace, size_t workspace_bytes,
-                          void *stream, StridedAddend sa = StridedAddend{nullptr, 0, 0, 0}) {
-  DSPN_REQUIRE(dy && (wt || wt_planes) && dx, "conv2d_dgrad: null pointer");
+                          void *stream, StridedAddend sa = StridedAddend{nullptr, 0, 0, 0}, BnRecompute rc2 = BnRecompute{0, nullptr, nullptr, 0}) {
+  DSPN_REQUIRE(dy && (wt || wt_planes) && (dx || rc2.mode == 1), "conv2d_dgrad: null pointer");
   DSPN_REQUIRE(ldy % kEPC == 0, "conv2d_dgrad: dy channel stride must be a multiple of %d", kEPC);
   DSPN_REQUIRE(stride == 1 || (stride == 2 && dil == 1), "conv2d_dgrad: stride 1, or stride 2 with dilation 1");
   DSPN_REQUIRE(N > 0 && H > 0 && W > 0 && Cin > 0 && R > 0 && S > 0, "conv2d_dgrad: bad geometry");
@@ -2057,7 +2078,10 @@
   g.bn_relu = bn.relu; g.bn_sums = bn.sums; g.bn_tile_base = 0;
   g.bn_dy_absmax = (bn.sums && !kHalf && math == DSPN_MATH_F32_F16X2) ? reinterpret_cast<unsigned *>(bn.dy_absmax) : nullptr;
   g.a_planes = scales.a_planes;
-  g.sadd = sa.p; g.sadd_h = sa.h; g.sadd_w = sa.w; g.probe = sa.probe;
+  g.sadd = sa.p; g.sadd_h = sa.h; g.sadd_w = sa.w; g.probe = sa.probe | rc2.probe;
+  g.bn_recompute = rc2.mode; g.bn_coef = rc2.coef;
+  if (rc2.mode == 2) g.bn_dy_absmax = reinterpret_cast<unsigned *>(rc2.dx_absmax);
+  if (rc2.mode == 1) g.bn_dy_absmax = nullptr;
   int class_tiles[4] = {0, 0, 0, 0};
   if (bn.sums) dgrad_tiles(N, H, W, Cin, stride, class_tiles);
   hipStream_t s = (hipStream_t)stream;
@@ -2106,8 +2130,17 @@
                              const st_t *bn_x, const float *bn_scale, const float *bn_shift, const float *bn_mean,
                              const float *bn_rstd, int bn_relu, float *bn_sums, size_t bn_sums_bytes, float *bn_dy_absmax,
                              int math, const float *dy_absmax, const float *w_absmax, void *workspace, size_t workspace_bytes,
-                             void *stream, StridedAddend sa) {
+                             void *stream, StridedAddend sa, BnRecompute rc2 = BnRecompute{0, nullptr, nullptr, 0}) {
   DSPN_REQUIRE(N > 0 && Ho > 0 && Wo > 0 && ldy > 0, "conv2d_dgrad: bad geometry");
+  if (rc2.mode) {
+    const char *who = rc2.mode == 1 ? DSPN_FN_NAME(dspn_conv2d_dgrad_bn_sums) : DSPN_FN_NAME(dspn_conv2d_dgrad_bn_apply);
+    DSPN_REQUIRE(!dspn::kHalf, "%s: float tensors only (the bfloat16 build has no such kernel)", who);
+    DSPN_REQUIRE(R == 1 && S == 1 && stride == 1 && pad_h == 0 && pad_w == 0 && Ho == H && Wo == W,
+                 "%s: a 1 x 1 / stride-1 / pad-0 convolution only", who);
+    DSPN_REQUIRE((dx_ldc <= 0 || dx_ldc == Cin), "%s: needs a dense dx (dx_ldc %d, Cin %d)", who, dx_ldc, Cin);
+    DSPN_REQUIRE(Cin > 0 && Cin % 4 == 0, "%s: Cin %% 4 == 0", who);
+    DSPN_REQUIRE(batch_chunk(N, (long long)sizeof(st_t) * Ho * Wo * ldy) == N, "%s: dy of 2 GiB or more", who);
+  }
   if (sa.p) {
     constexpr const char *who = DSPN_FN_NAME(dspn_conv2d_dgrad_bn_sadd);
     DSPN_REQUIRE(stride == 1 && !accumulate, "%s: the strided addend goes with a stride-1 data gradient that is the only writer of dx (no accumulate)", who);
@@ -2133,12 +2166,47 @@
     const int rc = conv2d_dgrad_one(math, OpScales{dy_absmax, w_absmax, dy_planes}, dy + (long long)n0 * Ho * Wo * ldy, wt, wt_planes, dx + (long long)n0 * H * W * ldc, n, H,
                                     W, Cin, ldy, R, S, stride, pad_h, pad_w, dil, Ho, Wo, dx_ldc, accumulate,
                                     BnBwd{bn_x, bn_scale, bn_shift, bn_mean, bn_rstd, bn_relu, bn_sums, bn_dy_absmax}, workspace,
-                                    workspace_bytes, stream, sa);
+                                    workspace_bytes, stream, sa, rc2);
     if (rc) return rc;
   }
   return 0;
 }
 extern "C" {
+int DSPN_FN(dspn_conv2d_dgrad_bn_sums)(const st_t *dy, const st_t *wt, const void *wt_planes, st_t *dx, int N, int H, int W,
+                             int Cin, int ldy, int R, int S, int stride, int pad_h, int pad_w, int dil, int Ho,
+                             int Wo, int dx_ldc, int accumulate,
+                             const st_t *bn_x, const float *bn_scale, const float *bn_shift, const float *bn_mean,
+                             const float *bn_rstd, int bn_relu, float *bn_sums, size_t bn_sums_bytes, float *bn_dy_absmax,
+                             int math, const float *dy_absmax, const float *w_absmax, void *workspace, size_t workspace_bytes,
+                             void *stream) {
+  constexpr const char *who = DSPN_FN_NAME(dspn_conv2d_dgrad_bn_sums);
+  DSPN_REQUIRE(!dx && !accumulate && !bn_dy_absmax, "%s: stores no dx (dx == NULL, accumulate 0, no bn_dy_absmax); dspn_conv2d_dgrad_bn is the call that does", who);
+  DSPN_REQUIRE(bn_sums, "%s: bn_sums missing", who);
+  return conv2d_dgrad_bn_impl(dy, wt, wt_planes, nullptr, N, H, W, Cin, ldy, R, S, stride, pad_h, pad_w, dil, Ho, Wo, dx_ldc, 0, bn_x,
+                              bn_scale, bn_shift, bn_mean, bn_rstd, bn_relu, bn_sums, bn_sums_bytes, nullptr, math, dy_absmax,
+                              w_absmax, workspace, workspace_bytes, stream, StridedAddend{nullptr, 0, 0, 0}, BnRecompute{1, nullptr, nullptr, 0});
+}
+int DSPN_FN(dspn_conv2d_dgrad_bn_apply)(const st_t *dy, const st_t *wt, const void *wt_planes, st_t *dx, int N, int H, int W,
+                             int Cin, int ldy, int R, int S, int stride, int pad_h, int pad_w, int dil, int Ho,
+                             int Wo, int dx_ldc, int accumulate,
+                             const st_t *bn_x, const float *bn_scale, const float *bn_shift, int bn_relu, float *dx_absmax,
+                             int math, const float *dy_absmax, const float *w_absmax, const void *bn_workspace,
+                             size_t bn_workspace_bytes, void *stream) {
+  constexpr const char *who = DSPN_FN_NAME(dspn_conv2d_dgrad_bn_apply);
+  DSPN_REQUIRE(dx && bn_x && bn_workspace && (!bn_relu || (bn_scale && bn_shift)), "%s: null pointer", who);
+  if (Cin > 0 && bn_workspace_bytes < sizeof(float) * 3 * (size_t)Cin)
+    return dspn::fail(DSPN_ERR_WORKSPACE_, "%s: the BatchNorm workspace holds 3 * Cin coefficients", who);
+  const int rc = conv2d_dgrad_bn_impl(dy, wt, wt_planes, dx, N, H, W, Cin, ldy, R, S, stride, pad_h, pad_w, dil, Ho, Wo, dx_ldc, accumulate,
+                                      bn_x, bn_scale, bn_shift, nullptr, nullptr, bn_relu, nullptr, 0, nullptr, math, dy_absmax, w_absmax,
+                                      nullptr, 0, stream, StridedAddend{nullptr, 0, 0, 0},
+                                      BnRecompute{2, static_cast<const float *>(bn_workspace), dx_absmax, 1});
+  if (rc) return rc;
+  dspn::bn_jobs_run((hipStream_t)stream);
+  return conv2d_dgrad_bn_impl(dy, wt, wt_planes, dx, N, H, W, Cin, ldy, R, S, stride, pad_h, pad_w, dil, Ho, Wo, dx_ldc, accumulate,
+                              bn_x, bn_scale, bn_shift, nullptr, nullptr, bn_relu, nullptr, 0, nullptr, math, dy_absmax, w_absmax,
+                              nullptr, 0, stream, StridedAddend{nullptr, 0, 0, 0},
+                              BnRecompute{2, static_cast<const float *>(bn_workspace), dx_absmax, 0});
+}
 int DSPN_FN(dspn_conv2d_dgrad_bn)(const st_t *dy, const st_t *wt, const void *wt_planes, st_t *dx, int N, int H, int W,
                              int Cin, int ldy, int R, int S, int stride, int pad_h, int pad_w, int dil, int Ho,
                              int Wo, int dx_ldc, int accumulate,
@@ -2171,6 +2239,21 @@
   return conv2d_dgrad_bn_impl(q, nullptr, q, q, N, H, W, Cin, ldy, 1, 1, 1, 0, 0, 1, H, W, Cin, 0, q, q, q, q, q, 1, q,
                               sizeof(float) * 2 * (size_t)tiles * Cin, q, DSPN_MATH_F32_F16X2 | (dy_planes ? DSPN_MATH_DY_PLANES : 0), q, q,
                               nullptr, 0, nullptr, StridedAddend{q, (H + 1) / 2, (W + 1) / 2, 1}) == 0 ? 1 : 0;
+}
+#endif
+
+#ifndef DSPN_HALF
+int dspn_conv2d_dgrad_bn_recompute_route_f32(int N, int H, int W, int Cin, int ldy, int dy_planes) {
+  float *const q = reinterpret_cast<float *>(uintptr_t(256));
+  const int tiles = dgrad_bn_tiles(N, H, W, Cin, 1);
+  if (tiles <= 0 || N <= 0 || ldy <= 0) return 0;
+  const int math = DSPN_MATH_F32_F16X2 | (dy_planes ? DSPN_MATH_DY_PLANES : 0);
+  const StridedAddend none{nullptr, 0, 0, 0};
+  return conv2d_dgrad_bn_impl(q, nullptr, q, nullptr, N, H, W, Cin, ldy, 1, 1, 1, 0, 0, 1, H, W, Cin, 0, q, q, q, q, q, 1, q,
+                              sizeof(float) * 2 * (size_t)tiles * Cin, nullptr, math, q, q, nullptr, 0, nullptr, none,
+                              BnRecompute{1, nullptr, nullptr, 1}) == 0 &&
+         conv2d_dgrad_bn_impl(q, nullptr, q, q, N, H, W, Cin, ldy, 1, 1, 1, 0, 0, 1, H, W, Cin, 1, q, q, q, nullptr, nullptr, 1, nullptr,
+                              0, nullptr, math, q, q, nullptr, 0, nullptr, none, BnRecompute{2, q, q, 1}) == 0 ? 1 : 0;
 }
 #endif
 
diff --git a/dspnet_amd/csrc/conv_geom.h b/dspnet_amd/csrc/conv_geom.h
--- a/dspnet_amd/csrc/conv_geom.h
+++ b/dspnet_amd/csrc/conv_geom.h
@@ -37,6 +37,8 @@
   int sadd_h, sadd_w;
   unsigned sadd_bytes;
   int probe;
+  int bn_recompute;
+  const float *bn_coef;
 };
 
 __device__ __forceinline__ int xcd_remap(int bid, int nblk) {
diff --git a/dspnet_amd/csrc/conv_wide.h b/dspnet_amd/csrc/conv_wide.h
--- a/dspnet_amd/csrc/conv_wide.h
+++ b/dspnet_amd/csrc/conv_wide.h
@@ -226,7 +226,8 @@
 }
 
 #ifndef DSPN_HALF
-template <int WAVES_M, int WAVES_N, int EPI, int RB = 16, int SR = 128, bool CLOSE = false, bool SADD = false>
+template <int WAVES_M, int WAVES_N, int EPI, int RB = 16, int SR = 128, bool CLOSE = false, bool SADD = false,
+          bool SUMS_ONLY = false, bool APPLY = false>
 __device__ __forceinline__ void direct_epilogue(const ConvGeom &g, char *exch, f32x16 (&acc)[2][2], const float inv_a, const float inv_b, const int m0,
                                                 const int n0, const int M, const int tid, const int wave,
                                                 const float *__restrict__ bias, float *__restrict__ out,
@@ -248,7 +249,9 @@
   int col[TN];
   unsigned cbyte[TN];
   bool cv[TN];
+  static_assert(!(SUMS_ONLY || APPLY) || (EPI == 2 && !SADD && !(SUMS_ONLY && APPLY)), "the two passes of the recomputed data gradient: BatchNorm-backward epilogue, one at a time");
   float bv[TN], bsc[TN], bsh[TN], bmu[TN], brs[TN];
+  float ka[TN], kc1[TN], kc0[TN];
 #pragma unroll
   for (int j = 0; j < TN; ++j) {
     col[j] = n0 + wn + j * 32 + lc;
@@ -256,8 +259,10 @@
     cbyte[j] = cv[j] ? (unsigned)col[j] * 4u : kOOB;
     bv[j] = (has_bias && cv[j]) ? bias[col[j]] : 0.f;
     bsc[j] = bsh[j] = bmu[j] = brs[j] = 0.f;
+    ka[j] = kc1[j] = kc0[j] = 0.f;
     if (EPI == 2 && cv[j]) {
-      bmu[j] = g.bn_mean[col[j]]; brs[j] = g.bn_rstd[col[j]];
+      if constexpr (APPLY) { ka[j] = g.bn_coef[col[j]]; kc1[j] = g.bn_coef[g.Cout + col[j]]; kc0[j] = g.bn_coef[2 * g.Cout + col[j]]; }
+      else { bmu[j] = g.bn_mean[col[j]]; brs[j] = g.bn_rstd[col[j]]; }
       if (g.bn_relu) { bsc[j] = g.bn_scale[col[j]]; bsh[j] = g.bn_shift[col[j]]; }
     }
   }
@@ -309,10 +314,12 @@
           const unsigned off = rb + cbyte[j];
           if constexpr (SADD)
             rq[s_][rr][j] = (rr & 1) ? 0.f : __builtin_bit_cast(float, __builtin_amdgcn_raw_buffer_load_b32(rs_s, (int)(sa_off[j] + (unsigned)(rr >> 1) * pitch), 0, 0));
+          else if constexpr (SUMS_ONLY)
+            rq[s_][rr][j] = 0.f;
           else
           rq[s_][rr][j] = addsrc ? __builtin_bit_cast(float, __builtin_amdgcn_raw_buffer_load_b32(rs_a, (int)off, 0, 0)) : 0.f;
           xq[s_][rr][j] = __builtin_bit_cast(float, __builtin_amdgcn_raw_buffer_load_b32(rs_x, (int)off, 0, 0));
-          oq[s_][rr][j] = both ? __builtin_bit_cast(float, __builtin_amdgcn_raw_buffer_load_b32(rs_o, (int)off, 0, 0)) : 0.f;
+          oq[s_][rr][j] = (both && !SUMS_ONLY && !APPLY) ? __builtin_bit_cast(float, __builtin_amdgcn_raw_buffer_load_b32(rs_o, (int)off, 0, 0)) : 0.f;
         }
       }
     };
@@ -328,15 +335,25 @@
 #pragma unroll
         for (int j = 0; j < TN; ++j) {
           float v = acc[i][j][r] * inv_a * inv_b + bv[j];
+          if constexpr (APPLY) {
+            v += 0.f;
+            const float xv = xq[s_][rr][j];
+            const float gd = (!g.bn_relu || fmaf(xv, bsc[j], bsh[j]) > 0.f) ? v : 0.f;
+            float o = dspn::bn_apply_element(ka[j], gd, kc1[j], xv, kc0[j]);
+            if (accum) o += rq[s_][rr][j];
+            __builtin_amdgcn_raw_buffer_store_b32(__builtin_bit_cast(unsigned, o), rs_o, (int)(rb + cbyte[j]), 0, 0);
+            gmx = fmaxf(gmx, fabsf(o));
+          } else {
           v += rq[s_][rr][j];
           if (both) v += oq[s_][rr][j];
           if (relu) v = v > 0.f ? v : 0.f;
-          __builtin_amdgcn_raw_buffer_store_b32(__builtin_bit_cast(unsigned, v), rs_o, (int)(rb + cbyte[j]), 0, 0);
+          if constexpr (!SUMS_ONLY) __builtin_amdgcn_raw_buffer_store_b32(__builtin_bit_cast(unsigned, v), rs_o, (int)(rb + cbyte[j]), 0, 0);
           const float xv = xq[s_][rr][j];
           const float gd = (!g.bn_relu || fmaf(xv, bsc[j], bsh[j]) > 0.f) ? v : 0.f;
           gs[j] += gd;
           gss[j] += gd * ((xv - bmu[j]) * brs[j]);
-          gmx = fmaxf(gmx, fabsf(v));
+          if constexpr (!SUMS_ONLY) gmx = fmaxf(gmx, fabsf(v));
+          }
         }
       }
     }
@@ -403,7 +420,7 @@
   }
   if constexpr (EPI == 0) gmx_all = fmaxf(gmx_all, gmx);
   if constexpr (EPI == 2) gmx_all = fmaxf(gmx_all, gmx);
-  if constexpr (EPI != 0) {
+  if constexpr (EPI != 0 && !APPLY) {
     float *red = reinterpret_cast<float *>(exch);
     float *red2 = red + PARTS * BN * 4;
     const bool mmx = EPI == 1 && g.minmax != nullptr;
@@ -481,7 +498,7 @@
     }
 }
 
-template <int WAVES_M, int WAVES_N, int STAGES, int EPI, int SR = 128, bool XT = false, bool SADD = false>
+template <int WAVES_M, int WAVES_N, int STAGES, int EPI, int SR = 128, bool XT = false, bool SADD = false, int BNR = 0>
 __global__ __launch_bounds__(WAVES_M * WAVES_N * 64, 2) void conv_ntw_kernel(
     const st_t *__restrict__ in, const st_t *__restrict__ wgt, const float *__restrict__ bias,
     st_t *__restrict__ out, const ConvGeom g, const int m_tiles, const int n_tiles,
@@ -499,6 +516,7 @@
   static_assert(BM % SR == 0, "BatchNorm tables are per SR rows");
   static_assert(!XT || !kHalf, "the tile-spanning loop: float build");
   static_assert(!SADD || (XT && EPI == 2 && SR == 128), "the strided addend: tile-spanning loop, BatchNorm-backward sums, 128-row tables");
+  static_assert(BNR == 0 || (XT && EPI == 2 && SR == 128 && !SADD && BNR <= 2), "the recomputed data gradient: tile-spanning loop, BatchNorm-backward epilogue, 128-row tables");
   extern __shared__ __attribute__((aligned(1024))) char wsm[];
 
 #ifdef DSPN_ABLATE
@@ -674,7 +692,7 @@
       zero_acc();
       int last_slot = 0;
       for (int kt = 0; kt < nk; ++kt) {
-        if (!first && kt < D) asm volatile("s_waitcnt vmcnt(63)" ::: "memory");
+        if (BNR != 1 && !first && kt < D) asm volatile("s_waitcnt vmcnt(63)" ::: "memory");
         else asm volatile("s_waitcnt vmcnt(%0)" ::"n"((D - 1) * NI) : "memory");
         __builtin_amdgcn_s_barrier();
         if (kt + D < nk) {
@@ -692,14 +710,14 @@
       char *exch = wsm + STAGES * STG;
       if constexpr (EXCH_IN_RING) {
         exch = wsm + last_slot * STG;
-        if constexpr (EPI != 0) { asm volatile("s_waitcnt lgkmcnt(0)" ::: "memory"); __builtin_amdgcn_s_barrier(); }
-      }
-      if constexpr (!kHalf) direct_epilogue<WAVES_M, WAVES_N, EPI, (EPI == 2 ? 4 : 8), SR, false, SADD>(g, exch, acc, inv_a, inv_b, m0, n0, M, tid, wave, bias, out, residual, gmx_all);
+        if constexpr (EPI != 0 && BNR != 2) { asm volatile("s_waitcnt lgkmcnt(0)" ::: "memory"); __builtin_amdgcn_s_barrier(); }
+      }
+      if constexpr (!kHalf) direct_epilogue<WAVES_M, WAVES_N, EPI, (EPI == 2 ? 4 : 8), SR, false, SADD, BNR == 1, BNR == 2>(g, exch, acc, inv_a, inv_b, m0, n0, M, tid, wave, bias, out, residual, gmx_all);
       DSPN_STAMP(5);
     }
     DSPN_STAMP_FLUSH;
     asm volatile("s_waitcnt vmcnt(0)" ::: "memory");
-    if constexpr (EPI != 1) {
+    if constexpr (EPI != 1 && BNR != 1) {
       asm volatile("s_waitcnt lgkmcnt(0)" ::: "memory");
       __builtin_amdgcn_s_barrier();
       wide_publish_absmax<NWV>(g, wsm, gmx_all, tid);
@@ -1128,7 +1146,7 @@
 }
 #endif
 
-template <int WAVES_M, int WAVES_N, int STAGES, int EPI, int SR, bool XT, bool SADD = false>
+template <int WAVES_M, int WAVES_N, int STAGES, int EPI, int SR, bool XT, bool SADD = false, int BNR = 0>
 int launch_ntw_impl(const st_t *in, const st_t *w, const float *bias, st_t *out, const ConvGeom &g, hipStream_t s,
                     const st_t *residual) {
   constexpr int BM = WAVES_M * 64, BN = WAVES_N * 64;
@@ -1136,9 +1154,10 @@
   const int mt = (int)((M + BM - 1) / BM), nt = (g.Cout + BN - 1) / BN;
   const size_t lds = XT ? (size_t)STAGES * (BM + BN) * 128 + ((WAVES_M * WAVES_N == 8 || BM == 256) ? 0 : sizeof(float) * 4 * BN * 6)
                         : std::max<size_t>((size_t)STAGES * (BM + BN) * 128, sizeof(float) * BM * (BN + 4));
-  constexpr auto kern = conv_ntw_kernel<WAVES_M, WAVES_N, STAGES, EPI, SR, XT, SADD>;
+  constexpr auto kern = conv_ntw_kernel<WAVES_M, WAVES_N, STAGES, EPI, SR, XT, SADD, BNR>;
   const int grid_x = dspn::persistent_grid<kern>(WAVES_M * WAVES_N * 64, lds, (long long)mt * nt, "conv_ntw",
-                                                 SADD ? "conv_ntw<%d,%d,stages=%d,epi=%d,xt=%d,sadd>" : "conv_ntw<%d,%d,stages=%d,epi=%d,xt=%d>",
+                                                 SADD ? "conv_ntw<%d,%d,stages=%d,epi=%d,xt=%d,sadd>" : BNR == 1 ? "conv_ntw<%d,%d,stages=%d,epi=%d,xt=%d,sums>"
+                                                 : BNR == 2 ? "conv_ntw<%d,%d,stages=%d,epi=%d,xt=%d,apply>" : "conv_ntw<%d,%d,stages=%d,epi=%d,xt=%d>",
                                                  WAVES_M, WAVES_N, STAGES, EPI, (int)XT);
   if (grid_x < 0) return grid_x;
   {
@@ -1151,8 +1170,11 @@
 int launch_ntw_on(const st_t *in, const st_t *w, const float *bias, st_t *out, const ConvGeom &g, hipStream_t s, const st_t *residual) {
   if constexpr (XT && SR == 128 && WAVES_M == 2 && !kHalf) {
     if (g.bn_sums && g.sadd) return launch_ntw_impl<WAVES_M, WAVES_N, STAGES, 2, SR, XT, true>(in, w, bias, out, g, s, residual);
+    if (g.bn_recompute == 1) return launch_ntw_impl<WAVES_M, WAVES_N, STAGES, 2, SR, XT, false, 1>(in, w, bias, out, g, s, residual);
+    if (g.bn_recompute == 2) return launch_ntw_impl<WAVES_M, WAVES_N, STAGES, 2, SR, XT, false, 2>(in, w, bias, out, g, s, residual);
   }
   if (g.sadd) return dspn::fail(DSPN_ERR_ARG_, "conv: this kernel does not take a strided addend");
+  if (g.bn_recompute) return dspn::fail(DSPN_ERR_ARG_, "conv: this kernel has no sums-only / apply form");
   if (g.bn_sums) return launch_ntw_impl<WAVES_M, WAVES_N, STAGES, 2, SR, XT>(in, w, bias, out, g, s, residual);
   if (g.stats) return launch_ntw_impl<WAVES_M, WAVES_N, STAGES, 1, SR, XT>(in, w, bias, out, g, s, residual);
   return launch_ntw_impl<WAVES_M, WAVES_N, STAGES, 0, SR, XT>(in, w, bias, out, g, s, residual);
diff --git a/dspnet_amd/csrc/conv_wide.hip b/dspnet_amd/csrc/conv_wide.hip
--- a/dspnet_amd/csrc/conv_wide.hip
+++ b/dspnet_amd/csrc/conv_wide.hip
@@ -2,6 +2,7 @@
 #include "dspn_store.h"
 #include "dspn_pieces.h"
 #include "conv_geom.h"
+#include "bn_final_job.h"
 #include "../../include/dspn_nn.h"
 #include <algorithm>
 #include <type_traits>
@@ -103,7 +104,7 @@
   return WideTile::P128x128;
 }
 WideRoute wide_route(const ConvGeomT<st_t> &g, long long M, int nk) {
-  WideRoute r{wide_tile_choice(M, g.Cout, nk, (g.stats || g.bn_sums) ? 1 : 0)};
+  WideRoute r{wide_tile_choice(M, g.Cout, nk, (g.stats || g.bn_sums || g.bn_recompute) ? 1 : 0)};
 #ifndef DSPN_HALF
   if (!r) return r;
   if (!g.a_planes)
diff --git a/dspnet_amd/csrc/nn.hip b/dspnet_amd/csrc/nn.hip
--- a/dspnet_amd/csrc/nn.hip
+++ b/dspnet_amd/csrc/nn.hip
@@ -1830,6 +1830,13 @@
   return dspn::check_launch(what);
 }
 
+#ifndef DSPN_HALF
+void dspn::bn_jobs_run(hipStream_t s) {
+  for (dspn::BnFinalJob job; dspn::bn_job_take(s, &job);)
+    hipLaunchKernelGGL(bn_final_job_kernel, dim3(job.blocks), dim3(256), 0, s, job);
+}
+#endif
+
 extern "C" {
 
 #ifndef DSPN_HALF
@@ -2033,7 +2040,7 @@
   DSPN_REQUIRE((flags & ~(DSPN_BN_SUMS_PLANES | DSPN_BN_SUMS_FINALIZE_ONLY | DSPN_BN_SUMS_APPLY_ONLY | DSPN_BN_SUMS_PARKED)) == 0 &&
                    half != (DSPN_BN_SUMS_FINALIZE_ONLY | DSPN_BN_SUMS_APPLY_ONLY) && (!parked || half == DSPN_BN_SUMS_FINALIZE_ONLY),
                "bn_backward_from_sums: flag word = dx_planes | 2 (finalize only, | 8: parked for the next weight gradient) | 4 (apply only)");
-  DSPN_REQUIRE(x && dy && mean && rstd && workspace && tile_sums && tiles > 0, "bn_backward_from_sums: null pointer");
+  DSPN_REQUIRE(x && (dy || half == DSPN_BN_SUMS_FINALIZE_ONLY) && mean && rstd && workspace && tile_sums && tiles > 0, "bn_backward_from_sums: null pointer");
   DSPN_REQUIRE(dx || flags == DSPN_BN_SUMS_FINALIZE_ONLY, "bn_backward_from_sums: dx == NULL needs the finalize-only flag word 2");
   DSPN_REQUIRE(!planes || (!dspn::kHalf && !accumulate && C % 32 == 0 && dx_absmax && dy_absmax && x_chan_minmax &&
                            static_cast<const void *>(dx) != static_cast<const void *>(dy) && static_cast<const void *>(dx) != static_cast<const void *>(x)),
@@ -2046,8 +2053,7 @@
     return dspn::fail(DSPN_ERR_WORKSPACE_, "bn_backward_from_sums: workspace too small (3*C floats)");
   float *coef = static_cast<float *>(workspace);
   if (half == DSPN_BN_SUMS_APPLY_ONLY) {
-    for (dspn::BnFinalJob job; dspn::bn_job_take(S_(stream), &job);)
-      hipLaunchKernelGGL(bn_final_job_kernel, dim3(job.blocks), dim3(256), 0, S_(stream), job);
+    dspn::bn_jobs_run(S_(stream));
   } else {
     BnTiles t{tile_sums, tiles, 1, tiles, nullptr};
     bn_group_tiles<1>(S_(stream), t, C, coef + 3 * (size_t)C, workspace_bytes - coef_bytes);
diff --git a/dspnet_amd/engine.py b/dspnet_amd/engine.py
--- a/dspnet_amd/engine.py
+++ b/dspnet_amd/engine.py
@@ -186,6 +186,7 @@
         self.side_plan = None
         self.slab_tables = {}
         self.sc_compact_buf = None
+        self.bn1_recompute_calls = 0
         self.wt_table = None
         self.wt_batched = False
         self.arena = self.grad_arena = self.mom_arena = None
@@ -658,7 +659,7 @@
             if isinstance(n, BatchNorm):
                 if n._pending is not None:
                     streams.add(n._pending[2])
-                n._pending, n.bwd_sums_ready = None, False
+                n._pending, n.bwd_sums_ready, n._recompute = None, False, None
         for s in streams:
             fn.bn_discard_parked(s)
 
@@ -843,6 +844,7 @@
         self._g = g
         self.completes_x_grad = False
         self._pending = None
+        self._recompute = None
 
     def _moving(self):
         if self.use_global_stats:
@@ -896,17 +898,31 @@
 
     def _from_sums(self, beside, args, kw):
         kw["workspace"] = self.bwd_ws
-        if not beside:
+        if beside:
+            fn.bn_backward_from_sums(*args, phase=1, park=True, **kw)
+            self._pending = (args, kw, fn.stream())
+        elif self._recompute is None:
             fn.bn_backward_from_sums(*args, **kw)
-            return
-        fn.bn_backward_from_sums(*args, phase=1, park=True, **kw)
-        self._pending = (args, kw, fn.stream())
+        else:
+            fn.bn_backward_from_sums(*args, phase=1, **kw)
+            self._apply(args, kw)
+
+    def _apply(self, args, kw):
+        rc, self._recompute = self._recompute, None
+        if rc is None:
+            fn.bn_backward_from_sums(*args, phase=2, **kw)
+            return
+        conv, dy, planes, dya, wa = rc
+        fn.conv2d_dgrad_bn_apply(dy, conv.wt, self.x.data, self.scale, self.shift, self.relu, self.bwd_ws, kw["dx"],
+                                 accumulate=kw["accumulate"], dx_absmax=kw["dx_absmax"], wt_planes=conv.wtp, math=conv.math,
+                                 dy_absmax=dya, w_absmax=wa, dy_planes=planes, wt_shape=conv.wt_shape)
+        self._g.bn1_recompute_calls += 1
 
     def backward(self, beside=False):
         if self._pending is not None:
             args, kw, _ = self._pending
             self._pending = None
-            fn.bn_backward_from_sums(*args, phase=2, **kw)
+            self._apply(args, kw)
             return
         if not self.out._gw:
             return
@@ -962,6 +978,12 @@
 FUSE_CONV_MAGNITUDES = os.environ.get("DSPN_CONV_MAGNITUDES", "1") != "0"
 
 SC_COMPACT = os.environ.get("DSPN_SC_COMPACT", "1") != "0"
+
+BN1_RECOMPUTE = int(os.environ.get("DSPN_BN1_RECOMPUTE", "1"))
+
+
+def bn1_recompute_pays(M, C, K):
+    return K <= 128 and 4 * M * C >= 256 << 20
 
 
 def xa_unavailable(conv):
@@ -1026,6 +1048,7 @@
         self.bn_bwd_node = None
         self._wg_worth = None
         self.guard_fb = False
+        self.bn1_recompute = False
         self.sc_pair = None
         self.wp = self.wtp = None
         if g.device.type == "cuda":
@@ -1257,6 +1280,12 @@
             bn.bwd_sums_ready = True
             if bn.dx_planes:
                 bn_dya = self._g.scalar(bn.am_dyin)
+            if self._recompute_route(bn, planes, acc):
+                fn.conv2d_dgrad(dy, self.wt, self.x.shape, self.stride, self.pad, self.dil, bn_bwd=bn_bwd, wt_planes=self.wtp,
+                                math=self.math, dy_absmax=dya, w_absmax=wa, dy_planes=planes, wt_shape=self.wt_shape,
+                                sums_only=True)
+                bn._recompute = (self, dy, planes, dya, wa)
+                return
         if self.guard_fb:
             w3 = self._w3(True)
             fn.conv2d_dgrad(dy, self.wt if w3 is None else None, self.x.shape, self.stride, self.pad, self.dil, out=dx,
@@ -1269,6 +1298,16 @@
         fn.conv2d_dgrad(dy, self.wt, self.x.shape, self.stride, self.pad, self.dil, out=dx, accumulate=acc,
                         bn_bwd=bn_bwd, wt_planes=self.wtp, math=self.math, dy_absmax=dya, w_absmax=wa,
                         bn_dy_absmax=bn_dya, dy_planes=planes, wt_shape=self.wt_shape, strided_addend=sa)
+
+    def _recompute_route(self, bn, planes, acc):
+        if (not self.bn1_recompute or not BN1_RECOMPUTE or acc or self.guard_fb or not planes or self._g.device.type != "cuda"
+                or not bn.x.requires_grad or bn.pool_grad is not None or bn.dx_planes or bn._pending is not None):
+            return False
+        N, H, W, C = self.x.shape
+        K = self.wt_shape[3]
+        if BN1_RECOMPUTE < 2 and not bn1_recompute_pays(N * H * W, C, K):
+            return False
+        return fn.conv2d_dgrad_recompute_route(self.x.shape, K, planes)
 
     def _compact_shortcut(self, dy, planes, dya, wa):
         conv1, x, g = self.sc_pair, self.x, self._g
diff --git a/dspnet_amd/functional.py b/dspnet_amd/functional.py
--- a/dspnet_amd/functional.py
+++ b/dspnet_amd/functional.py
@@ -45,6 +45,11 @@
     "dspn_conv2d_dgrad_bn_sadd_f32": (_i, [_vp, _vp, _vp, _vp, _i, _i, _i, _i, _i, _i, _i, _i, _i, _i, _i, _i, _i, _i, _i,
                                            _vp, _vp, _vp, _vp, _vp, _i, _vp, _sz, _vp, _i, _vp, _vp, _vp, _sz, _vp, _i, _i, _vp]),
     "dspn_conv2d_dgrad_bn_sadd_route_f32": (_i, [_i, _i, _i, _i, _i, _i]),
+    "dspn_conv2d_dgrad_bn_sums_f32": (_i, [_vp, _vp, _vp, _vp, _i, _i, _i, _i, _i, _i, _i, _i, _i, _i, _i, _i, _i, _i, _i,
+                                           _vp, _vp, _vp, _vp, _vp, _i, _vp, _sz, _vp, _i, _vp, _vp, _vp, _sz, _vp]),
+    "dspn_conv2d_dgrad_bn_apply_f32": (_i, [_vp, _vp, _vp, _vp, _i, _i, _i, _i, _i, _i, _i, _i, _i, _i, _i, _i, _i, _i, _i,
+                                            _vp, _vp, _vp, _i, _vp, _i, _vp, _vp, _vp, _sz, _vp]),
+    "dspn_conv2d_dgrad_bn_recompute_route_f32": (_i, [_i, _i, _i, _i, _i, _i]),
     "dspn_bn_backward_from_sums_f32": (_i, [_vp, _vp, _vp, _vp, _vp, _vp, _vp, _vp, _i, _vp, _vp, _vp, _ll, _i, _i, _i,
                                             _vp, _vp, _vp, _vp, _i, _vp, _sz, _vp]),
     "dspn_bn_discard_parked": (_i, [_vp]),
@@ -117,7 +122,8 @@
 })
 
 
-for _name in ("dspn_conv2d_forward_bn", "dspn_conv2d_dgrad_bn", "dspn_conv2d_dgrad_bn_sadd", "dspn_conv2d_wgrad_bn", "dspn_conv2d_wgrad_slabs",
+for _name in ("dspn_conv2d_forward_bn", "dspn_conv2d_dgrad_bn", "dspn_conv2d_dgrad_bn_sadd", "dspn_conv2d_dgrad_bn_sums",
+              "dspn_conv2d_dgrad_bn_apply", "dspn_conv2d_wgrad_bn", "dspn_conv2d_wgrad_slabs",
               "dspn_conv2d_input_sum_grad", "dspn_bn_stats", "dspn_bn_apply", "dspn_bn_backward",
               "dspn_bn_backward_from_sums", "dspn_add", "dspn_relu_backward", "dspn_relu_backward_colsum", "dspn_colsum",
               "dspn_nchw_to_nhwc", "dspn_copy_block", "dspn_tap_sum", "dspn_tap_spread", "dspn_maxpool_forward", "dspn_maxpool_forward_bn",
@@ -499,9 +505,30 @@
     return bool(L().dspn_conv2d_dgrad_bn_sadd_route_f32(N, H, W, C, ldy, int(bool(dy_planes))))
 
 
+def conv2d_dgrad_recompute_route(x_shape, ldy, dy_planes):
+    N, H, W, C = x_shape
+    return bool(L().dspn_conv2d_dgrad_bn_recompute_route_f32(N, H, W, C, ldy, int(bool(dy_planes))))
+
+
+def conv2d_dgrad_bn_apply(dy, wt, bn_x, scale, shift, relu, bn_workspace, dx, accumulate=False, dx_absmax=None, wt_planes=None,
+                          math=None, dy_absmax=None, w_absmax=None, dy_planes=False, wt_shape=None):
+    N, H, W, C = bn_x.shape
+    Cin, R, S, ldy = wt.shape if wt is not None else wt_shape
+    assert dx.shape == bn_x.shape and dy.shape == (N, H, W, ldy) and Cin == C, (dx.shape, dy.shape, Cin)
+    math = _math_code(math)
+    if not (math == 3 and dy.dtype == torch.float32):
+        dy_absmax = w_absmax = None
+    check(_f("dspn_conv2d_dgrad_bn_apply", dy)(ptr(dy), ptr(wt), ptr(wt_planes), ptr(dx), N, H, W, Cin, ldy, R, S, 1, 0, 0, 1, H, W,
+                                              dx.shape[3], int(accumulate), ptr(bn_x), ptr(scale), ptr(shift), int(relu),
+                                              ptr(dx_absmax), math | (MATH_DY_PLANES if dy_planes else 0), ptr(dy_absmax),
+                                              ptr(w_absmax), ptr(bn_workspace), bn_workspace.numel() * bn_workspace.element_size(),
+                                              stream()), "conv2d_dgrad_bn_apply")
+    return dx
+
+
 def conv2d_dgrad(dy, wt, x_shape, stride=1, pad=0, dil=1, out=None, accumulate=False, bn_bwd=None, wt_planes=None,
                  math=None, dy_absmax=None, w_absmax=None, bn_dy_absmax=None, dy_planes=False, wt_shape=None,
-                 strided_addend=None):
+                 strided_addend=None, sums_only=False):
     N, H, W, Cx = x_shape
     Cin, R, S, ldy = wt.shape if wt is not None else wt_shape
     assert dy.shape[3] == ldy, (dy.shape, (Cin, R, S, ldy))
@@ -520,14 +547,16 @@
     else:
         wt_planes = None
     Ho, Wo = dy.shape[1], dy.shape[2]
-    if out is None:
+    if sums_only:
+        assert out is None and bn_bwd is not None and not accumulate and bn_dy_absmax is None and strided_addend is None
+    elif out is None:
         out = (zeros if Cx != Cin else empty)(N, H, W, Cx, device=dy.device, dtype=dy.dtype)
-    assert (wt is None or wt.dtype == dy.dtype) and dy.dtype == out.dtype, (dy.dtype, out.dtype)
+    assert (wt is None or wt.dtype == dy.dtype) and (sums_only or dy.dtype == out.dtype), (dy.dtype, out)
     ws = workspace(L().dspn_conv2d_split_workspace_bytes(N * H * W, Cin), dy.device, "split")
     ph, pw = _hw(pad)
     bx, bsc, bsh, bmu, brs, brelu, bsums = bn_bwd if bn_bwd is not None else (None, None, None, None, None, False, None)
     args = (ptr(dy), ptr(wt), ptr(wt_planes), ptr(out), N, H, W, Cin, ldy, R, S, stride, ph, pw,
-            dil, Ho, Wo, out.shape[3], int(accumulate), ptr(bx), ptr(bsc), ptr(bsh), ptr(bmu),
+            dil, Ho, Wo, Cx if sums_only else out.shape[3], int(accumulate), ptr(bx), ptr(bsc), ptr(bsh), ptr(bmu),
             ptr(brs), int(brelu), ptr(bsums), 0 if bsums is None else bsums.numel() * 4,
             ptr(bn_dy_absmax), math | (MATH_DY_PLANES if dy_planes else 0), ptr(dy_absmax),
             ptr(w_absmax), ptr(ws), ws.numel())
@@ -535,6 +564,8 @@
         sa = strided_addend
         assert sa.dtype == out.dtype and sa.is_contiguous() and sa.shape == (N, (H + 1) // 2, (W + 1) // 2, Cin), (sa.shape, x_shape)
         check(_f("dspn_conv2d_dgrad_bn_sadd", dy)(*args, ptr(sa), sa.shape[1], sa.shape[2], stream()), "conv2d_dgrad")
+    elif sums_only:
+        check(_f("dspn_conv2d_dgrad_bn_sums", dy)(*args, stream()), "conv2d_dgrad")
     else:
         check(_f("dspn_conv2d_dgrad_bn", dy)(*args, stream()), "conv2d_dgrad")
     return out
@@ -738,7 +769,7 @@
              (BN_SUMS_PARKED if park else 0))
     if workspace is None:
         workspace = _scratch(12 * C + L().dspn_bn_tiles_workspace_bytes(tiles, C), x.device, "bn_from_sums")
-    assert dy.dtype == x.dtype
+    assert (dy is None and phase == 1) or dy.dtype == x.dtype
     check(_f("dspn_bn_backward_from_sums", x)(ptr(x), ptr(scale), ptr(shift), ptr(dy), ptr(mean), ptr(rstd), ptr(gamma),
                                              ptr(sums), tiles, ptr(dx), ptr(dgamma), ptr(dbeta), rows, C, int(relu),
                                              int(accumulate), ptr(dx_absmax), ptr(dx_absmin), ptr(dy_absmax), ptr(x_chan_minmax),
diff --git a/dspnet_amd/graph_plan.py b/dspnet_amd/graph_plan.py
--- a/dspnet_amd/graph_plan.py
+++ b/dspnet_amd/graph_plan.py
@@ -38,6 +38,7 @@
     if os.environ.get("DSPN_DY_PLANES", "1") != "0":
         gradient_planes(g, index)
     shortcut_compaction(g, index)
+    bn1_recompute(g, index)
 
 
 def resolve_auto_deferred(g, index):
@@ -132,6 +133,21 @@
         largest = max(largest, N * ((H + 1) // 2) * ((W + 1) // 2) * C)
     if largest:
         g.sc_compact_buf = fn.zeros(largest, device=g.device)
+
+
+def bn1_recompute(g, index):
+    if g.math != "f16x2" or g.device.type != "cuda":
+        return
+    for idx, c in enumerate(g.nodes):
+        n = c.bn_bwd_node if isinstance(c, E.Conv) else None
+        if n is None or c.sc_pair is not None or c.math != "f16x2" or n.out.dtype != torch.float32:
+            continue
+        if not (c.w.shape[1:3] == (1, 1) and c.stride == 1 and c.pad == (0, 0) and c.dil == 1 and not c.tap_expand
+                and c.input_sum_grad is None and c.x is n.out and n.out.shape[3] == c.w.shape[3]):
+            continue
+        if index.reader_nodes(n.out) != {idx} or n.dx_planes or not n.x.requires_grad:
+            continue
+        c.bn1_recompute = True
 
 
 def input_planes(g):
diff --git a/include/dspn_nn.h b/include/dspn_nn.h
--- a/include/dspn_nn.h
+++ b/include/dspn_nn.h
@@ -62,6 +62,18 @@
                                   void *workspace, size_t workspace_bytes, const float *strided_addend, int addend_h, int addend_w,
                                   void *stream);
 int dspn_conv2d_dgrad_bn_sadd_route_f32(int N, int H, int W, int Cin, int ldy, int dy_planes);
+int dspn_conv2d_dgrad_bn_sums_f32(const float *dy, const float *wt, const void *wt_planes, float *dx, int N, int H, int W, int Cin, int ldy,
+                                  int R, int S, int stride, int pad_h, int pad_w, int dil, int Ho, int Wo, int dx_ldc,
+                                  int accumulate, const float *bn_x, const float *bn_scale, const float *bn_shift,
+                                  const float *bn_mean, const float *bn_rstd, int bn_relu, float *bn_sums,
+                                  size_t bn_sums_bytes, float *bn_dy_absmax, int math, const float *dy_absmax, const float *w_absmax,
+                                  void *workspace, size_t workspace_bytes, void *stream);
+int dspn_conv2d_dgrad_bn_apply_f32(const float *dy, const float *wt, const void *wt_planes, float *dx, int N, int H, int W, int Cin, int ldy,
+                                   int R, int S, int stride, int pad_h, int pad_w, int dil, int Ho, int Wo, int dx_ldc,
+                                   int accumulate, const float *bn_x, const float *bn_scale, const float *bn_shift, int bn_relu,
+                                   float *dx_absmax, int math, const float *dy_absmax, const float *w_absmax,
+                                   const void *bn_workspace, size_t bn_workspace_bytes, void *stream);
+int dspn_conv2d_dgrad_bn_recompute_route_f32(int N, int H, int W, int Cin, int ldy, int dy_planes);
 
 size_t dspn_conv2d_input_sum_grad_workspace_bytes(int Ho, int Wo, int ldy, int R, int S);
 int dspn_conv2d_input_sum_grad_f32(const float *dy, const float *w, float *out, int N, int H, int W,
@@ -124,6 +136,19 @@
                                    const float *absmax_unused_a, const float *absmax_unused_b, void *workspace,
                                    size_t workspace_bytes, const dspn_bf16 *strided_addend, int addend_h, int addend_w,
                                    void *stream);
+int dspn_conv2d_dgrad_bn_sums_bf16(const dspn_bf16 *dy, const dspn_bf16 *wt, const void *wt_planes_unused, dspn_bf16 *dx, int N, int H, int W,
+                                   int Cin, int ldy, int R, int S, int stride, int pad_h, int pad_w, int dil, int Ho, int Wo,
+                                   int dx_ldc, int accumulate, const dspn_bf16 *bn_x, const float *bn_scale,
+                                   const float *bn_shift, const float *bn_mean, const float *bn_rstd, int bn_relu,
+                                   float *bn_sums, size_t bn_sums_bytes, float *bn_dy_absmax_unused, int math,
+                                   const float *absmax_unused_a, const float *absmax_unused_b, void *workspace,
+                                   size_t workspace_bytes, void *stream);
+int dspn_conv2d_dgrad_bn_apply_bf16(const dspn_bf16 *dy, const dspn_bf16 *wt, const void *wt_planes_unused, dspn_bf16 *dx, int N, int H, int W,
+                                    int Cin, int ldy, int R, int S, int stride, int pad_h, int pad_w, int dil, int Ho, int Wo,
+                                    int dx_ldc, int accumulate, const dspn_bf16 *bn_x, const float *bn_scale,
+                                    const float *bn_shift, int bn_relu, float *dx_absmax_unused, int math,
+                                    const float *absmax_unused_a, const float *absmax_unused_b, const void *bn_workspace,
+                                    size_t bn_workspace_bytes, void *stream);
 int dspn_conv2d_wgrad_bn_bf16(const dspn_bf16 *x, const float *in_scale, const float *in_shift, int in_relu,
                               const dspn_bf16 *dy, float *dw, int N, int H, int W, int Cin, int Cout, int ldy,
                               int R, int S, int stride, int pad_h, int pad_w, int dil, int Ho, int Wo,
```

After: 985.7 images/s (median of 6 runs). 1.1% higher.
